# cassiusfive/balatro-gym

Measured on AMD Instinct MI355X. Metric: env-steps/sec at 65536 envs, random policy; achieved HBM GB/s vs peak, higher is better.
Workload: dtype int64/f64

## Files before the change

balatro_gym_amd/csrc/bg_device.h:

```cpp
#pragma once
#include <hip/hip_runtime.h>
#include <stdint.h>
#include "bg_tables.h"

#define BG_NHOT 8
#define BG_NDECK 4
#define BG_NCOLD 7
#define BG_NTMPL 2
#define BG_MT_N 624
#define BG_MT_M 397
#define BG_MTS 640
#define BG_BLOCK 64

#define BG_DEVERR_GSTREAM 1u
#define BG_DEVERR_SHOPBLK 2u
#define BG_DEVERR_DECKRING 4u
#define BG_DEVERR_SHOPRING 8u

typedef __attribute__((address_space(1))) unsigned long long g_u64;
typedef __attribute__((address_space(1))) uint32_t g_u32;
__device__ __forceinline__ unsigned long long bg_ld8a(const void* p) { return __hip_atomic_load((g_u64*)p, __ATOMIC_RELAXED, __HIP_MEMORY_SCOPE_AGENT); }
__device__ __forceinline__ uint32_t bg_ld4a(const void* p) { return __hip_atomic_load((g_u32*)p, __ATOMIC_RELAXED, __HIP_MEMORY_SCOPE_AGENT); }
__device__ __forceinline__ void bg_st8a(void* p, unsigned long long v) { __hip_atomic_store((g_u64*)p, v, __ATOMIC_RELAXED, __HIP_MEMORY_SCOPE_AGENT); }
__device__ __forceinline__ uint4 bg_ld16a(const void* p) {
  const unsigned long long a = bg_ld8a(p), b = bg_ld8a((const char*)p + 8);
  return make_uint4((uint32_t)a, (uint32_t)(a >> 32), (uint32_t)b, (uint32_t)(b >> 32));
}

struct BgDev {
  int N;
  uint32_t flags;
  int max_ante;
  int KG, KS, KD;
  uint4* hot;
  uint4* deck;
  uint4* cold;
  uint4* tmpl;
  uint4* ndeck;
  uint32_t* gblk;
  uint32_t* sblk;
  uint32_t* sovf;
  uint32_t* deckmt;
  uint32_t* shopgenmt;
  uint32_t* err;
  uint32_t* wl_count;
  uint32_t* wl;
  uint32_t* wl_shop;
  uint32_t* sseed;
  uint32_t* smeta;
  const uint32_t* prod_view;
  const uint32_t* prod_in;
  uint32_t* prod_out;
  unsigned long long* dbg;
  uint4* cstate;
  uint4* ctmpl;
  uint32_t* cardmt;
  uint32_t* sealmt;
  const uint32_t* jtab;
};

struct Env {
  int64_t chips_scored, round_chips;
  int64_t best_hand;
  int32_t chips_needed, money;
  int32_t hp_total, hp_ante, jokers_sold, shop_reroll_state, shop_reroll_base;
  int32_t ante, round, phase, hands_left, discards_left, hand_size, nhand, nsel, njokers, ncons, n_magic, n_minim,
      boss_type, boss_req, bflags, shop_n;
  uint64_t hand, sel;
  uint32_t highlighted, face_down, boss_hp, boss_types, cons0, cons1;
  uint64_t jokers;
  int32_t shop_ante, d_head, d_cons, d_ready;
  uint64_t boss_cards;
  uint64_t levels;
  int32_t g_cur, g_cons, g_valid;
  int32_t g_idx, s_idx, s_cur, s_cons, s_ready;
  int32_t ndrop, nfo;
  uint64_t excess;
  int32_t max_ante;
};

#define BG_BF_FIRST_HAND 1
#define BG_BF_SHOP_EXISTS 2

__device__ __forceinline__ uint32_t bg_b(uint32_t w, int i) { return (w >> (8 * i)) & 0xffu; }

__device__ __forceinline__ void bg_unpack(const uint4 c[BG_NHOT], Env& e) {
  e.chips_scored = (int64_t)(((uint64_t)c[0].y << 32) | c[0].x);
  e.round_chips = (int64_t)(((uint64_t)c[0].w << 32) | c[0].z);
  e.best_hand = (int64_t)(((uint64_t)c[1].y << 32) | c[1].x);
  e.chips_needed = (int32_t)c[1].z;
  e.money = (int32_t)c[1].w;
  e.hp_total = (int32_t)c[2].x;
  e.hp_ante = (int32_t)(c[2].y & 0xffffu);
  e.jokers_sold = (int32_t)(c[2].y >> 16);
  e.shop_reroll_state = (int32_t)c[2].z;
  e.shop_reroll_base = (int32_t)c[2].w;
  e.ante = bg_b(c[3].x, 0); e.round = bg_b(c[3].x, 1); e.phase = bg_b(c[3].x, 2); e.hands_left = bg_b(c[3].x, 3);
  e.discards_left = bg_b(c[3].y, 0); e.hand_size = (int)(int8_t)bg_b(c[3].y, 1);  e.nhand = bg_b(c[3].y, 2); e.nsel = bg_b(c[3].y, 3);
  e.njokers = bg_b(c[3].z, 0); e.ncons = bg_b(c[3].z, 1); e.n_magic = bg_b(c[3].z, 2); e.n_minim = bg_b(c[3].z, 3);
  e.boss_type = bg_b(c[3].w, 0); e.boss_req = bg_b(c[3].w, 1); e.bflags = bg_b(c[3].w, 2); e.shop_n = bg_b(c[3].w, 3);
  e.hand = ((uint64_t)c[4].y << 32) | c[4].x;
  e.sel = ((uint64_t)c[4].w << 32) | c[4].z;
  e.highlighted = c[5].x & 0xffffu; e.face_down = bg_b(c[5].x, 2); e.boss_hp = bg_b(c[5].x, 3);
  e.boss_types = c[5].y & 0xffffu; e.cons0 = bg_b(c[5].y, 2); e.cons1 = bg_b(c[5].y, 3);
  e.jokers = (uint64_t)c[5].z | ((uint64_t)(c[5].w & 0xffu) << 32);
  e.shop_ante = bg_b(c[5].w, 1); e.d_head = bg_b(c[5].w, 2); e.d_cons = bg_b(c[5].w, 3); e.d_ready = 0;
  e.boss_cards = ((uint64_t)c[6].y << 32) | c[6].x;
  e.levels = (uint64_t)c[6].z | ((uint64_t)(c[6].w & 0xffffu) << 32);
  e.g_cur = bg_b(c[6].w, 2); e.g_cons = bg_b(c[6].w, 3); e.g_valid = 0;
  e.g_idx = (int32_t)(c[7].x & 0xffffu); e.s_idx = (int32_t)(c[7].x >> 16);
  e.s_cur = bg_b(c[7].y, 0); e.s_cons = bg_b(c[7].y, 1); e.s_ready = 0; e.ndrop = bg_b(c[7].y, 2); e.nfo = bg_b(c[7].y, 3);
  e.excess = (uint64_t)c[7].z | ((uint64_t)(c[7].w & 0xffffu) << 32);
  e.max_ante = (int32_t)(c[7].w >> 16) & 0xff;
}

__device__ __forceinline__ uint32_t bg_p4(int a, int b, int c, int d) {
  return (uint32_t)(a & 0xff) | ((uint32_t)(b & 0xff) << 8) | ((uint32_t)(c & 0xff) << 16) | ((uint32_t)(d & 0xff) << 24);
}

__device__ __forceinline__ void bg_pack(const Env& e, uint4 c[BG_NHOT]) {
  c[0] = make_uint4((uint32_t)e.chips_scored, (uint32_t)((uint64_t)e.chips_scored >> 32), (uint32_t)e.round_chips,
                    (uint32_t)((uint64_t)e.round_chips >> 32));
  c[1] = make_uint4((uint32_t)e.best_hand, (uint32_t)((uint64_t)e.best_hand >> 32), (uint32_t)e.chips_needed, (uint32_t)e.money);
  c[2] = make_uint4((uint32_t)e.hp_total, ((uint32_t)e.hp_ante & 0xffffu) | ((uint32_t)e.jokers_sold << 16),
                    (uint32_t)e.shop_reroll_state, (uint32_t)e.shop_reroll_base);
  c[3] = make_uint4(bg_p4(e.ante, e.round, e.phase, e.hands_left), bg_p4(e.discards_left, e.hand_size, e.nhand, e.nsel),
                    bg_p4(e.njokers, e.ncons, e.n_magic, e.n_minim), bg_p4(e.boss_type, e.boss_req, e.bflags, e.shop_n));
  c[4] = make_uint4((uint32_t)e.hand, (uint32_t)(e.hand >> 32), (uint32_t)e.sel, (uint32_t)(e.sel >> 32));
  c[5] = make_uint4((e.highlighted & 0xffffu) | ((e.face_down & 0xffu) << 16) | ((e.boss_hp & 0xffu) << 24),
                    (e.boss_types & 0xffffu) | ((e.cons0 & 0xffu) << 16) | ((e.cons1 & 0xffu) << 24), (uint32_t)e.jokers,
                    bg_p4((int)(e.jokers >> 32), e.shop_ante, e.d_head, e.d_cons));
  c[6] = make_uint4((uint32_t)e.boss_cards, (uint32_t)(e.boss_cards >> 32), (uint32_t)e.levels,
                    ((uint32_t)(e.levels >> 32) & 0xffffu) | ((uint32_t)(e.g_cur & 0xff) << 16) | ((uint32_t)(e.g_cons & 0xff) << 24));
  c[7] = make_uint4(((uint32_t)e.g_idx & 0xffffu) | ((uint32_t)e.s_idx << 16), bg_p4(e.s_cur, e.s_cons, e.ndrop, e.nfo),
                    (uint32_t)e.excess, ((uint32_t)(e.excess >> 32) & 0xffffu) | ((uint32_t)(e.max_ante & 0xff) << 16));
}

__device__ __forceinline__ void bg_derive_ready(Env& e, uint32_t prod) {
  e.d_ready = (int)((prod - (uint32_t)e.d_cons) & 0xffu);
  e.s_ready = (int)(((prod >> 8) - (uint32_t)e.s_cons) & 0xffu);
  e.g_valid = (int)(((prod >> 16) - (uint32_t)e.g_cons) & 0xffu);
}
__device__ __forceinline__ void bg_load_env(const BgDev& d, int env, Env& e) {
  uint4 c[BG_NHOT];
#pragma unroll
  for (int k = 0; k < BG_NHOT; k++) c[k] = d.hot[(size_t)k * d.N + env];
  bg_unpack(c, e);
  bg_derive_ready(e, d.prod_view ? d.prod_view[env] : 0u);
}
__device__ __forceinline__ void bg_store_env(const BgDev& d, int env, const Env& e) {
  uint4 c[BG_NHOT];
  bg_pack(e, c);
#pragma unroll
  for (int k = 0; k < BG_NHOT; k++) d.hot[(size_t)k * d.N + env] = c[k];
}

__device__ __forceinline__ int bg_get8(uint64_t v, int i) { return (int)((v >> (8 * i)) & 0xffull); }
__device__ __forceinline__ uint64_t bg_set8(uint64_t v, int i, int x) {
  return (v & ~(0xffull << (8 * i))) | ((uint64_t)(x & 0xff) << (8 * i));
}
__device__ __forceinline__ uint64_t bg_del8(uint64_t v, int i) {
  uint64_t lowmask = i ? ((1ull << (8 * i)) - 1) : 0ull;
  uint64_t lo = v & lowmask;
  uint64_t hi = (i < 7) ? (v >> (8 * (i + 1))) << (8 * i) : 0ull;
  return lo | hi;
}
__device__ __forceinline__ int bg_level(const Env& e, int ht) { return (int)((e.levels >> (4 * ht)) & 0xf); }

__device__ __forceinline__ uint32_t* bg_gblock(const BgDev& d, int env, int slot) { return d.gblk + ((size_t)env * d.KG + slot) * BG_MTS; }
#define BG_SW_T 56
#define BG_SW_PK 56
#define BG_SW_SEED 62
#define BG_SLOT_WORDS 64
#define BG_S_FASTMAX (BG_SW_T - 1)
static_assert(BG_SW_T >= 28 && BG_SW_PK == BG_SW_T && BG_SW_PK % 4 == 0 && BG_SW_PK + 6 == BG_SW_SEED && BG_SW_SEED + 2 == BG_SLOT_WORDS, "shop slot");
#define BG_BF_SHOP_OVF 4
__device__ __forceinline__ uint32_t* bg_sblock(const BgDev& d, int env, int slot) { return d.sblk + ((size_t)env * d.KS + slot) * BG_SLOT_WORDS; }
__device__ __forceinline__ uint32_t* bg_sovf(const BgDev& d, int env) { return d.sovf + (size_t)env * BG_MTS; }
__device__ __forceinline__ void bg_mt_seed_rolled(uint32_t* p, uint32_t key) {
  uint32_t g = 19650218u, a = g;
#pragma unroll 1
  for (uint32_t i = 1; i < 624u; i++) {
    g = 1812433253u * (g ^ (g >> 30)) + i;
    a = (g ^ ((a ^ (a >> 30)) * 1664525u)) + key;
    p[i] = a;
  }
  __builtin_amdgcn_fence(__ATOMIC_RELEASE, "agent");
  __builtin_amdgcn_fence(__ATOMIC_ACQUIRE, "agent");
  const uint32_t m1 = (p[1] ^ ((a ^ (a >> 30)) * 1664525u)) + key;
  uint32_t b = m1;
#pragma unroll 1
  for (uint32_t i = 2; i < 624u; i++) {
    b = (p[i] ^ ((b ^ (b >> 30)) * 1566083941u)) - i;
    p[i] = b;
  }
  p[1] = (m1 ^ ((b ^ (b >> 30)) * 1566083941u)) - 1u;
  p[0] = 0x80000000u;
}
__device__ __forceinline__ uint32_t* bg_deckmt(const BgDev& d, int env) { return d.deckmt + (size_t)env * BG_MTS; }
__device__ __forceinline__ uint32_t* bg_shopgenmt(const BgDev& d, int env) { return d.shopgenmt + (size_t)env * BG_MTS; }

#ifdef BG_TIMING
__shared__ unsigned long long bg_probe_lds[32];
#define BG_PROBE_BEGIN() unsigned long long _pt = __builtin_readcyclecounter()
#define BG_PROBE(k) do { unsigned long long _n = __builtin_readcyclecounter(); \
    if ((int)threadIdx.x == __ffsll((long long)__ballot(1)) - 1 + (int)(threadIdx.x & ~63u)) atomicAdd(&bg_probe_lds[k], _n - _pt); \
    _pt = __builtin_readcyclecounter(); } while (0)
#define BG_PROBE_INIT() do { if (threadIdx.x < 32) bg_probe_lds[threadIdx.x] = 0; __syncthreads(); } while (0)
#define BG_PROBE_FLUSH(d) do { __syncthreads(); if (threadIdx.x < 32 && (d).dbg && bg_probe_lds[threadIdx.x]) atomicAdd(&(d).dbg[threadIdx.x], bg_probe_lds[threadIdx.x]); } while (0)
#else
#define BG_PROBE_BEGIN() do {} while (0)
#define BG_PROBE(k) do {} while (0)
#define BG_PROBE_INIT() do {} while (0)
#define BG_PROBE_FLUSH(d) do {} while (0)
#endif

#define BG_RB 128
typedef __attribute__((address_space(3))) uint8_t lds_u8;
typedef __attribute__((address_space(3))) uint32_t lds_u32;
struct Deck0 { uint64_t lo, hi; static constexpr bool kCards = false; };
struct DeckLds { lds_u32* col; static constexpr bool kCards = false; };
struct Deck0C : Deck0 { static constexpr bool kCards = true; };
struct DeckLdsC : DeckLds { static constexpr bool kCards = true; };
#define BG_NCST 7
__device__ __forceinline__ uint32_t bg_cstate(const BgDev& d, int env, int ci) {
  return (uint32_t)((const uint16_t*)&d.cstate[(size_t)(ci >> 3) * d.N + env])[ci & 7];
}
__device__ __forceinline__ Deck0 bg_load_deck0(const BgDev& d, int env) {
  uint4 c = d.deck[env];
  Deck0 r;
  r.lo = ((uint64_t)c.y << 32) | c.x;
  r.hi = ((uint64_t)c.w << 32) | c.z;
  return r;
}
__device__ __forceinline__ void bg_deck_set(Deck0& dk, int k, uint4 c) {
  if (k == 0) { dk.lo = ((uint64_t)c.y << 32) | c.x; dk.hi = ((uint64_t)c.w << 32) | c.z; }
}
__device__ __forceinline__ void bg_deck_set(DeckLds& dk, int k, uint4 c) {
  dk.col[(4 * k) * BG_RB] = c.x; dk.col[(4 * k + 1) * BG_RB] = c.y; dk.col[(4 * k + 2) * BG_RB] = c.z; dk.col[(4 * k + 3) * BG_RB] = c.w;
}
__device__ __forceinline__ int bg_card(const BgDev& d, int env, const Deck0& k, int idx) {
  if (idx < 16) return (int)(((idx < 8 ? k.lo : k.hi) >> (8 * (idx & 7))) & 0xffull);
  const uint32_t* p = (const uint32_t*)&d.deck[(size_t)(idx >> 4) * d.N + env];
  return (int)((bg_ld4a(p + ((idx & 15) >> 2)) >> (8 * (idx & 3))) & 0xffu);
}
template <int S, bool C> struct DeckLdsS { lds_u32* col; static constexpr bool kCards = C; };
template <int S, bool C>
__device__ __forceinline__ void bg_deck_set(DeckLdsS<S, C>& dk, int k, uint4 c) {
  dk.col[(4 * k) * S] = c.x; dk.col[(4 * k + 1) * S] = c.y; dk.col[(4 * k + 2) * S] = c.z; dk.col[(4 * k + 3) * S] = c.w;
}
template <int S, bool C>
__device__ __forceinline__ int bg_card(const BgDev& d, int env, const DeckLdsS<S, C>& k, int idx) {
  return (int)((const lds_u8*)k.col)[(idx >> 2) * (S * 4) + (idx & 3)];
}
__device__ __forceinline__ int bg_card(const BgDev& d, int env, const DeckLds& k, int idx) {
  return (int)((const lds_u8*)k.col)[(idx >> 2) * (BG_RB * 4) + (idx & 3)];
}

struct DeckHead { uint64_t lo, hi; };
__device__ __forceinline__ DeckHead bg_deck_head(const BgDev& d, int env, const Deck0& k) { return DeckHead{k.lo, k.hi}; }
template <int S, bool C>
__device__ __forceinline__ DeckHead bg_deck_head(const BgDev& d, int env, const DeckLdsS<S, C>& k) {
  const uint32_t a = k.col[0], b = k.col[S], c = k.col[2 * S], e = k.col[3 * S];
  return DeckHead{((uint64_t)b << 32) | a, ((uint64_t)e << 32) | c};
}
template <class DK>
__device__ __forceinline__ int bg_card_h(const BgDev& d, int env, const DK& k, const DeckHead& h, int idx) {
  if (idx < 16) return (int)(((idx < 8 ? h.lo : h.hi) >> (8 * (idx & 7))) & 0xffull);
  return bg_card(d, env, k, idx);
}

__device__ __forceinline__ uint32_t bg_temper(uint32_t y) {
  y ^= (y >> 11);
  y ^= (y << 7) & 0x9d2c5680u;
  y ^= (y << 15) & 0xefc60000u;
  y ^= (y >> 18);
  return y;
}
__device__ __forceinline__ uint32_t bg_twist(uint32_t a, uint32_t b, uint32_t far) {
  uint32_t y = (a & 0x80000000u) | (b & 0x7fffffffu);
  return far ^ (y >> 1) ^ ((y & 1u) ? 0x9908b0dfu : 0u);
}

__device__ __forceinline__ uint32_t bg_lazy_next(uint32_t* S) {
  uint32_t c = S[BG_MT_N] & 0x3ffu;
  const uint32_t c1 = c + 1 == BG_MT_N ? 0u : c + 1, cf = c + BG_MT_M >= BG_MT_N ? c + BG_MT_M - BG_MT_N : c + BG_MT_M;
  const uint32_t y = bg_twist(S[c], S[c1], S[cf]);
  S[c] = y;
  S[BG_MT_N] = c1 | 0x80000000u;
  return bg_temper(y);
}
__device__ __forceinline__ double bg_lazy_random(uint32_t* S) {
  const uint32_t a = bg_lazy_next(S) >> 5, b = bg_lazy_next(S) >> 6;
  return ((double)a * 67108864.0 + (double)b) * (1.0 / 9007199254740992.0);
}

#define BG_WIN 16
struct JTables {
  uint64_t jd[152];
  uint32_t jm[152];
  uint64_t jr[152];
  uint8_t jf[152];
  uint8_t cost[152];
  double pow115[101];
  double pow15[16];
  double pow08[16];
  uint32_t inv[64];
};
typedef __attribute__((address_space(3))) const JTables lds_JTables;
struct RngWin {
  lds_JTables* jt;
  lds_u32* lds;
  int g_blk, g_start, g_len;
  int s_start, s_len;
  bool defer_adv;
  bool need_inv;
};
__device__ __forceinline__ void bg_win_init(RngWin& w, uint32_t* lds_lane, const JTables* jt = nullptr) {
  w.jt = (lds_JTables*)jt; w.lds = (lds_u32*)lds_lane; w.g_blk = -1; w.g_start = 0; w.g_len = 0; w.s_start = 0; w.s_len = 0; w.defer_adv = false; w.need_inv = false;
}
__device__ __noinline__ void bg_win_fill(lds_u32* lds, const uint32_t* src, int len) {
#pragma unroll 1
  for (int base = 0; base < len; base += BG_WIN) {
    uint32_t v[BG_WIN];
#pragma unroll
    for (int j = 0; j < BG_WIN; j++) v[j] = (base + j < len) ? src[base + j] : 0u;
#pragma unroll
    for (int j = 0; j < BG_WIN; j++) if (base + j < len) lds[(base + j) * BG_BLOCK] = v[j];
  }
}

__device__ __forceinline__ void bg_gnorm(const BgDev& d, Env& e) {
  if (e.g_idx >= BG_MT_N) { e.g_cur = (e.g_cur + 1 == d.KG) ? 0 : e.g_cur + 1; e.g_idx -= BG_MT_N; e.g_valid--; e.g_cons = (e.g_cons + 1) & 0xff; }
}
__device__ __forceinline__ void bg_gskip(const BgDev& d, Env& e, int count) {
  bg_gnorm(d, e);
  e.g_idx += count;
}
__device__ __forceinline__ uint32_t bg_gdraw(const BgDev& d, int env, Env& e, RngWin& w) {
  bg_gnorm(d, e);
  if (e.g_valid <= 0) { atomicOr(d.err, BG_DEVERR_GSTREAM); e.g_valid = 0; return 0u; }
  uint32_t off = (uint32_t)(e.g_idx - w.g_start);
  uint32_t y;
  if (w.g_blk == e.g_cur && off < (uint32_t)w.g_len) y = w.lds[off * BG_BLOCK];
  else y = bg_gblock(d, env, e.g_cur)[e.g_idx];
  e.g_idx++;
  return bg_temper(y);
}
__device__ __forceinline__ uint32_t bg_gpeek(const BgDev& d, int env, const Env& e, int off) {
  int idx = e.g_idx + off, blk = e.g_cur, need = 1;
  if (idx >= BG_MT_N) { idx -= BG_MT_N; blk = (blk + 1 == d.KG) ? 0 : blk + 1; need = 2; }
  if (idx >= BG_MT_N) { idx -= BG_MT_N; blk = (blk + 1 == d.KG) ? 0 : blk + 1; need = 3; }
  if (e.g_valid < need) { atomicOr(d.err, BG_DEVERR_GSTREAM); return 0u; }
  return bg_temper(bg_gblock(d, env, blk)[idx]);
}
__device__ __forceinline__ const uint32_t* bg_gpeek_addr(const BgDev& d, int env, const Env& e, int off, bool& ok) {
  int idx = e.g_idx + off, blk = e.g_cur, need = 1;
  if (idx >= BG_MT_N) { idx -= BG_MT_N; blk = (blk + 1 == d.KG) ? 0 : blk + 1; need = 2; }
  if (idx >= BG_MT_N) { idx -= BG_MT_N; blk = (blk + 1 == d.KG) ? 0 : blk + 1; need = 3; }
  ok = e.g_valid >= need;
  return bg_gblock(d, env, ok ? blk : e.g_cur) + (ok ? idx : 0);
}
__device__ __forceinline__ uint32_t bg_gtouch(const BgDev& d, int env, const Env& e, int off) {
  int idx = e.g_idx + off, blk = e.g_cur, need = 1;
  if (idx >= BG_MT_N) { idx -= BG_MT_N; blk = (blk + 1 == d.KG) ? 0 : blk + 1; need = 2; }
  if (idx >= BG_MT_N) { idx -= BG_MT_N; blk = (blk + 1 == d.KG) ? 0 : blk + 1; need = 3; }
  return e.g_valid >= need ? bg_gblock(d, env, blk)[idx] : 0u;
}
struct __attribute__((packed, aligned(4))) BgU4 { uint32_t x, y, z, w; };
__device__ __forceinline__ void bg_gpeek12(const BgDev& d, int env, const Env& e, int skip, uint32_t (&out)[12], uint32_t& avail) {
  int idx = e.g_idx + skip, blk = e.g_cur, need = 1;
  if (idx >= BG_MT_N) { idx -= BG_MT_N; blk = (blk + 1 == d.KG) ? 0 : blk + 1; need = 2; }
  if (idx >= BG_MT_N) { idx -= BG_MT_N; blk = (blk + 1 == d.KG) ? 0 : blk + 1; need = 3; }
  avail = 0;
  if (e.g_valid >= need) {
    const int in_blk = BG_MT_N - idx;
    avail = (e.g_valid > need || in_blk >= 12) ? 0xfffu : ((1u << in_blk) - 1u);
    const BgU4* p = (const BgU4*)(bg_gblock(d, env, blk) + idx);
#pragma unroll
    for (int g = 0; g < 3; g++) {
      BgU4 v = p[g];
      out[4 * g] = bg_temper(v.x); out[4 * g + 1] = bg_temper(v.y); out[4 * g + 2] = bg_temper(v.z); out[4 * g + 3] = bg_temper(v.w);
    }
  } else {
#pragma unroll
    for (int i = 0; i < 12; i++) out[i] = 0u;
  }
}
__device__ __forceinline__ void bg_gpeek12_raw(const BgDev& d, int env, const Env& e, int skip, uint32_t (&out)[12], uint32_t& avail) {
  int idx = e.g_idx + skip, blk = e.g_cur, need = 1;
  if (idx >= BG_MT_N) { idx -= BG_MT_N; blk = (blk + 1 == d.KG) ? 0 : blk + 1; need = 2; }
  if (idx >= BG_MT_N) { idx -= BG_MT_N; blk = (blk + 1 == d.KG) ? 0 : blk + 1; need = 3; }
  const bool have = e.g_valid >= need;
  const int in_blk = BG_MT_N - idx;
  avail = have ? ((e.g_valid > need || in_blk >= 12) ? 0xfffu : ((1u << in_blk) - 1u)) : 0u;
  const BgU4* p = (const BgU4*)(bg_gblock(d, env, have ? blk : e.g_cur) + (have ? idx : 0));
#pragma unroll
  for (int g = 0; g < 3; g++) {
    const BgU4 v = p[g];
    out[4 * g] = v.x; out[4 * g + 1] = v.y; out[4 * g + 2] = v.z; out[4 * g + 3] = v.w;
  }
}
__device__ __forceinline__ void bg_gprefetch(const BgDev& d, int env, Env& e, RngWin& w, int count) {
  bg_gnorm(d, e);
  if (e.g_valid <= 0) return;
  int len = BG_MT_N - e.g_idx;
  if (len > count) len = count;
  if (len > BG_WIN) len = BG_WIN;
  bg_win_fill(w.lds, bg_gblock(d, env, e.g_cur) + e.g_idx, len);
  w.g_blk = e.g_cur; w.g_start = e.g_idx; w.g_len = len;
  w.s_len = 0;
}
__device__ __noinline__ uint32_t bg_sword_slow(const uint32_t* S, int k) {
  uint32_t far;
  if (k < BG_MT_N - BG_MT_M) far = S[k + BG_MT_M];
  else {
    const int k1 = k - (BG_MT_N - BG_MT_M);
    uint32_t far1;
    if (k1 < BG_MT_N - BG_MT_M) far1 = S[k1 + BG_MT_M];
    else { const int k2 = k1 - (BG_MT_N - BG_MT_M); far1 = bg_twist(S[k2], S[k2 + 1], S[k2 + BG_MT_M]); }
    far = bg_twist(S[k1], S[k1 + 1], far1);
  }
  const uint32_t nxt = k < BG_MT_N - 1 ? S[k + 1] : bg_twist(S[0], S[1], S[BG_MT_M]);
  return bg_twist(S[k], nxt, far);
}
__device__ __forceinline__ void bg_shop_overflow(const BgDev& d, int env, Env& e) {
  bg_mt_seed_rolled(bg_sovf(d, env), bg_sblock(d, env, e.s_cur)[BG_SW_SEED]);
  __builtin_amdgcn_fence(__ATOMIC_RELEASE, "agent");
  __builtin_amdgcn_fence(__ATOMIC_ACQUIRE, "agent");
  e.bflags |= BG_BF_SHOP_OVF;
}
__device__ __forceinline__ const uint32_t* bg_sbase(const BgDev& d, int env, const Env& e, bool& full) {
  full = (e.bflags & BG_BF_SHOP_OVF) != 0;
  if (full) __builtin_amdgcn_fence(__ATOMIC_ACQUIRE, "agent");
  return full ? bg_sovf(d, env) : bg_sblock(d, env, e.s_cur);
}
__device__ __forceinline__ uint32_t bg_sdraw(const BgDev& d, int env, Env& e, RngWin& w) {
  if (e.s_idx >= BG_MT_N) { atomicOr(d.err, BG_DEVERR_SHOPBLK); return 0u; }
  uint32_t off = (uint32_t)(e.s_idx - w.s_start);
  uint32_t y;
  if (off < (uint32_t)w.s_len) y = w.lds[off * BG_BLOCK];
  else {
    if (e.s_idx > BG_S_FASTMAX && !(e.bflags & BG_BF_SHOP_OVF)) bg_shop_overflow(d, env, e);
    bool full;
    const uint32_t* S = bg_sbase(d, env, e, full);
    y = full ? bg_temper(bg_sword_slow(S, e.s_idx)) : S[e.s_idx];
  }
  e.s_idx++;
  return y;
}
__device__ __forceinline__ void bg_swin_fill(lds_u32* lds, const uint32_t* S, bool full, int k0, int len) {
  if (!full) {
    uint32_t A[BG_WIN];
#pragma unroll
    for (int j = 0; j < BG_WIN; j++) A[j] = (j < len) ? S[k0 + j] : 0u;
#pragma unroll
    for (int j = 0; j < BG_WIN; j++) if (j < len) lds[j * BG_BLOCK] = A[j];
    return;
  }
  uint32_t A[BG_WIN + 1], F[BG_WIN];
  const uint32_t* SF = S + k0 + BG_MT_M;
#pragma unroll
  for (int j = 0; j < BG_WIN + 1; j++) A[j] = (j <= len) ? S[k0 + j] : 0u;
#pragma unroll
  for (int j = 0; j < BG_WIN; j++) F[j] = (j < len) ? SF[j] : 0u;
#pragma unroll
  for (int j = 0; j < BG_WIN; j++) if (j < len) lds[j * BG_BLOCK] = bg_temper(bg_twist(A[j], A[j + 1], F[j]));
}
__device__ __forceinline__ void bg_sprefetch(const BgDev& d, int env, Env& e, RngWin& w, int count) {
  bool full;
  const uint32_t* S = bg_sbase(d, env, e, full);
  int len = (full ? (BG_MT_N - BG_MT_M) : (BG_S_FASTMAX + 1)) - e.s_idx;
  if (len > count) len = count;
  if (len > BG_WIN) len = BG_WIN;
  if (len < 0) len = 0;
  if (len > 0) bg_swin_fill(w.lds, S, full, e.s_idx, len);
  w.s_start = e.s_idx; w.s_len = len;
  w.g_len = 0; w.g_blk = -1;
}
template <bool SHOP>
__device__ __forceinline__ uint32_t bg_randbelow(const BgDev& d, int env, Env& e, RngWin& w, uint32_t n) {
  int k = 32 - __clz(n);
  uint32_t r;
  int guard = 0;
  do {
    r = (SHOP ? bg_sdraw(d, env, e, w) : bg_gdraw(d, env, e, w)) >> (32 - k);
  } while (r >= n && ++guard < 4096);
  return r < n ? r : 0u;
}
__device__ __forceinline__ double bg_grandom(const BgDev& d, int env, Env& e, RngWin& w) {
  uint32_t a = bg_gdraw(d, env, e, w) >> 5;
  uint32_t b = bg_gdraw(d, env, e, w) >> 6;
  return ((double)a * 67108864.0 + (double)b) * (1.0 / 9007199254740992.0);
}

__device__ __forceinline__ int bg_card_chips(int code) {
  int r = (code >> 2) + 2;
  return r <= 10 ? r : (r == 14 ? 11 : 10);
}
__device__ __forceinline__ void bg_hand_base(int ht, int level, int& chips, int& mult) {
  int bc, bm;
  switch (ht) {
    case 0: bc = 5; bm = 1; break;
// ... 80 lines not shown
```

balatro_gym_amd/csrc/bg_lib.hip:

```cpp
#include "../../include/balatro_mi355x.h"
#include "bg_step.h"
#include <hip/hip_ext.h>
#include <stdio.h>
#include <stdlib.h>
#include <string.h>
#include <type_traits>
#include <string>
#include <vector>


struct InfoPtrs {
  int64_t* final_score; int32_t* error; int32_t* flags; int32_t* aux; int8_t* hand_type; int8_t* cards_played;
  double* reward_terms;
  double* score_breakdown;
};

static_assert(offsetof(ObsPtrs, rows) == sizeof(bg_obs_ptrs), "the first 31 members of ObsPtrs must mirror bg_obs_ptrs");
static_assert(sizeof(InfoPtrs) == sizeof(bg_info_ptrs), "InfoPtrs must mirror bg_info_ptrs");

__device__ __forceinline__ void bg_emit_info(size_t row, const StepOut& o, uint8_t* trunc, const InfoPtrs& info) {
  if (trunc) trunc[row] = 0;
  if (info.final_score) info.final_score[row] = o.final_score;
  if (info.error) info.error[row] = o.error;
  if (info.flags) info.flags[row] = o.flags;
  if (info.aux) info.aux[row] = o.aux;
  if (info.hand_type) info.hand_type[row] = (int8_t)o.hand_type;
  if (info.cards_played) info.cards_played[row] = (int8_t)o.cards_played;
  if (info.reward_terms) {
    double2* q = (double2*)(info.reward_terms + row * 8);
#pragma unroll
    for (int i = 0; i < 4; i++) q[i] = make_double2(o.terms[2 * i], o.terms[2 * i + 1]);
  }
  if (info.score_breakdown && o.hand_type < 0) {
    double2* q = (double2*)(info.score_breakdown + row * 8);
#pragma unroll
    for (int i = 0; i < 4; i++) q[i] = make_double2(0.0, 0.0);
  }
}

#include "bg_engine.h"
#include "bg_engine3.h"

template <bool CARDS>
__global__ __launch_bounds__(BG_BLOCK) void bg_reset_kernel(BgDev d, const uint8_t* __restrict__ mask_in, ObsPtrs obs) {
  using DeckT = typename std::conditional<CARDS, Deck0C, Deck0>::type;
  int env = blockIdx.x * BG_BLOCK + threadIdx.x;
  if (env >= d.N) return;
  Env e;
  bg_load_env(d, env, e);
  DeckT dk; static_cast<Deck0&>(dk) = bg_load_deck0(d, env);
  if (!mask_in || mask_in[env]) { bg_env_reset(d, env, e, dk); bg_store_env(d, env, e); }
  ShopRegs sr; sr.valid = false;
  uint64_t mask = bg_action_mask(d, env, e, sr);
  bg_write_obs<false>(d, env, (size_t)env, e, dk, obs, mask, sr, RowExtra{0.0, 0, 0u});
}

__global__ __launch_bounds__(BG_BLOCK) void bg_observe_kernel(BgDev d, ObsPtrs obs) {
  int env = blockIdx.x * BG_BLOCK + threadIdx.x;
  if (env >= d.N) return;
  Env e;
  bg_load_env(d, env, e);
  Deck0 dk = bg_load_deck0(d, env);
  ShopRegs sr; sr.valid = false;
  uint64_t mask = bg_action_mask(d, env, e, sr);
  bg_write_obs<false>(d, env, (size_t)env, e, dk, obs, mask, sr, RowExtra{0.0, 0, 0u});
}

struct alignas(64) BgG16 { uint32_t v[16]; };
struct BgGenrandTab {
  BgG16 blk[BG_MT_N / 16];
  constexpr BgGenrandTab() : blk{} {
    uint32_t x = 19650218u;
    blk[0].v[0] = x;
    for (int i = 1; i < BG_MT_N; i++) { x = 1812433253u * (x ^ (x >> 30)) + (uint32_t)i; blk[i / 16].v[i % 16] = x; }
  }
};
static_assert(BG_MT_N % 16 == 0, "624 = 39 blocks of 16");
static constexpr BgGenrandTab BG_GENRAND{};

template <bool SLOT>
__device__ __forceinline__ void bg_mt_seed_impl(uint32_t* p, uint32_t key) {
  constexpr int NB = BG_MT_N / 16;
  uint4* p4 = (uint4*)p;
  uint32_t a = BG_GENRAND.blk[0].v[0], a1 = 0;
  {
    BgG16 cur = BG_GENRAND.blk[0];
#pragma unroll 1
    for (int b = 0; b < NB; b++) {
      const BgG16 nxt = BG_GENRAND.blk[b + 1 < NB ? b + 1 : NB - 1];
#pragma unroll
      for (int c = 0; c < 16; c++) {
        if (b > 0 || c >= 1) {
          a = (cur.v[c] ^ ((a ^ (a >> 30)) * 1664525u)) + key;
          if (b == 0 && c == 1) a1 = a;
        }
      }
      cur = nxt;
    }
  }
  const uint32_t a1w = (a1 ^ ((a ^ (a >> 30)) * 1664525u)) + key;
  a = BG_GENRAND.blk[0].v[0];
  a = (BG_GENRAND.blk[0].v[1] ^ ((a ^ (a >> 30)) * 1664525u)) + key;
  uint32_t bprev = a1w, w2 = 0, w3 = 0;
  uint32_t far0 = 0, far1 = 0, out2 = 0, out3 = 0;
  uint32_t acc = 0;
  {
    BgG16 cur = BG_GENRAND.blk[0];
#pragma unroll 1
    for (int b = 0; b < NB; b++) {
      const BgG16 nxt = BG_GENRAND.blk[b + 1 < NB ? b + 1 : NB - 1];
      uint32_t v[16];
#pragma unroll
      for (int c = 0; c < 16; c++) {
        v[c] = 0;
        if (b > 0 || c >= 2) {
          a = (cur.v[c] ^ ((a ^ (a >> 30)) * 1664525u)) + key;
          bprev = (a ^ ((bprev ^ (bprev >> 30)) * 1566083941u)) - (uint32_t)(16 * b + c);
          v[c] = bprev;
        }
      }
      if (b == 0) { w2 = v[2]; w3 = v[3]; }
      if constexpr (!SLOT) {
#pragma unroll
        for (int k = 0; k < 4; k++) {
          const int q = 4 * b + k;
          if (q == 0) continue;
          p4[q] = make_uint4(v[4 * k], v[4 * k + 1], v[4 * k + 2], v[4 * k + 3]);
        }
      } else {
        if (b < 4) {
#pragma unroll
          for (int k = 0; k < 4; k++) if (4 * b + k > 0) p4[4 * b + k] = make_uint4(v[4 * k], v[4 * k + 1], v[4 * k + 2], v[4 * k + 3]);
        } else if (b >= 24 && b <= 28) {
          const int kb = 16 * b - BG_MT_M;
          if (b == 24) { far0 = v[13]; far1 = v[14]; out2 = bg_temper(bg_twist(w2, w3, v[15])); }
          else {
            const int g0 = kb >> 2;
            uint32_t nr[20];
#pragma unroll
            for (int g = 0; g < 5; g++) {
              uint4 t = make_uint4(0u, 0u, 0u, 0u);
              if (g0 + g > 0 && g0 + g < BG_SLOT_WORDS / 4) t = p4[g0 + g];
              nr[4 * g] = t.x; nr[4 * g + 1] = t.y; nr[4 * g + 2] = t.z; nr[4 * g + 3] = t.w;
            }
            if (b == 25) nr[3] = w3;
            auto outputs = [&](auto kbc) {
              constexpr int KB = decltype(kbc)::value;
#pragma unroll
              for (int c = 0; c < 16; c++) {
                const int k = KB + c;
                if (k < BG_SW_T) {
                  const uint32_t o = bg_temper(bg_twist(nr[3 + c], nr[4 + c], v[c]));
                  if (k == 3) out3 = o; else p[k] = o;
                  if (k >= 4 && k < 24) {
                    acc |= (o >> 24) << (8 * (k & 3));
                    if ((k & 3) == 3) { p[BG_SW_PK + (k >> 2)] = acc; acc = 0u; }
                  }
                }
              }
            };
            if (b == 25) outputs(std::integral_constant<int, 16 * 25 - BG_MT_M>{});
            else if (b == 26) outputs(std::integral_constant<int, 16 * 26 - BG_MT_M>{});
            else if (b == 27) outputs(std::integral_constant<int, 16 * 27 - BG_MT_M>{});
            else outputs(std::integral_constant<int, 16 * 28 - BG_MT_M>{});
          }
        }
      }
      cur = nxt;
    }
  }
  const uint32_t w1 = (a1w ^ ((bprev ^ (bprev >> 30)) * 1566083941u)) - 1u;
  if constexpr (!SLOT) p4[0] = make_uint4(0x80000000u, w1, w2, w3);
  else {
    const uint32_t out0 = bg_temper(bg_twist(0x80000000u, w1, far0)), out1 = bg_temper(bg_twist(w1, w2, far1));
    p4[0] = make_uint4(out0, out1, out2, out3);
    static_assert(BG_SW_PK == 56 && BG_SW_SEED == 62 && BG_SLOT_WORDS == 64, "slot tail layout");
    p[BG_SW_PK] = (out0 >> 24) | ((out1 >> 24) << 8) | ((out2 >> 24) << 16) | (out3 & 0xff000000u);
    *(uint2*)(p + BG_SW_SEED) = make_uint2(key, 0u);
  }
}
__device__ void bg_mt_seed(uint32_t* __restrict__ p, uint32_t key) { bg_mt_seed_impl<false>(p, key); }
__device__ void bg_mt_seed_slot(uint32_t* __restrict__ p, uint32_t key) { bg_mt_seed_impl<true>(p, key); }

__device__ __forceinline__ uint32_t bg_q156(uint32_t q) { return q >= 156u ? q - 156u : q; }
#define BG_LAZY_U 4
#define BG_LAZY_U_SEEDRING 2
#define BG_WL_COUNTERS 32
#define BG_REFILL_WAVE_PRIO 0
template <int U = BG_LAZY_U, class F>
__device__ __forceinline__ uint32_t bg_lazy_stream(uint32_t* S, uint32_t c, bool active, F&& take) {
  uint4* S4 = (uint4*)S;
  uint32_t q = c >> 2, off = c & 3u, fq = bg_q156(q + 99u);
  uint4 a[U + 1], f[U + 1];
#pragma unroll
  for (int g = 0; g <= U; g++) { a[g] = make_uint4(0, 0, 0, 0); f[g] = a[g]; }
  if (active) {
#pragma unroll
    for (int g = 0; g <= U; g++) { a[g] = S4[bg_q156(q + (uint32_t)g)]; f[g] = S4[bg_q156(fq + (uint32_t)g)]; }
  }
#pragma unroll 1
  while (__ballot(active) != 0ull) {
    uint4 an[U], fn[U];
#pragma unroll
    for (int g = 0; g < U; g++) { an[g] = a[0]; fn[g] = a[0]; }
    if (active) {
#pragma unroll
      for (int g = 0; g < U; g++) { an[g] = S4[bg_q156(q + (uint32_t)(U + 1 + g))]; fn[g] = S4[bg_q156(fq + (uint32_t)(U + 1 + g))]; }
    }
    bool more = active;
#pragma unroll
    for (int g = 0; g < U; g++) {
      const uint4 a0 = a[g], f0 = f[g];
      const uint32_t n0 = bg_twist(a0.x, a0.y, f0.y), n1 = bg_twist(a0.y, a0.z, f0.z), n2 = bg_twist(a0.z, a0.w, f0.w), n3 = bg_twist(a0.w, a[g + 1].x, f[g + 1].x);
      const uint32_t goff = g == 0 ? off : 0u;
      uint4 o = a0;
      uint32_t used = 0;
      if (more && goff == 0u) { o.x = n0; used++; more = take(n0); }
      if (more && goff <= 1u) { o.y = n1; used++; more = take(n1); }
      if (more && goff <= 2u) { o.z = n2; used++; more = take(n2); }
      if (more) { o.w = n3; used++; more = take(n3); }
      if (used) {
        const uint32_t qg = bg_q156(q + (uint32_t)g);
        S4[qg] = o;
        if (!more) { c = 4u * qg + goff + used; if (c >= (uint32_t)BG_MT_N) c -= (uint32_t)BG_MT_N; active = false; }
      }
    }
    q = bg_q156(q + (uint32_t)U); fq = bg_q156(fq + (uint32_t)U); off = 0u;
    a[0] = a[U]; f[0] = f[U];
#pragma unroll
    for (int g = 0; g < U; g++) { a[g + 1] = an[g]; f[g + 1] = fn[g]; }
  }
  return c;
}

#define BG_MTB 16
#define BG_SSEED 128
#define BG_LAZY_SEEDED 0x80000000u
__device__ void bg_mt_twist(const uint32_t* src, uint32_t* dst) {
  uint32_t cur = src[0], first_new = 0;
  const uint4* s4 = (const uint4*)src;
  uint4* d4 = (uint4*)dst;
#pragma unroll 1
  for (int base = 0; base < BG_MT_N; base += BG_MTB) {
    uint32_t nx[BG_MTB + 4], fr[BG_MTB + 4];
#pragma unroll
    for (int g = 0; g < BG_MTB / 4 + 1; g++) { uint4 v = s4[base / 4 + g]; nx[4 * g] = v.x; nx[4 * g + 1] = v.y; nx[4 * g + 2] = v.z; nx[4 * g + 3] = v.w; }
    if (base == 224) {
#pragma unroll
      for (int j = 0; j < BG_MTB; j++) { int kk = base + j; fr[j + 1] = (kk < BG_MT_N - BG_MT_M) ? src[kk + BG_MT_M] : dst[kk + BG_MT_M - BG_MT_N]; }
    } else {
      const uint4* f4 = base < 224 ? s4 + (base + BG_MT_M - 1) / 4 : (const uint4*)dst + (base + BG_MT_M - BG_MT_N - 1) / 4;
#pragma unroll
      for (int g = 0; g < BG_MTB / 4 + 1; g++) { uint4 v = f4[g]; fr[4 * g] = v.x; fr[4 * g + 1] = v.y; fr[4 * g + 2] = v.z; fr[4 * g + 3] = v.w; }
    }
    uint32_t v[BG_MTB];
#pragma unroll
    for (int j = 0; j < BG_MTB; j++) {
      uint32_t nxt = (base + j == BG_MT_N - 1) ? first_new : nx[j + 1];
      v[j] = bg_twist(cur, nxt, fr[j + 1]);
      if (base + j == 0) first_new = v[j];
      cur = nxt;
    }
#pragma unroll
    for (int j = 0; j < BG_MTB / 4; j++) d4[base / 4 + j] = make_uint4(v[4 * j], v[4 * j + 1], v[4 * j + 2], v[4 * j + 3]);
  }
}

#include "bg_ops.h"
#include "bg_sim.h"
#include "bg_encode.h"
#include "bg_gae.h"
#include "bg_norm.h"
#include "bg_head.h"

__global__ __launch_bounds__(BG_BLOCK) void bg_seed_kernel(BgDev d, const int64_t* __restrict__ seeds,
                                                          const uint8_t* __restrict__ mask_in, int reseed_global) {
  int env = blockIdx.x * BG_BLOCK + threadIdx.x;
  if (env >= d.N) return;
  if (mask_in && !mask_in[env]) return;
  RngWin w;
  bg_win_init(w, nullptr);
  Env e;
  bg_load_env(d, env, e);
  int64_t seed = seeds[env];
  if (reseed_global) {
    uint32_t gs = (uint32_t)((uint64_t)seed + 16000ull);
    uint32_t* g = bg_gblock(d, env, 0);
    bg_mt_seed(g, gs);
    bg_mt_twist(g, g);
    e.g_cur = 0; e.g_idx = 0; e.g_cons = 0; e.g_valid = 1;
  }
  if (seed == 0) {
    uint64_t r;
    int guard = 0;
    do {
      uint64_t lo = bg_gdraw(d, env, e, w);
      uint64_t hi = bg_gdraw(d, env, e, w) >> 31;
      r = lo | (hi << 32);
    } while (r >= 4294967296ull && ++guard < 4096);
    seed = (int64_t)(r & 0xffffffffull);
  }
  uint32_t base = (uint32_t)(uint64_t)seed;
  bg_mt_seed(bg_deckmt(d, env), base);
  bg_deckmt(d, env)[BG_MT_N] = BG_LAZY_SEEDED;
  bg_mt_seed(bg_shopgenmt(d, env), base + 2000u);
  bg_shopgenmt(d, env)[BG_MT_N] = BG_LAZY_SEEDED;
  if (d.cardmt) {
    bg_mt_seed(d.cardmt + (size_t)env * BG_MTS, base + 11000u);
    d.cardmt[(size_t)env * BG_MTS + BG_MT_N] = BG_LAZY_SEEDED;
    bg_mt_seed(d.sealmt + (size_t)env * BG_MTS, base + 13000u);
    d.sealmt[(size_t)env * BG_MTS + BG_MT_N] = BG_LAZY_SEEDED;
  }
  e.d_head = 0; e.d_cons = 0; e.d_ready = 0;
  e.s_cons = 0; e.s_ready = 0;
  d.smeta[env] = 0;
  {
    uint32_t gp = reseed_global ? 1u : (uint32_t)((e.g_cons + e.g_valid) & 0xff);
    uint32_t pv = 0u | (0u << 8) | (gp << 16) | 0x80000000u;
    d.prod_out[env] = pv;
    ((uint32_t*)d.prod_in)[env] = pv;
  }
  bg_store_env(d, env, e);
}

__global__ __launch_bounds__(BG_BLOCK) void bg_refill_zero_kernel(BgDev d) { if (threadIdx.x < BG_WL_COUNTERS) d.wl_count[threadIdx.x] = 0; }

struct BgPart { uint32_t p, q; };
__device__ __forceinline__ uint32_t bg_part_lo(uint32_t count, BgPart pt) { return (uint32_t)(((uint64_t)count * pt.p) / pt.q); }
__device__ __forceinline__ uint32_t bg_part_hi(uint32_t count, BgPart pt) { return (uint32_t)(((uint64_t)count * (pt.p + 1u)) / pt.q); }

__global__ __launch_bounds__(BG_BLOCK) void bg_refill_scan_kernel(BgDev d) {
  int env = blockIdx.x * BG_BLOCK + threadIdx.x;
  if (env >= d.N) return;
  size_t N = d.N;
  uint32_t w5 = ((const uint32_t*)&d.hot[(size_t)5 * N + env])[3];
  uint32_t w6 = ((const uint32_t*)&d.hot[(size_t)6 * N + env])[3];
  uint2 w7 = *((const uint2*)&d.hot[(size_t)7 * N + env]);
  uint32_t prod = d.prod_in[env];
  int d_cons = bg_b(w5, 3), g_cons = bg_b(w6, 3), s_cur = bg_b(w7.y, 0), s_cons = bg_b(w7.y, 1);
  int d_ready = (int)((prod - (uint32_t)d_cons) & 0xffu);
  int s_ready = (int)(((prod >> 8) - (uint32_t)s_cons) & 0xffu);
  int g_valid = (int)(((prod >> 16) - (uint32_t)g_cons) & 0xffu);
  const bool seeded = (prod >> 31) != 0;
  if (!seeded) { d.prod_out[env] = prod; return; }
  if (s_ready < d.KS - 1) {
    uint32_t sm = d.smeta[env];
    int head = (int)(sm & 0xffu), cnt = (int)((sm >> 8) & 0xffu);
    int emitted = d.KS - 1 - s_ready;
    if (emitted > cnt) emitted = cnt;
    if (emitted > 0) {
      const uint32_t base = atomicAdd(&d.wl_count[3], (uint32_t)emitted);
#pragma unroll 1
      for (int k = 0; k < emitted; k++) {
        int slot = s_cur + 1 + s_ready + k; while (slot >= d.KS) slot -= d.KS;
        d.wl_shop[2 * (size_t)(base + k)] = (uint32_t)env | ((uint32_t)slot << 24);
        d.wl_shop[2 * (size_t)(base + k) + 1] = d.sseed[(size_t)env * BG_SSEED + ((head + k) & (BG_SSEED - 1))];
      }
      head = (head + emitted) & (BG_SSEED - 1); cnt -= emitted;
    } else emitted = 0;
    if (emitted) {
      d.smeta[env] = (uint32_t)head | ((uint32_t)cnt << 8);
      prod = (prod & 0xffff00ffu) | ((((prod >> 8) + (uint32_t)emitted) & 0xffu) << 8);
    }
    if (cnt < BG_SSEED - 8) { uint32_t i = atomicAdd(&d.wl_count[1], 1u); d.wl[N + i] = (uint32_t)env; }
  }
  d.prod_out[env] = prod;
  if (d_ready < d.KD) { uint32_t i = atomicAdd(&d.wl_count[0], 1u); d.wl[i] = (uint32_t)env; }
  if (g_valid > 0 && g_valid < d.KG) { uint32_t i = atomicAdd(&d.wl_count[2], 1u); d.wl[2 * N + i] = (uint32_t)env; }
}

__global__ __launch_bounds__(BG_BLOCK) __attribute__((amdgpu_waves_per_eu(4, 4))) void bg_refill_deck_kernel(BgDev d, BgPart pt, uint32_t cursor_idx, uint32_t max_made) {
  __builtin_amdgcn_s_setprio(BG_REFILL_WAVE_PRIO);
  __shared__ uint8_t sdeck[52][BG_BLOCK];
  const size_t N = d.N;
  const int tid = threadIdx.x;
  const uint32_t count0 = d.wl_count[0], lo = bg_part_lo(count0, pt), count = bg_part_hi(count0, pt);
  uint32_t* const cursor = &d.wl_count[cursor_idx];
  const int cap = max_made ? (int)max_made : 1 << 30;
  int env = 0, d_head = 0, d_ready = 0, made = 0;
  uint32_t prod = 0, cur = 0;
  uint32_t* mt = bg_deckmt(d, 0);
  bool have = false, need = false, dry = false;
#pragma unroll 1
  while (true) {
    if (!dry) {
      const unsigned long long freem = __ballot(!have);
      if (freem != 0ull) {
        const int leader = __ffsll(freem) - 1, nfree = __popcll(freem);
        uint32_t base = 0;
        if (tid == leader) base = atomicAdd(cursor, (uint32_t)nfree);
        base = lo + (uint32_t)__shfl((int)base, leader);
        dry = base + (uint32_t)nfree >= count;
        const uint32_t my = base + (uint32_t)__popcll(freem & ((1ull << tid) - 1ull));
        if (!have && my < count) {
          env = (int)d.wl[my];
          mt = bg_deckmt(d, env);
          const uint32_t w5 = ((const uint32_t*)&d.hot[(size_t)5 * N + env])[3];
          prod = d.prod_out[env];
          d_head = bg_b(w5, 2);
          d_ready = (int)((prod - (uint32_t)bg_b(w5, 3)) & 0xffu);
          cur = mt[BG_MT_N] & 0x3ffu;
          made = 0;
          need = d_ready < d.KD;
          have = need;
        }
      }
    }
    if (__ballot(need) == 0ull) { if (dry) break; continue; }
    if (need) { int p = 0; for (int s = 0; s < 4; s++) for (int r = 0; r < 13; r++) sdeck[p++][tid] = (uint8_t)(r * 4 + s); }
    int i = 51;
    cur = bg_lazy_stream(mt, cur, need, [&](uint32_t y) {
      const int k = 32 - __clz((uint32_t)(i + 1));
      const uint32_t j = bg_temper(y) >> (32 - k);
      if (j <= (uint32_t)i) {
        const uint8_t a = sdeck[i][tid], b = sdeck[j][tid];
        sdeck[i][tid] = b; sdeck[j][tid] = a;
        i--;
      }
      return i >= 1;
    });
    if (need) {
      const int slot = (d_head + d_ready) % d.KD;
#pragma unroll
      for (int k = 0; k < BG_NDECK; k++) {
        uint32_t wv[4] = {0, 0, 0, 0};
#pragma unroll
        for (int b = 0; b < 16; b++) { int i2 = k * 16 + b; if (i2 < 52) wv[b >> 2] |= (uint32_t)sdeck[i2][tid] << (8 * (b & 3)); }
        d.ndeck[((size_t)slot * BG_NDECK + k) * N + env] = make_uint4(wv[0], wv[1], wv[2], wv[3]);
      }
      d_ready++; made++;
      need = d_ready < d.KD && made < cap;
      if (!need) {
        mt[BG_MT_N] = cur | BG_LAZY_SEEDED;
        ((uint8_t*)&d.prod_out[env])[0] = (uint8_t)((prod + (uint32_t)made) & 0xffu);
        have = false;
      }
    }
  }
}

__global__ __launch_bounds__(BG_BLOCK) void bg_refill_seedring_kernel(BgDev d, BgPart pt) {
  __builtin_amdgcn_s_setprio(BG_REFILL_WAVE_PRIO);
  size_t N = d.N;
  const uint32_t count0 = d.wl_count[1], lo = bg_part_lo(count0, pt), count = bg_part_hi(count0, pt);
  for (uint32_t base = lo + blockIdx.x * BG_BLOCK; base < count; base += gridDim.x * BG_BLOCK) {
    const bool valid = base + threadIdx.x < count;
    const int env = valid ? (int)d.wl[N + base + threadIdx.x] : 0;
    uint32_t* mt = bg_shopgenmt(d, env);
    int head = 0, cnt = BG_SSEED;
    uint32_t cur = 0;
    if (valid) {
      const uint32_t sm = d.smeta[env];
      head = (int)(sm & 0xffu); cnt = (int)((sm >> 8) & 0xffu);
      cur = mt[BG_MT_N] & 0x3ffu;
    }
    const bool need = valid && cnt < BG_SSEED;
    cur = bg_lazy_stream<BG_LAZY_U_SEEDRING>(mt, cur, need, [&](uint32_t y) {
      const uint32_t r = bg_temper(y);
      if (r < 2147483648u) { d.sseed[(size_t)env * BG_SSEED + ((head + cnt) & (BG_SSEED - 1))] = r; cnt++; }
      return cnt < BG_SSEED;
    });
    if (need) {
      mt[BG_MT_N] = cur | BG_LAZY_SEEDED;
      d.smeta[env] = (uint32_t)head | ((uint32_t)cnt << 8);
    }
  }
}

__global__ __launch_bounds__(BG_BLOCK, 8) void bg_refill_shop_kernel(BgDev d, BgPart pt) {
  const uint32_t count0 = d.wl_count[3], lo = bg_part_lo(count0, pt), count = bg_part_hi(count0, pt);
  for (uint32_t item = lo + blockIdx.x * BG_BLOCK + threadIdx.x; item < count; item += gridDim.x * BG_BLOCK) {
    uint32_t es = d.wl_shop[2 * (size_t)item], seed = d.wl_shop[2 * (size_t)item + 1];
    bg_mt_seed_slot(bg_sblock(d, (int)(es & 0xffffffu), (int)(es >> 24)), seed);
  }
}
__global__ __launch_bounds__(BG_BLOCK) void bg_refill_gblk_kernel(BgDev d, BgPart pt) {
  __builtin_amdgcn_s_setprio(BG_REFILL_WAVE_PRIO);
  const size_t N = d.N;
  const uint32_t count0 = d.wl_count[2], lo = bg_part_lo(count0, pt), count = bg_part_hi(count0, pt);
  const int l = threadIdx.x;
  constexpr int NR = (BG_MT_N + 63) / 64;
  for (uint32_t item = lo + blockIdx.x; item < count; item += gridDim.x) {
    const int env = (int)d.wl[2 * N + item];
    const uint32_t w6 = ((const uint32_t*)&d.hot[(size_t)6 * N + env])[3];
    const uint32_t prod = d.prod_out[env];
    const int g_cur = bg_b(w6, 2), g_cons = bg_b(w6, 3);
    int g_valid = (int)(((prod >> 16) - (uint32_t)g_cons) & 0xffu);
    if (g_valid <= 0 || g_valid >= d.KG) continue;
    int last = (g_cur + g_valid - 1) % d.KG, made = 0;
    uint32_t o[NR + 1];
    {
      const uint32_t* src = bg_gblock(d, env, last);
#pragma unroll
      for (int r = 0; r < NR; r++) o[r] = (64 * r + l < BG_MT_N) ? __builtin_nontemporal_load(&src[64 * r + l]) : 0u;
      o[NR] = 0u;
    }
#pragma unroll 1
    while (g_valid < d.KG) {
      const int nxt = last + 1 == d.KG ? 0 : last + 1;
      uint32_t* dst = bg_gblock(d, env, nxt);
      uint32_t n[NR];
#pragma unroll
      for (int r = 0; r < NR; r++) {
        const int k = 64 * r + l;
        const uint32_t up_same = __shfl(o[r], (l + 1) & 63), up_next = __shfl(o[r + 1], 0);
        uint32_t up = l == 63 ? up_next : up_same;
        if (r == NR - 1) { const uint32_t new0 = __shfl(n[0], 0); if (k == BG_MT_N - 1) up = new0; }
        uint32_t far = 0u;
        if (64 * r < BG_MT_N - BG_MT_M) {
          const uint32_t a = r + 6 < NR ? __shfl(o[r + 6], (l + 13) & 63) : 0u, b2 = r + 7 < NR ? __shfl(o[r + 7], (l + 13) & 63) : 0u;
          far = l + 13 < 64 ? a : b2;
        }
        if (64 * r + 63 >= BG_MT_N - BG_MT_M) {
          const uint32_t a = r >= 4 ? __shfl(n[r >= 4 ? r - 4 : 0], (l + 29) & 63) : 0u, b2 = r >= 3 ? __shfl(n[r >= 3 ? r - 3 : 0], (l + 29) & 63) : 0u;
          const uint32_t fn = l + 29 < 64 ? a : b2;
          if (k >= BG_MT_N - BG_MT_M) far = fn;
        }
        n[r] = bg_twist(o[r], up, far);
        if (k < BG_MT_N) __builtin_nontemporal_store(n[r], &dst[k]);
      }
      if (l < 16) bg_gblock(d, env, last)[BG_MT_N + l] = n[0];
#pragma unroll
      for (int r = 0; r < NR; r++) o[r] = n[r];
      last = nxt; g_valid++; made++;
    }
    if (made && l == 0) {
      const uint32_t g = ((prod >> 16) + (uint32_t)made) & 0xffu;
      ((uint8_t*)&d.prod_out[env])[2] = (uint8_t)g;
    }
  }
}

__global__ __launch_bounds__(BG_BLOCK) void bg_inject_kernel(BgDev d, const uint8_t* __restrict__ mask_in) {
  int env = blockIdx.x * BG_BLOCK + threadIdx.x;
  if (env >= d.N) return;
  if (mask_in && !mask_in[env]) return;
  Env e;
  bg_load_env(d, env, e);
  uint4 t0 = d.tmpl[env], t1 = d.tmpl[(size_t)d.N + env];
  if (t0.y & 0x80000000u) { e.njokers = (int)bg_b(t0.y, 1); e.jokers = (uint64_t)t0.x | ((uint64_t)(t0.y & 0xffu) << 32); }
  if (t0.y & 0x40000000u) e.money = (int32_t)t0.z;
  if (t0.y & 0x20000000u) e.ante = (int)bg_b(t0.y, 2);
  if (t0.y & 0x10000000u) { e.levels = (uint64_t)t1.x | ((uint64_t)(t1.y & 0xffffu) << 32); e.excess = 0; }
  if (t1.z & 0x80000000u) { e.ncons = (int)bg_b(t1.z, 0); e.cons0 = bg_b(t1.z, 1); e.cons1 = bg_b(t1.z, 2); }
  bg_store_env(d, env, e);
}

__global__ __launch_bounds__(256) void bg_tables_build_kernel(uint32_t* out) {
  __shared__ JTables jt;
  { uint32_t* w = (uint32_t*)&jt; for (int i = threadIdx.x; i < (int)(sizeof(JTables) / 4); i += blockDim.x) w[i] = 0u; }
  __syncthreads();
  bg_tables_init(&jt);
  const uint32_t* w = (const uint32_t*)&jt;
  for (int i = threadIdx.x; i < (int)(sizeof(JTables) / 4); i += blockDim.x) out[i] = w[i];
}

__global__ __launch_bounds__(BG_BLOCK) void bg_inject_deck_kernel(BgDev d, const uint4* __restrict__ decks, const uint8_t* __restrict__ mask_in) {
  int env = blockIdx.x * BG_BLOCK + threadIdx.x;
  if (env >= d.N) return;
  if (mask_in && !mask_in[env]) return;
#pragma unroll
  for (int k = 0; k < BG_NDECK; k++) d.deck[(size_t)k * d.N + env] = decks[(size_t)env * BG_NDECK + k];
}
__global__ __launch_bounds__(BG_BLOCK) void bg_set_cap_kernel(BgDev d, const int32_t* __restrict__ caps, int scalar, const uint8_t* __restrict__ mask_in) {
  int env = blockIdx.x * BG_BLOCK + threadIdx.x;
  if (env >= d.N) return;
  if (mask_in && !mask_in[env]) return;
  uint32_t* w = ((uint32_t*)&d.hot[(size_t)7 * d.N + env]) + 3;
  const int cap = caps ? caps[env] : scalar;
  *w = (*w & 0xffffu) | ((uint32_t)(cap & 0xff) << 16);
}

struct bg_handle {
  BgDev dev;
  int device_id;
  bool seeded;
  int64_t* d_seeds;
  uint8_t* d_mask;
  uint32_t* d_jtab;
  int steps_since_refill;
  std::vector<uint4> h_tmpl;
  std::vector<hipEvent_t> ev_pool;
  std::vector<uint8_t> h_cap;
  uint64_t bytes;
  std::string err;
  bool profiling;
  uint32_t* d_prod[2];
  long refill_seq;
  long refill_done;
  long view_min;
  bool async_refill;
  hipStream_t side;
  hipEvent_t ev_refill[2];
  hipEvent_t ev_rollout;
  std::vector<hipEvent_t> ev_rollout_t, ev_refill_t, ev_step_t;
  std::vector<int> rollout_steps;
  struct RefillPiece { int kind; uint32_t part, nparts; int grid; uint32_t cursor, max_made; };
  std::vector<RefillPiece> pieces;
  size_t piece_next;
  BgDev piece_dev;
  int refill_sliced, piece_parts[4], deck_passes;
  uint32_t eng_smask; int eng_copiers;
  int engine;
  int e3_cfg, e3_epw;
  uint8_t* gpeer[8]; uint8_t** d_gpeer; int gworld, grank;
};

static std::string g_create_err;

struct BgDeviceGuard {
  int prev = -1;
  bool switched = false;
  explicit BgDeviceGuard(int dev) {
    if (hipGetDevice(&prev) == hipSuccess && prev != dev) switched = hipSetDevice(dev) == hipSuccess;
  }
  ~BgDeviceGuard() { if (switched) (void)hipSetDevice(prev); }
};
#define BG_GUARD(h) BgDeviceGuard _guard((h)->device_id)

#define BG_HIP(call)                                                                                   \
  do {                                                                                                 \
    hipError_t _e = (call);                                                                            \
    if (_e != hipSuccess) {                                                                            \
      h->err = std::string(#call) + ": " + hipGetErrorString(_e);                                      \
      return BG_E_HIP;                                                                                 \
    }                                                                                                  \
  } while (0)

template <typename T>
static hipError_t bg_alloc(bg_handle* h, T** p, size_t count) {
  size_t bytes = count * sizeof(T);
  hipError_t e = hipMalloc((void**)p, bytes);
  if (e != hipSuccess) return e;
  h->bytes += bytes;
  return hipMemset(*p, 0, bytes);
}

static int bg_grid(const bg_handle* h) { return (h->dev.N + BG_BLOCK - 1) / BG_BLOCK; }

static hipEvent_t bg_ev_take(bg_handle* h) {
  if (!h->ev_pool.empty()) { hipEvent_t e = h->ev_pool.back(); h->ev_pool.pop_back(); return e; }
  hipEvent_t e = nullptr;
  return hipEventCreate(&e) == hipSuccess ? e : nullptr;
}
static void bg_ev_begin(bg_handle* h, std::vector<hipEvent_t>& v, hipStream_t s) {
  if (!h->profiling) return;
  hipEvent_t a = bg_ev_take(h), b = bg_ev_take(h);
  if (!a || !b) { if (a) h->ev_pool.push_back(a); if (b) h->ev_pool.push_back(b); return; }
  v.push_back(a); v.push_back(b);
  (void)hipEventRecord(a, s);
}
static void bg_ev_pair(bg_handle* h, std::vector<hipEvent_t>& v, hipEvent_t& a, hipEvent_t& b) {
  a = b = nullptr;
  if (!h->profiling) return;
  a = bg_ev_take(h); b = bg_ev_take(h);
  if (!a || !b) { if (a) h->ev_pool.push_back(a); if (b) h->ev_pool.push_back(b); a = b = nullptr; return; }
  v.push_back(a); v.push_back(b);
}
static void bg_ev_end(bg_handle* h, std::vector<hipEvent_t>& v, hipStream_t s) {
  if (!h->profiling || v.empty()) return;
  (void)hipEventRecord(v.back(), s);
}
static double bg_ev_sum(bg_handle* h, std::vector<hipEvent_t>& v) {
  double ms = 0;
  for (size_t i = 0; i + 1 < v.size(); i += 2) {
    float f = 0;
    if (hipEventElapsedTime(&f, v[i], v[i + 1]) == hipSuccess) ms += f;
    h->ev_pool.push_back(v[i]); h->ev_pool.push_back(v[i + 1]);
  }
  v.clear();
  return ms;
}

#ifndef BG_BUILD_SIGNATURE
#define BG_BUILD_SIGNATURE "unsigned"
#endif

extern "C" {

static const char bg_sig_marker[] = "bgsig:" BG_BUILD_SIGNATURE;
const char* bg_build_signature(void) { return bg_sig_marker + 6; }

int bg_debug_counters(bg_handle* h, unsigned long long* out16) {
  if (!h || !out16) return BG_E_ARG;
  BG_GUARD(h);
  BG_HIP(hipDeviceSynchronize());
  BG_HIP(hipMemcpy(out16, h->dev.dbg, 32 * sizeof(unsigned long long), hipMemcpyDeviceToHost));
  BG_HIP(hipMemset(h->dev.dbg, 0, 32 * sizeof(unsigned long long)));
  return 0;
}

static long bg_gwords(int flags, int steps) { return (flags & BG_FLAG_SCORER_JOKERS) ? 32l * steps + 128 : 24l * steps; }
static int bg_gsteps(int flags, int blocks) {
  const long w = (long)blocks * BG_MT_N;
  const long t = (flags & BG_FLAG_SCORER_JOKERS) ? (w - 128) / 32 : w / 24;
  return t < 0 ? 0 : (int)t;
}

int bg_debug_worklists(bg_handle* h, unsigned int* out4) {
  if (!h || !out4) return BG_E_ARG;
  BG_GUARD(h);
  BG_HIP(hipDeviceSynchronize());
  BG_HIP(hipMemcpy(out4, h->dev.wl_count, 4 * sizeof(unsigned int), hipMemcpyDeviceToHost));
  return 0;
}

int bg_set_profiling(bg_handle* h, int enable) {
  if (!h) return BG_E_ARG;
  h->profiling = enable != 0;
  if (h->profiling) { BG_GUARD(h); while (h->ev_pool.size() < 128) { hipEvent_t e = nullptr; if (hipEventCreate(&e) != hipSuccess) break; h->ev_pool.push_back(e); } }
  return 0;
}

int bg_get_profile(bg_handle* h, double* out8) {
  if (!h || !out8) return BG_E_ARG;
  BG_GUARD(h);
  BG_HIP(hipDeviceSynchronize());
  double nr = (double)(h->ev_rollout_t.size() / 2), nf = (double)(h->ev_refill_t.size() / 2), ns = (double)(h->ev_step_t.size() / 2);
  double steps = 0;
  for (int t : h->rollout_steps) steps += t;
  h->rollout_steps.clear();
  out8[0] = bg_ev_sum(h, h->ev_rollout_t); out8[1] = nr; out8[2] = steps;
  out8[3] = bg_ev_sum(h, h->ev_refill_t); out8[4] = nf;
  out8[5] = bg_ev_sum(h, h->ev_step_t); out8[6] = ns; out8[7] = 0;
  return 0;
}

int bg_create(int n_envs, int device_id, uint32_t flags, int max_ante, bg_handle** out) { return bg_create_ex(n_envs, device_id, flags, max_ante, 0, out); }

int bg_create_ex(int n_envs, int device_id, uint32_t flags, int max_ante, int fused_steps_hint, bg_handle** out) {
  if (!out || n_envs <= 0) { g_create_err = "bg_create: bad arguments"; return BG_E_ARG; }
  int ndev = 0;
  if (hipGetDeviceCount(&ndev) != hipSuccess || ndev <= 0) {
    g_create_err = "bg_create: no HIP device visible (this library has no CPU fallback)";
    return BG_E_NODEVICE;
  }
  if (device_id < 0 || device_id >= ndev) { g_create_err = "bg_create: device_id out of range"; return BG_E_ARG; }
  bg_handle* h = new bg_handle();
  h->device_id = device_id; h->seeded = false; h->bytes = 0; h->profiling = false;
  { const char* av = getenv("BG_ASYNC_REFILL"); h->async_refill = av ? atoi(av) != 0 : true; }
  {
    auto geti = [](const char* k, int dflt) { const char* v = getenv(k); return v ? atoi(v) : dflt; };
    h->refill_sliced = geti("BG_REFILL_SLICED", 1);
    { const int dp[4] = {2, 1, 2, 8};
      for (int k = 0; k < 4; k++) h->piece_parts[k] = dp[k];
      auto get4 = [](const char* k, int* out, int lo, int hi) { const char* v = getenv(k); if (!v) return; int a[4]; if (sscanf(v, "%d,%d,%d,%d", &a[0], &a[1], &a[2], &a[3]) == 4) for (int i = 0; i < 4; i++) out[i] = a[i] < lo ? lo : a[i] > hi ? hi : a[i]; };
      get4("BG_REFILL_PARTS", h->piece_parts, 1, 16); }
    h->piece_next = 0;
    h->deck_passes = 3;
    while (h->deck_passes * h->piece_parts[0] > BG_WL_COUNTERS - 8) { if (h->deck_passes > 1) h->deck_passes--; else h->piece_parts[0]--; }
    h->eng_smask = (uint32_t)geti("BG_ENG_SMASK", BG_ENG_SMASK_DEFAULT); h->eng_copiers = geti("BG_ENG_COPIERS", 0); if (h->eng_copiers < 0 || h->eng_copiers > 3) h->eng_copiers = 0;
    if (h->eng_smask == 0 || h->eng_smask >= (1u << BG_ENG_NW) || __builtin_popcount(h->eng_smask) > BG_ENG_NSV) h->eng_smask = BG_ENG_SMASK_DEFAULT;
    h->engine = geti("BG_ENGINE", 3);
    if (h->engine != 1 && h->engine != 3) { delete h; g_create_err = "bg_create: BG_ENGINE must be 3 (bg_engine3.h, the default) or 1 (bg_engine.h); the two-kernel engine 2 was retired in round 5"; return BG_E_ARG; }
    h->e3_cfg = geti("BG_E3_CFG", 0);
    if (h->e3_cfg != 0 && h->e3_cfg != 113 && h->e3_cfg != 213 && h->e3_cfg != 413) { delete h; g_create_err = "bg_create: BG_E3_CFG must be 113, 213 or 413 (100 x owner waves + 10 x slices + service waves)"; return BG_E_ARG; }
    for (int g = 0; g < 8; g++) h->gpeer[g] = nullptr;
    h->d_gpeer = nullptr;
    h->gworld = 0; h->grank = 0;
    h->e3_epw = geti("BG_E3_EPW", 0);
    if (h->e3_epw != 0 && (h->e3_epw < 1 || h->e3_epw > 64)) { delete h; g_create_err = "bg_create: BG_E3_EPW must be in [1, 64]"; return BG_E_ARG; }
  }
  h->d_prod[0] = h->d_prod[1] = nullptr; h->refill_seq = 0; h->view_min = 0; h->refill_done = -1; h->side = nullptr;
  h->ev_refill[0] = h->ev_refill[1] = nullptr; h->ev_rollout = nullptr;
  h->d_seeds = nullptr; h->d_mask = nullptr; h->d_jtab = nullptr; h->steps_since_refill = 0;
  memset(&h->dev, 0, sizeof(h->dev));
  BgDev& d = h->dev;
  d.N = n_envs; d.flags = flags; d.max_ante = max_ante;
  const char* kg = getenv("BG_KG"); const char* ks = getenv("BG_KS"); const char* kd = getenv("BG_KD");
  int dsd = n_envs <= 131072 ? 248 : (n_envs <= 262144 ? 124 : (n_envs <= 1048576 ? 24 : 12));
  int dg = 2 * (int)((bg_gwords(flags, 3 * (dsd / 2)) + BG_MT_N - 1) / BG_MT_N) + 1; if (dg < 5) dg = 5;
  if (fused_steps_hint > 0) {
    const int hint = fused_steps_hint > 372 ? 372 : fused_steps_hint;
    int ring = 2 * ((hint + 2) / 3); if (ring < 4) ring = 4;
    int gb = 2 * (int)((bg_gwords(flags, hint) + BG_MT_N - 1) / BG_MT_N) + 1; if (gb < 5) gb = 5;
    if (ring < dsd) dsd = ring;
    if (gb < dg) dg = gb;
  }
  d.KG = kg ? atoi(kg) : dg; d.KS = ks ? atoi(ks) : dsd + 1; d.KD = kd ? atoi(kd) : dsd;
  if (d.KG < 2 || d.KS < 2 || d.KD < 1 || d.KG > 250 || d.KS > 250 || d.KD > 250) { delete h; g_create_err = "bg_create: bad ring depths"; return BG_E_ARG; }
  size_t N = (size_t)n_envs;
  BG_GUARD(h);
  hipError_t e = hipSuccess;
  if (e == hipSuccess) e = bg_alloc(h, &d.hot, BG_NHOT * N);
  if (e == hipSuccess) e = bg_alloc(h, &d.deck, BG_NDECK * N);
  if (e == hipSuccess) e = bg_alloc(h, &d.cold, BG_NCOLD * N);
  if (e == hipSuccess) e = bg_alloc(h, &d.tmpl, BG_NTMPL * N);
  if (e == hipSuccess) e = bg_alloc(h, &d.ndeck, (size_t)d.KD * BG_NDECK * N);
  if (e == hipSuccess) e = bg_alloc(h, &d.gblk, (size_t)d.KG * BG_MTS * N);
  if (e == hipSuccess) e = bg_alloc(h, &d.sblk, (size_t)d.KS * BG_SLOT_WORDS * N);
  if (e == hipSuccess) e = bg_alloc(h, &d.sovf, (size_t)BG_MTS * N);
  if (e == hipSuccess && (flags & BG_FLAG_CARD_STATES)) {
    e = bg_alloc(h, &d.cstate, (size_t)BG_NCST * N);
    if (e == hipSuccess) e = bg_alloc(h, &d.ctmpl, (size_t)BG_NCST * N);
    if (e == hipSuccess) e = bg_alloc(h, &d.cardmt, (size_t)BG_MTS * N);
    if (e == hipSuccess) e = bg_alloc(h, &d.sealmt, (size_t)BG_MTS * N);
  }
  if (e == hipSuccess) e = bg_alloc(h, &d.deckmt, (size_t)BG_MTS * N);
  if (e == hipSuccess) e = bg_alloc(h, &d.shopgenmt, (size_t)BG_MTS * N);
  if (e == hipSuccess) e = bg_alloc(h, &d.wl_count, BG_WL_COUNTERS);
  if (e == hipSuccess) e = bg_alloc(h, &d.wl, 3 * N);
  if (e == hipSuccess) e = bg_alloc(h, &d.wl_shop, 2 * N * (size_t)(d.KS - 1));
  if (e == hipSuccess) e = bg_alloc(h, &d.sseed, (size_t)BG_SSEED * N);
  if (e == hipSuccess) e = bg_alloc(h, &d.smeta, N);
  if (e == hipSuccess) e = bg_alloc(h, &h->d_prod[0], N);
  if (e == hipSuccess) e = bg_alloc(h, &h->d_prod[1], N);
  int prio_least = 0, prio_greatest = 0;
  if (e == hipSuccess) e = hipDeviceGetStreamPriorityRange(&prio_least, &prio_greatest);
  if (e == hipSuccess) e = hipStreamCreateWithPriority(&h->side, hipStreamNonBlocking, prio_least);
  if (e == hipSuccess) e = hipEventCreateWithFlags(&h->ev_refill[0], hipEventDisableTiming);
  if (e == hipSuccess) e = hipEventCreateWithFlags(&h->ev_refill[1], hipEventDisableTiming);
  if (e == hipSuccess) e = hipEventCreateWithFlags(&h->ev_rollout, hipEventDisableTiming);
  if (e == hipSuccess) e = bg_alloc(h, &h->d_jtab, (sizeof(JTables) + 3) / 4);
  if (e == hipSuccess) e = bg_alloc(h, &d.dbg, 32);
  if (e == hipSuccess) e = bg_alloc(h, &d.err, 4);
  if (e == hipSuccess) e = bg_alloc(h, &h->d_seeds, N);
  if (e == hipSuccess) e = bg_alloc(h, &h->d_mask, N);
  if (e != hipSuccess) {
    g_create_err = std::string("bg_create: ") + hipGetErrorString(e);
    bg_destroy(h);
    return BG_E_HIP;
  }
  d.prod_view = h->d_prod[0]; d.prod_in = h->d_prod[0]; d.prod_out = h->d_prod[1];
  d.jtab = h->d_jtab;
  hipLaunchKernelGGL(bg_tables_build_kernel, dim3(1), dim3(256), 0, 0, h->d_jtab);
  if (hipGetLastError() != hipSuccess || hipDeviceSynchronize() != hipSuccess) { g_create_err = "bg_create: table kernel failed"; bg_destroy(h); return BG_E_HIP; }
  h->h_tmpl.assign(BG_NTMPL * N, make_uint4(0, 0, 0, 0));
  h->h_cap.assign(N, (uint8_t)(max_ante > 0 && max_ante < 256 ? max_ante : 0));
  if (max_ante < 0 || max_ante > 255) { g_create_err = "bg_create: max_ante must be in [0, 255]"; bg_destroy(h); return BG_E_ARG; }
  if (max_ante > 0) {
    hipLaunchKernelGGL(bg_set_cap_kernel, dim3(bg_grid(h)), dim3(BG_BLOCK), 0, 0, d, (const int32_t*)nullptr, max_ante, (const uint8_t*)nullptr);
    if (hipGetLastError() != hipSuccess || hipDeviceSynchronize() != hipSuccess) { g_create_err = "bg_create: cap kernel failed"; bg_destroy(h); return BG_E_HIP; }
  }
  *out = h;
  return 0;
}

int bg_destroy(bg_handle* h) {
  if (!h) return 0;
  { BG_GUARD(h);
  BgDev& d = h->dev;
  (void)hipDeviceSynchronize();
  if (h->side) (void)hipStreamDestroy(h->side);
  for (int i = 0; i < 2; i++) if (h->ev_refill[i]) (void)hipEventDestroy(h->ev_refill[i]);
  if (h->ev_rollout) (void)hipEventDestroy(h->ev_rollout);
  for (hipEvent_t e : h->ev_pool) (void)hipEventDestroy(e);
  for (auto* v : {&h->ev_rollout_t, &h->ev_refill_t, &h->ev_step_t}) for (hipEvent_t e : *v) (void)hipEventDestroy(e);
  hipFree(h->d_prod[0]); hipFree(h->d_prod[1]);
  hipFree(d.hot); hipFree(d.deck); hipFree(d.cold); hipFree(d.tmpl); hipFree(d.ndeck); hipFree(d.gblk); hipFree(d.sblk); hipFree(d.sovf);
  hipFree(d.deckmt); hipFree(d.shopgenmt); hipFree(d.err); hipFree(h->d_seeds); hipFree(h->d_mask); hipFree(d.wl_count); hipFree(d.wl); hipFree(d.wl_shop); hipFree(d.sseed); hipFree(d.smeta); hipFree(d.dbg); hipFree(h->d_jtab); hipFree(h->d_gpeer); hipFree(d.cstate); hipFree(d.ctmpl); hipFree(d.cardmt); hipFree(d.sealmt);
  }
  delete h;
  return 0;
}

const char* bg_last_error(const bg_handle* h) { return h ? h->err.c_str() : g_create_err.c_str(); }
int bg_num_envs(const bg_handle* h) { return h ? h->dev.N : 0; }

static int bg_chunk_limit(const bg_handle* h, bool* async_out) {
  int ring = h->dev.KD < h->dev.KS - 1 ? h->dev.KD : h->dev.KS - 1;
  int gblocks = h->dev.KG - 1;
  const bool async = h->async_refill && ring >= 2 && gblocks >= 2;
  if (async) { ring /= 2; gblocks /= 2; }
  int max_chunk = 3 * ring;
  int gchunk = bg_gsteps(h->dev.flags, gblocks);
  if (gchunk < max_chunk) max_chunk = gchunk;
  if (max_chunk < 1) max_chunk = 1;
  if (async_out) *async_out = async;
  return max_chunk;
}
int bg_max_fused_steps(const bg_handle* h) { return h ? bg_chunk_limit(h, nullptr) : 0; }
uint64_t bg_state_bytes(const bg_handle* h) { return h ? h->bytes : 0; }

static uint32_t* bg_prod_latest(bg_handle* h) { return h->d_prod[(h->refill_seq + 1) & 1]; }

static BgDev bg_dev_view(bg_handle* h, const uint32_t* view) {
  BgDev d = h->dev;
  d.prod_view = view;
  return d;
}

static int bg_refill_pieces(bg_handle* h, int n);
static int bg_wait_refill(bg_handle* h, hipStream_t s, int back) {
  long i = h->refill_seq - 1 - back;
  if (i < 0) return 0;
  if (back == 0 && h->piece_next < h->pieces.size()) { int rc = bg_refill_pieces(h, 1 << 30); if (rc) return rc; }
  BG_HIP(hipStreamWaitEvent(s, h->ev_refill[i & 1], 0));
  return 0;
}

static int bg_refill_pieces(bg_handle* h, int n) {
  const BgDev& d = h->piece_dev;
  hipStream_t s = h->side;
  while (n-- > 0 && h->piece_next < h->pieces.size()) {
    const bg_handle::RefillPiece& pc = h->pieces[h->piece_next++];
    const BgPart pt{pc.part, pc.nparts};
    hipEvent_t ea = nullptr, eb = nullptr;
    bg_ev_pair(h, h->ev_refill_t, ea, eb);
    const dim3 g(pc.grid), b(BG_BLOCK);
    if (ea) {
      if (pc.kind == 0) hipExtLaunchKernelGGL(bg_refill_deck_kernel, g, b, 0, s, ea, eb, 0, d, pt, pc.cursor, pc.max_made);
      else if (pc.kind == 1) hipExtLaunchKernelGGL(bg_refill_seedring_kernel, g, b, 0, s, ea, eb, 0, d, pt);
      else if (pc.kind == 2) hipExtLaunchKernelGGL(bg_refill_gblk_kernel, g, b, 0, s, ea, eb, 0, d, pt);
      else hipExtLaunchKernelGGL(bg_refill_shop_kernel, g, b, 0, s, ea, eb, 0, d, pt);
    } else {
      if (pc.kind == 0) hipLaunchKernelGGL(bg_refill_deck_kernel, g, b, 0, s, d, pt, pc.cursor, pc.max_made);
      else if (pc.kind == 1) hipLaunchKernelGGL(bg_refill_seedring_kernel, g, b, 0, s, d, pt);
      else if (pc.kind == 2) hipLaunchKernelGGL(bg_refill_gblk_kernel, g, b, 0, s, d, pt);
      else hipLaunchKernelGGL(bg_refill_shop_kernel, g, b, 0, s, d, pt);
    }
    BG_HIP(hipGetLastError());
    if (h->piece_next == h->pieces.size()) BG_HIP(hipEventRecord(h->ev_refill[(h->refill_seq - 1) & 1], s));
  }
  return 0;
}

static int bg_refill_on(bg_handle* h, hipStream_t s, int steps_hint = -1, bool sliced = false) {
  BgDev d = h->dev;
  d.prod_in = bg_prod_latest(h);
  d.prod_out = h->d_prod[h->refill_seq & 1];
  d.prod_view = nullptr;
  bg_ev_begin(h, h->ev_refill_t, s);
  hipLaunchKernelGGL(bg_refill_zero_kernel, dim3(1), dim3(BG_BLOCK), 0, s, d);
  hipLaunchKernelGGL(bg_refill_scan_kernel, dim3(bg_grid(h)), dim3(BG_BLOCK), 0, s, d);
  if (sliced && s == h->side) {
    bg_ev_end(h, h->ev_refill_t, s);
    BG_HIP(hipGetLastError());
    h->pieces.clear(); h->piece_next = 0; h->piece_dev = d;
    static const int grid[4] = {512, 768, 1024, 1024};
    std::vector<bg_handle::RefillPiece> q[4];
    for (int pass = 0; pass < h->deck_passes; pass++)
      for (int p = 0; p < h->piece_parts[0]; p++)
        q[0].push_back({0, (uint32_t)p, (uint32_t)h->piece_parts[0], grid[0], (uint32_t)(8 + pass * h->piece_parts[0] + p), pass + 1 < h->deck_passes ? 6u : 0u});
    for (int kind = 1; kind < 4; kind++)
      for (int p = 0; p < h->piece_parts[kind]; p++) q[kind].push_back({kind, (uint32_t)p, (uint32_t)h->piece_parts[kind], grid[kind], 0u, 0u});
    static const int order[4] = {3, 0, 2, 1};
    size_t taken[4] = {0, 0, 0, 0};
    for (;;) {
      int best = -1; double share = 0.0;
      for (const int k : order) {
        if (taken[k] >= q[k].size()) continue;
        const double sh = (double)(q[k].size() - taken[k]) / (double)q[k].size();
        if (best < 0 || sh > share + 1e-9) { best = k; share = sh; }
      }
      if (best < 0) break;
      h->pieces.push_back(q[best][taken[best]++]);
    }
    h->refill_seq++;
    h->steps_since_refill = 0;
    return 0;
  }
  const BgPart whole{0u, 1u};
  const int full = 4096;
  int dense = full;
  if (steps_hint >= 0 && steps_hint < 372) { dense = (int)((long)full * (steps_hint + 24) / 372); if (dense < 512) dense = 512; if (dense > full) dense = full; }
  hipLaunchKernelGGL(bg_refill_deck_kernel, dim3(dense), dim3(BG_BLOCK), 0, s, d, whole, 4u, 0u);
  hipLaunchKernelGGL(bg_refill_seedring_kernel, dim3(dense), dim3(BG_BLOCK), 0, s, d, whole);
  hipLaunchKernelGGL(bg_refill_gblk_kernel, dim3(dense), dim3(BG_BLOCK), 0, s, d, whole);
  hipLaunchKernelGGL(bg_refill_shop_kernel, dim3(dense), dim3(BG_BLOCK), 0, s, d, whole);
  bg_ev_end(h, h->ev_refill_t, s);
  BG_HIP(hipGetLastError());
  BG_HIP(hipEventRecord(h->ev_refill[h->refill_seq & 1], s));
  h->refill_seq++;
  h->steps_since_refill = 0;
  return 0;
}

int bg_refill(bg_handle* h, void* stream) {
  if (!h) return BG_E_ARG;
  BG_GUARD(h);
  hipStream_t s = (hipStream_t)stream;
  int rc = bg_wait_refill(h, s, 0);
  if (rc) return rc;
  rc = bg_refill_on(h, s);
  h->view_min = h->refill_seq - 1;
  return rc;
}

int bg_check(bg_handle* h, void* stream) {
  if (!h) return BG_E_ARG;
  BG_GUARD(h);
  uint32_t w = 0;
  BG_HIP(hipMemcpyAsync(&w, h->dev.err, sizeof(w), hipMemcpyDeviceToHost, (hipStream_t)stream));
  BG_HIP(hipStreamSynchronize((hipStream_t)stream));
  if (w) {
    char buf[256];
    snprintf(buf, sizeof(buf), "device invariant violated: error word 0x%x (1 global-stream underflow, 2 shop block, 4 deck ring, 8 shop ring, 16 a bounded wait inside the step engine expired)", w);
    h->err = buf;
    return BG_E_INTERNAL;
  }
  return 0;
}

int bg_seed(bg_handle* h, const int64_t* seeds_host, const uint8_t* mask_host, int reseed_global, void* stream) {
  if (!h || !seeds_host) return BG_E_ARG;
  BG_GUARD(h);
  hipStream_t s = (hipStream_t)stream;
  size_t N = h->dev.N;
  BG_HIP(hipMemcpyAsync(h->d_seeds, seeds_host, N * sizeof(int64_t), hipMemcpyHostToDevice, s));
  if (mask_host) BG_HIP(hipMemcpyAsync(h->d_mask, mask_host, N, hipMemcpyHostToDevice, s));
  { int rcw = bg_wait_refill(h, s, 0); if (rcw) return rcw; }
  BgDev dseed = bg_dev_view(h, bg_prod_latest(h));
  dseed.prod_in = h->d_prod[0]; dseed.prod_out = h->d_prod[1];
  hipLaunchKernelGGL(bg_seed_kernel, dim3(bg_grid(h)), dim3(BG_BLOCK), 0, s, dseed, (const int64_t*)h->d_seeds,
                     mask_host ? (const uint8_t*)h->d_mask : (const uint8_t*)nullptr, reseed_global);
  BG_HIP(hipGetLastError());
  BG_HIP(hipStreamSynchronize(s));
  h->seeded = true;
  int rc = bg_refill(h, stream);
  if (rc) return rc;
  return bg_refill(h, stream);
}

static int bg_require_seeded(bg_handle* h) {
  if (!h) return BG_E_ARG;
  if (!h->seeded) { h->err = "bg_seed must be called before reset/step (streams are unseeded)"; return BG_E_ARG; }
  return 0;
}

static ObsPtrs bg_obs(const bg_obs_ptrs* o) {
  ObsPtrs p;
  memset(&p, 0, sizeof(p));
  if (o) memcpy(&p, o, sizeof(*o));
  return p;
}
static InfoPtrs bg_info(const bg_info_ptrs* o) {
  InfoPtrs p;
  if (o) memcpy(&p, o, sizeof(p)); else memset(&p, 0, sizeof(p));
  return p;
}

static void bg_obs_advance(ObsPtrs& o, size_t off) {
  if (o.hand) o.hand += off * 8; if (o.hand_size) o.hand_size += off; if (o.deck_size) o.deck_size += off;
  if (o.selected_cards) o.selected_cards += off * 8; if (o.chips_scored) o.chips_scored += off;
  if (o.round_chips_scored) o.round_chips_scored += off; if (o.progress_ratio) o.progress_ratio += off;
  if (o.mult) o.mult += off; if (o.chips_needed) o.chips_needed += off; if (o.money) o.money += off;
  if (o.ante) o.ante += off; if (o.round) o.round += off; if (o.hands_left) o.hands_left += off;
  if (o.discards_left) o.discards_left += off; if (o.joker_count) o.joker_count += off;
  if (o.joker_ids) o.joker_ids += off * 10; if (o.joker_slots) o.joker_slots += off;
  if (o.consumable_count) o.consumable_count += off; if (o.consumables) o.consumables += off * 5;
  if (o.consumable_slots) o.consumable_slots += off; if (o.shop_items) o.shop_items += off * 10;
  if (o.shop_costs) o.shop_costs += off * 10; if (o.shop_rerolls) o.shop_rerolls += off;
  if (o.hand_levels) o.hand_levels += off * 12; if (o.phase) o.phase += off; if (o.action_mask) o.action_mask += off * 60;
  if (o.hands_played) o.hands_played += off; if (o.best_hand_this_ante) o.best_hand_this_ante += off;
  if (o.boss_blind_active) o.boss_blind_active += off; if (o.boss_blind_type) o.boss_blind_type += off;
  if (o.face_down_cards) o.face_down_cards += off * 8;
}
static void bg_info_advance(InfoPtrs& p, size_t off) {
  if (p.final_score) p.final_score += off; if (p.error) p.error += off; if (p.flags) p.flags += off; if (p.aux) p.aux += off;
  if (p.hand_type) p.hand_type += off; if (p.cards_played) p.cards_played += off; if (p.reward_terms) p.reward_terms += off * 8;
  if (p.score_breakdown) p.score_breakdown += off * 8;
}

int bg_reset(bg_handle* h, const uint8_t* mask_dev, const bg_obs_ptrs* obs, void* stream) {
  int rc = bg_require_seeded(h);
  if (rc) return rc;
  BG_GUARD(h);
  rc = bg_wait_refill(h, (hipStream_t)stream, 0);
  if (rc) return rc;
  if (h->dev.cstate) hipLaunchKernelGGL(bg_reset_kernel<true>, dim3(bg_grid(h)), dim3(BG_BLOCK), 0, (hipStream_t)stream, bg_dev_view(h, bg_prod_latest(h)), mask_dev, bg_obs(obs));
  else hipLaunchKernelGGL(bg_reset_kernel<false>, dim3(bg_grid(h)), dim3(BG_BLOCK), 0, (hipStream_t)stream, bg_dev_view(h, bg_prod_latest(h)), mask_dev, bg_obs(obs));
  BG_HIP(hipGetLastError());
  return bg_refill(h, stream);
}

static int bg_engine_waves(int T) {
  if (T <= 192) return BG_ENG_NW - 1;
  return BG_ENG_NW;
}
static void bg_engine_launch(bg_handle* h, const BgDev& dv, const EngineArgs& a0, bool hash, bool info, hipStream_t st, hipEvent_t ev_a = nullptr, hipEvent_t ev_b = nullptr) {
  const bool cards = h->dev.cstate != nullptr;
  EngineArgs a = a0;
  if (h->engine == 3 && a.obs.rows && !info && !a.reward && !a.term && !a.actions_out) {
    a.th_play = a.th_other = 0x7fffffffu; a.th_more = 0u;
    const int cfg = h->e3_cfg ? h->e3_cfg : (h->dev.N <= 16384 ? 113 : (h->dev.N <= 32768 ? 213 : 413));
    int epw = 64;
    if (cfg == 113) {
      epw = h->e3_epw ? h->e3_epw : 64;
      if (!h->e3_epw) { while (epw > 16 && (h->dev.N + epw - 1) / epw < 256) epw >>= 1; }
      a.epw = (uint32_t)epw;
    }
#define BG_E3K(HV, CV, NOWV, KSV, NSVV, AV) do { \
      const dim3 g_((NOWV * KSV == 1) ? (h->dev.N + epw - 1) / epw : (h->dev.N + NOWV * KSV * 64 - 1) / (NOWV * KSV * 64)), b_((NOWV + NSVV) * BG_BLOCK); \
      if (ev_a) hipExtLaunchKernelGGL((bg_engine3_kernel<HV, CV, NOWV, KSV, NSVV, AV>), g_, b_, 0, st, ev_a, ev_b, 0, dv, a); \
      else hipLaunchKernelGGL((bg_engine3_kernel<HV, CV, NOWV, KSV, NSVV, AV>), g_, b_, 0, st, dv, a); } while (0)
#define BG_E3(NOWV, KSV, NSVV) do { \
      if (a.actions_in) { if (cards) BG_E3K(false, true, NOWV, KSV, NSVV, true); else BG_E3K(false, false, NOWV, KSV, NSVV, true); } \
      else if (hash && cards) BG_E3K(true, true, NOWV, KSV, NSVV, false); else if (hash) BG_E3K(true, false, NOWV, KSV, NSVV, false); \
      else if (cards) BG_E3K(false, true, NOWV, KSV, NSVV, false); else BG_E3K(false, false, NOWV, KSV, NSVV, false); } while (0)
    switch (cfg) {
      case 113: BG_E3(1, 1, 3); break;
      case 213: BG_E3(2, 1, 3); break;
      default: BG_E3(4, 1, 3); break;
    }
#undef BG_E3
#undef BG_E3K
    return;
  }
  a.n_waves = (uint32_t)bg_engine_waves((int)a.T);
  if (a.T == 1 && a.actions_in) a.th_play = a.th_other = 1u;
  a.copier = a.obs.rows ? (uint32_t)(h->eng_copiers > 0 ? h->eng_copiers : (a.T == 1 ? 2 : 1)) : 0u;
  if (a.copier && a.n_waves > BG_ENG_NW - a.copier) a.n_waves = BG_ENG_NW - a.copier;
  if (a.n_waves < BG_ENG_NW && a.serve_mask == BG_ENG_SMASK_DEFAULT)
    a.serve_mask = a.n_waves <= BG_ENG_NSV ? (1u << a.n_waves) - 1u : ((1u << BG_ENG_NSV) - 1u) << (a.n_waves - BG_ENG_NSV);
  if ((a.serve_mask & ((1u << a.n_waves) - 1u)) == 0u)
    a.serve_mask = a.n_waves <= BG_ENG_NSV ? (1u << a.n_waves) - 1u : ((1u << BG_ENG_NSV) - 1u) << (a.n_waves - BG_ENG_NSV);
  const dim3 g((h->dev.N + BG_ENG_NE - 1) / BG_ENG_NE), b(BG_ENG_NW * BG_BLOCK);
#define BG_ENG(HASHV, CARDSV, INFOV) do { \
    if (ev_a) hipExtLaunchKernelGGL((bg_engine_kernel<HASHV, CARDSV, INFOV>), g, b, 0, st, ev_a, ev_b, 0, dv, a); \
    else hipLaunchKernelGGL((bg_engine_kernel<HASHV, CARDSV, INFOV>), g, b, 0, st, dv, a); } while (0)
  if (info) { if (cards) BG_ENG(false, true, true); else BG_ENG(false, false, true); }
  else if (hash && cards) BG_ENG(true, true, false);
  else if (hash) BG_ENG(true, false, false);
  else if (cards) BG_ENG(false, true, false);
  else BG_ENG(false, false, false);
#undef BG_ENG
}

static void bg_engine_queues(const bg_handle* h, EngineArgs& a) { a.th_run = a.th_play = a.th_other = 64u; a.th_part = 1u; a.th_more = 0u; a.serve_mask = h->eng_smask; }

static int bg_step_budget(const bg_handle* h) {
  const int ring = h->dev.KD < h->dev.KS - 1 ? h->dev.KD : h->dev.KS - 1;
  int lim = 3 * ring;
  const int g = bg_gsteps(h->dev.flags, h->dev.KG - 1);
  if (g < lim) lim = g;
  return lim < 1 ? 1 : lim;
}

static int bg_step_impl(bg_handle* h, int K, const int32_t* actions_dev, const bg_obs_ptrs* obs, int obs_stride_steps, double* reward_dev,
                        uint8_t* terminated_dev, uint8_t* truncated_dev, const bg_info_ptrs* info, void* stream,
                        uint8_t* rows_dev = nullptr, uint64_t row_stride = 0) {
  int rc = bg_require_seeded(h);
  if (rc) return rc;
  BG_GUARD(h);
  if (!actions_dev || K <= 0) return BG_E_ARG;
  hipStream_t st = (hipStream_t)stream;
  const int budget = bg_step_budget(h);
  const size_t N = (size_t)h->dev.N;
  int done = 0;
  while (done < K) {
    if (h->steps_since_refill >= budget) { rc = bg_refill(h, stream); if (rc) return rc; }
    int chunk = K - done;
    if (chunk > budget - h->steps_since_refill) chunk = budget - h->steps_since_refill;
    rc = bg_wait_refill(h, st, 0);
    if (rc) return rc;
    const BgDev dv = bg_dev_view(h, bg_prod_latest(h));
    hipEvent_t ev_a = nullptr, ev_b = nullptr;
    bg_ev_pair(h, h->ev_step_t, ev_a, ev_b);
    {
      EngineArgs ea;
      memset(&ea, 0, sizeof(ea));
      ea.T = chunk; ea.actions_in = actions_dev + (size_t)done * N;
      ea.obs = bg_obs(obs); ea.obs_stride_steps = obs_stride_steps;
      const size_t off = obs_stride_steps ? (size_t)done * N : 0;
      if (off) bg_obs_advance(ea.obs, off);
      if (rows_dev) { ea.obs.rows = rows_dev; ea.obs.row_stride = (uint32_t)row_stride; }
      ea.reward = reward_dev ? reward_dev + off : nullptr; ea.term = terminated_dev ? terminated_dev + off : nullptr;
      ea.trunc = truncated_dev ? truncated_dev + off : nullptr;
      ea.info = bg_info(info);
      if (off) bg_info_advance(ea.info, off);
      bg_engine_queues(h, ea);
      ea.autoreset = (h->dev.flags & BG_FLAG_AUTORESET) ? 1u : 0u;
      bg_engine_launch(h, dv, ea, false, true, st, ev_a, ev_b);
    }
    BG_HIP(hipGetLastError());
    h->steps_since_refill += chunk;
    done += chunk;
  }
  return 0;
}

int bg_step(bg_handle* h, const int32_t* actions_dev, const bg_obs_ptrs* obs, double* reward_dev, uint8_t* terminated_dev,
            uint8_t* truncated_dev, const bg_info_ptrs* info, void* stream) {
  return bg_step_impl(h, 1, actions_dev, obs, 0, reward_dev, terminated_dev, truncated_dev, info, stream);
}

int bg_step_many(bg_handle* h, int K, const int32_t* actions_dev, const bg_obs_ptrs* obs, int obs_stride_steps, double* reward_dev,
                 uint8_t* terminated_dev, uint8_t* truncated_dev, const bg_info_ptrs* info, void* stream) {
  return bg_step_impl(h, K, actions_dev, obs, obs_stride_steps, reward_dev, terminated_dev, truncated_dev, info, stream);
}

static const char* bg_rows_args(const void* rows_dev, uint64_t row_stride_bytes) {
  if (!rows_dev || row_stride_bytes < BG_ROW_BYTES || (row_stride_bytes & 15) || ((uintptr_t)rows_dev & 15) || row_stride_bytes > 0xffffffffull)
    return "rows_dev must be 16-byte aligned and row_stride_bytes a multiple of 16, >= BG_ROW_BYTES";
  return nullptr;
}

int bg_step_rows(bg_handle* h, const int32_t* actions_dev, uint8_t* rows_dev, uint64_t row_stride_bytes, double* reward_dev,
                 uint8_t* terminated_dev, uint8_t* truncated_dev, const bg_info_ptrs* info, void* stream) {
  if (!h) return BG_E_ARG;
  if (const char* m = bg_rows_args(rows_dev, row_stride_bytes)) { h->err = std::string("bg_step_rows: ") + m; return BG_E_ARG; }
  return bg_step_impl(h, 1, actions_dev, nullptr, 0, reward_dev, terminated_dev, truncated_dev, info, stream, rows_dev, row_stride_bytes);
}

int bg_observe_rows(bg_handle* h, uint8_t* rows_dev, uint64_t row_stride_bytes, void* stream) {
  if (!h) return BG_E_ARG;
  if (const char* m = bg_rows_args(rows_dev, row_stride_bytes)) { h->err = std::string("bg_observe_rows: ") + m; return BG_E_ARG; }
  BG_GUARD(h);
  ObsPtrs o = bg_obs(nullptr);
  o.rows = rows_dev; o.row_stride = (uint32_t)row_stride_bytes;
  { const int rcw = bg_wait_refill(h, (hipStream_t)stream, 0); if (rcw) return rcw; }
  hipLaunchKernelGGL(bg_observe_kernel, dim3(bg_grid(h)), dim3(BG_BLOCK), 0, (hipStream_t)stream, bg_dev_view(h, bg_prod_latest(h)), o);
  BG_HIP(hipGetLastError());
  return 0;
}

int bg_observe(bg_handle* h, const bg_obs_ptrs* obs, void* stream) {
  if (!h) return BG_E_ARG;
  BG_GUARD(h);
  { const int rcw = bg_wait_refill(h, (hipStream_t)stream, 0); if (rcw) return rcw; }
  hipLaunchKernelGGL(bg_observe_kernel, dim3(bg_grid(h)), dim3(BG_BLOCK), 0, (hipStream_t)stream, bg_dev_view(h, bg_prod_latest(h)), bg_obs(obs));
  BG_HIP(hipGetLastError());
  return 0;
}

static int bg_rollout_impl(bg_handle* h, int T, int policy, uint64_t policy_seed, uint64_t env_index0, uint64_t t0,
                           const bg_obs_ptrs* obs, uint8_t* rows_dev, size_t row_stride, int obs_stride_steps,
                           double* reward_dev, uint8_t* terminated_dev, int32_t* actions_out_dev,
                           bg_rollout_stats* stats_dev, void* stream, const int32_t* actions_in_dev = nullptr, bool autoreset = true) {
  int rc = bg_require_seeded(h);
  if (rc) return rc;
  BG_GUARD(h);
  if (T <= 0) return BG_E_ARG;
  bool async = false;
  const int max_chunk = bg_chunk_limit(h, &async);
  if (async && h->steps_since_refill > max_chunk) { rc = bg_refill(h, stream); if (rc) return rc; }
  int done = 0;
  while (done < T) {
    int chunk = T - done < max_chunk ? T - done : max_chunk;
    ObsPtrs o = bg_obs(obs);
    size_t off = obs_stride_steps ? (size_t)done * (size_t)h->dev.N : 0;
    if (rows_dev) { o.rows = rows_dev + off * row_stride; o.row_stride = (uint32_t)row_stride; }
    if (off) bg_obs_advance(o, off);
    if (h->profiling) h->rollout_steps.push_back(chunk);
    const bool need = h->steps_since_refill + chunk > max_chunk;
    const long s0 = h->refill_seq;
    const bool refill_after = need && async && s0 >= 1 && s0 - 1 >= h->view_min;
    const bool pieces_after = !need && async && h->piece_next < h->pieces.size();
    if (pieces_after) BG_HIP(hipEventRecord(h->ev_rollout, (hipStream_t)stream));
    if (need && async) {
      BG_HIP(hipEventRecord(h->ev_rollout, (hipStream_t)stream));
      if (h->piece_next < h->pieces.size()) {
        BG_HIP(hipStreamWaitEvent(h->side, h->ev_rollout, 0));
        rc = bg_refill_pieces(h, 1 << 30);
        if (rc) return rc;
      }
      if (!refill_after) {
        BG_HIP(hipStreamWaitEvent(h->side, h->ev_rollout, 0));
        rc = bg_wait_refill(h, h->side, 0);
        if (rc) return rc;
        rc = bg_refill_on(h, h->side, h->steps_since_refill + chunk);
        if (rc) return rc;
      }
    } else if (need) {
      rc = bg_refill(h, stream);
      if (rc) return rc;
    }
    long vi = h->refill_seq - 1;
    if (refill_after) vi = s0 - 1;
    else if (async && vi - 1 >= h->view_min) vi--;
    if (vi >= 0 && vi > h->refill_done) {
      if (hipEventQuery(h->ev_refill[vi & 1]) == hipSuccess) h->refill_done = vi;
      else BG_HIP(hipStreamWaitEvent((hipStream_t)stream, h->ev_refill[vi & 1], 0));
    }
    const uint32_t* view = vi >= 0 ? h->d_prod[vi & 1] : bg_prod_latest(h);
    hipEvent_t ev_a = nullptr, ev_b = nullptr;
    bg_ev_pair(h, h->ev_rollout_t, ev_a, ev_b);
    BgDev dv = bg_dev_view(h, view);
    {
      const bool hash = (policy & BG_POLICY_HASH_OBS) != 0;
      const int pol = policy & 0xff;
      double* rw = reward_dev ? reward_dev + off : nullptr;
      uint8_t* tm = terminated_dev ? terminated_dev + off : nullptr;
      int32_t* ac = actions_out_dev ? actions_out_dev + off : nullptr;
      hipStream_t st = (hipStream_t)stream;
      uint64_t tt = t0 + (uint64_t)done;
      EngineArgs ea;
      memset(&ea, 0, sizeof(ea));
      ea.T = chunk; ea.policy = pol; ea.policy_seed = policy_seed; ea.env_index0 = env_index0; ea.t0 = tt;
      ea.obs = o; ea.obs_stride_steps = obs_stride_steps; ea.reward = rw; ea.term = tm; ea.actions_out = ac; ea.stats = stats_dev;
      bg_engine_queues(h, ea); ea.autoreset = autoreset ? 1u : 0u;
      if (actions_in_dev) ea.actions_in = actions_in_dev + (size_t)done * (size_t)h->dev.N;
      if (h->gworld > 0 && rows_dev && h->engine == 3 && done + chunk == T) {
        ea.gpeer = h->d_gpeer;
        ea.gworld = (uint32_t)h->gworld; ea.grank = (uint32_t)h->grank;
      }
      bg_engine_launch(h, dv, ea, hash, false, st, ev_a, ev_b);
    }
    BG_HIP(hipGetLastError());
    if (refill_after) {
      BG_HIP(hipStreamWaitEvent(h->side, h->ev_rollout, 0));
      rc = bg_wait_refill(h, h->side, 0);
      if (rc) return rc;
      const bool sliced = h->refill_sliced != 0 && 2 * chunk <= max_chunk;
      rc = bg_refill_on(h, h->side, h->steps_since_refill + chunk, sliced);
      if (rc) return rc;
    }
    if ((refill_after || pieces_after) && h->piece_next < h->pieces.size()) {
      const int u = h->steps_since_refill;
      int m = 1 + (max_chunk - (u + chunk)) / (chunk > 0 ? chunk : 1);
      if (m < 1) m = 1;
      const int pending = (int)(h->pieces.size() - h->piece_next), extra = refill_after ? 1 : 0;
      const int np = (pending + extra + m - 1) / m - extra;
      if (np > 0) {
        if (!refill_after) BG_HIP(hipStreamWaitEvent(h->side, h->ev_rollout, 0));
        rc = bg_refill_pieces(h, np);
        if (rc) return rc;
      }
    }
    h->steps_since_refill += chunk;
    done += chunk;
  }
  return 0;
}

int bg_set_gather_peers(bg_handle* h, void* const* bufs, int world, int rank) {
  if (!h) return BG_E_ARG;
  if (world == 0) { h->gworld = 0; return 0; }
  if (!bufs || world < 1 || world > 8 || rank < 0 || rank >= world) { h->err = "bg_set_gather_peers: world must be 1..8, rank inside it, bufs the world gather buffers"; return BG_E_ARG; }
  if (h->engine != 3) { h->err = "bg_set_gather_peers: only bg_engine3.h's packed-record rollouts write gather buffers (BG_ENGINE=3)"; return BG_E_ARG; }
  BG_GUARD(h);
  for (int g = 0; g < world; g++) {
    if (!bufs[g] || ((uintptr_t)bufs[g] & 15)) { h->err = "bg_set_gather_peers: every gather buffer must be a 16-byte aligned device pointer"; return BG_E_ARG; }
    hipPointerAttribute_t at;
    memset(&at, 0, sizeof(at));
    if (hipPointerGetAttributes(&at, bufs[g]) != hipSuccess) { (void)hipGetLastError(); h->err = "bg_set_gather_peers: a gather buffer is not a device allocation this process knows"; return BG_E_ARG; }
    if (at.device != h->device_id) {
      int can = 0;
      if (hipDeviceCanAccessPeer(&can, h->device_id, at.device) != hipSuccess || !can) { (void)hipGetLastError(); h->err = "bg_set_gather_peers: this device cannot access a peer's gather buffer (no peer access between the two devices)"; return BG_E_ARG; }
      const hipError_t pe = hipDeviceEnablePeerAccess(at.device, 0);
      if (pe != hipSuccess && pe != hipErrorPeerAccessAlreadyEnabled) { (void)hipGetLastError(); h->err = std::string("bg_set_gather_peers: hipDeviceEnablePeerAccess: ") + hipGetErrorString(pe); return BG_E_HIP; }
      (void)hipGetLastError();
    }
  }
  for (int g = 0; g < 8; g++) h->gpeer[g] = g < world ? (uint8_t*)bufs[g] : nullptr;
  if (!h->d_gpeer) BG_HIP(hipMalloc((void**)&h->d_gpeer, sizeof(h->gpeer)));
  BG_HIP(hipDeviceSynchronize());
  BG_HIP(hipMemcpy(h->d_gpeer, h->gpeer, sizeof(h->gpeer), hipMemcpyHostToDevice));
  h->gworld = world; h->grank = rank;
  return 0;
}

int bg_rollout(bg_handle* h, int T, int policy, uint64_t policy_seed, uint64_t env_index0, uint64_t t0,
               const bg_obs_ptrs* obs, int obs_stride_steps, double* reward_dev, uint8_t* terminated_dev,
               int32_t* actions_out_dev, bg_rollout_stats* stats_dev, void* stream) {
  return bg_rollout_impl(h, T, policy, policy_seed, env_index0, t0, obs, nullptr, 0, obs_stride_steps, reward_dev,
                         terminated_dev, actions_out_dev, stats_dev, stream);
}

int bg_rollout_rows(bg_handle* h, int T, int policy, uint64_t policy_seed, uint64_t env_index0, uint64_t t0,
                    uint8_t* rows_dev, uint64_t row_stride_bytes, int rows_stride_steps, bg_rollout_stats* stats_dev,
                    void* stream) {
  if (!h) return BG_E_ARG;
  if ((uint64_t)h->dev.N * (uint64_t)bg_max_fused_steps(h) > 0xffffffffull) { h->err = "bg_rollout_rows: more than 2**32 records per launch (envs x fused steps)"; return BG_E_ARG; }
  if (!rows_dev || row_stride_bytes < BG_ROW_BYTES || (row_stride_bytes & 15) || ((uintptr_t)rows_dev & 15) || row_stride_bytes > 0xffffffffull) {
    h->err = "bg_rollout_rows: rows_dev must be 16-byte aligned and row_stride_bytes a multiple of 16, >= BG_ROW_BYTES";
    return BG_E_ARG;
  }
  return bg_rollout_impl(h, T, policy, policy_seed, env_index0, t0, nullptr, rows_dev, (size_t)row_stride_bytes,
                         rows_stride_steps, nullptr, nullptr, nullptr, stats_dev, stream);
}

int bg_step_many_rows(bg_handle* h, int K, const int32_t* actions_dev, uint8_t* rows_dev, uint64_t row_stride_bytes,
                      int rows_stride_steps, bg_rollout_stats* stats_dev, void* stream) {
  if (!h) return BG_E_ARG;
  if (!actions_dev || K <= 0) { h->err = "bg_step_many_rows: actions_dev must be a device pointer to [K, N] int32 actions, K > 0"; return BG_E_ARG; }
  if ((uint64_t)h->dev.N * (uint64_t)bg_max_fused_steps(h) > 0xffffffffull) { h->err = "bg_step_many_rows: more than 2**32 records per launch (envs x fused steps)"; return BG_E_ARG; }
  if (const char* m = bg_rows_args(rows_dev, row_stride_bytes)) { h->err = std::string("bg_step_many_rows: ") + m; return BG_E_ARG; }
  return bg_rollout_impl(h, K, 0, 0, 0, 0, nullptr, rows_dev, (size_t)row_stride_bytes, rows_stride_steps, nullptr, nullptr, nullptr, stats_dev,
                         stream, actions_dev, (h->dev.flags & BG_FLAG_AUTORESET) != 0);
}

__global__ __launch_bounds__(BG_BLOCK) void bg_inject_cards_kernel(BgDev d, const uint16_t* __restrict__ cs, const uint8_t* __restrict__ mask_in, int apply_now) {
  int env = blockIdx.x * BG_BLOCK + threadIdx.x;
  if (env >= d.N) return;
  if (mask_in && !mask_in[env]) return;
  const uint4* src = (const uint4*)(cs + (size_t)env * 56);
#pragma unroll
  for (int k = 0; k < BG_NCST; k++) {
    uint4 v = src[k];
    d.ctmpl[(size_t)k * d.N + env] = v;
    if (apply_now) d.cstate[(size_t)k * d.N + env] = v;
  }
}

int bg_inject_cards(bg_handle* h, const uint8_t* enh_host, const uint8_t* edition_host, const uint8_t* seal_host,
                    const uint8_t* mask_host, int apply_now, void* stream) {
  if (!h) return BG_E_ARG;
  if (!h->dev.cstate) { h->err = "bg_inject_cards: the handle was created without BG_FLAG_CARD_STATES"; return BG_E_ARG; }
  BG_GUARD(h);
  hipStream_t s = (hipStream_t)stream;
  const size_t N = h->dev.N;
  std::vector<uint16_t> packed(N * 56, 0);
  for (size_t i = 0; i < N; i++)
    for (int c = 0; c < 52; c++) {
      const uint32_t e = enh_host ? enh_host[i * 52 + c] : 0, d = edition_host ? edition_host[i * 52 + c] : 0, sl = seal_host ? seal_host[i * 52 + c] : 0;
      if (e > 15 || d > 15 || sl > 15) { h->err = "bg_inject_cards: state codes are 0..15"; return BG_E_ARG; }
      packed[i * 56 + c] = (uint16_t)(e | (d << 4) | (sl << 8));
    }
  uint16_t* dcs = nullptr;
  BG_HIP(hipMalloc(&dcs, packed.size() * sizeof(uint16_t)));
  BG_HIP(hipMemcpyAsync(dcs, packed.data(), packed.size() * sizeof(uint16_t), hipMemcpyHostToDevice, s));
  if (mask_host) BG_HIP(hipMemcpyAsync(h->d_mask, mask_host, N, hipMemcpyHostToDevice, s));
  hipLaunchKernelGGL(bg_inject_cards_kernel, dim3(bg_grid(h)), dim3(BG_BLOCK), 0, s, h->dev, (const uint16_t*)dcs,
                     mask_host ? (const uint8_t*)h->d_mask : (const uint8_t*)nullptr, apply_now);
  BG_HIP(hipGetLastError());
  BG_HIP(hipStreamSynchronize(s));
  BG_HIP(hipFree(dcs));
  return 0;
}

int bg_inject(bg_handle* h, const int32_t* jokers_host, const int32_t* njokers_host, const int64_t* money_host,
              const int32_t* ante_host, const uint8_t* levels_host, const uint8_t* mask_host, int apply_now, void* stream) {
  if (!h) return BG_E_ARG;
  BG_GUARD(h);
  hipStream_t s = (hipStream_t)stream;
  size_t N = h->dev.N;
  for (size_t i = 0; i < N; i++) {
    if (mask_host && !mask_host[i]) continue;
    uint4& t0 = h->h_tmpl[i];
    uint4& t1 = h->h_tmpl[N + i];
    uint32_t fl = t0.y >> 24;
    uint32_t j4 = t0.y & 0xffu, nj = (t0.y >> 8) & 0xffu, an = (t0.y >> 16) & 0xffu;
    if (jokers_host && njokers_host) {
      int n = njokers_host[i];
      if (n < 0 || n > 5) { h->err = "bg_inject: njokers must be in [0,5]"; return BG_E_ARG; }
      uint32_t lo = 0; j4 = 0;
      for (int k = 0; k < n; k++) {
        int id = jokers_host[i * 5 + k];
        if (id < 1 || id > 150) { h->err = "bg_inject: joker id out of range"; return BG_E_ARG; }
        if (k < 4) lo |= (uint32_t)id << (8 * k); else j4 = (uint32_t)id;
      }
      t0.x = lo; nj = (uint32_t)n; fl |= 0x80u;
    }
    if (money_host) { if (money_host[i] >= 0) { t0.z = (uint32_t)(int32_t)money_host[i]; fl |= 0x40u; } else fl &= ~0x40u; }
    if (ante_host) {
      if (ante_host[i] > 255 || (h->h_cap[i] > 0 && ante_host[i] > (int)h->h_cap[i])) { h->err = "bg_inject: template ante above the env's curriculum cap (max_ante)"; return BG_E_ARG; }
      if (ante_host[i] > 0) { an = (uint32_t)ante_host[i] & 0xffu; fl |= 0x20u; } else fl &= ~0x20u;
    }
    if (levels_host) {
      uint64_t lv = 0; bool any = false;
      for (int k = 0; k < 12; k++) { int l = levels_host[i * 12 + k]; if (l) any = true; if (l < 1) l = 1; if (l > 15) l = 15; lv |= (uint64_t)l << (4 * k); }
      if (any) { t1.x = (uint32_t)lv; t1.y = (uint32_t)(lv >> 32); fl |= 0x10u; } else fl &= ~0x10u;
    }
    t0.y = j4 | (nj << 8) | (an << 16) | (fl << 24);
  }
  BG_HIP(hipMemcpyAsync(h->dev.tmpl, h->h_tmpl.data(), BG_NTMPL * N * sizeof(uint4), hipMemcpyHostToDevice, s));
  if (apply_now) {
    if (mask_host) BG_HIP(hipMemcpyAsync(h->d_mask, mask_host, N, hipMemcpyHostToDevice, s));
    { const int rcw = bg_wait_refill(h, s, 0); if (rcw) return rcw; }
    hipLaunchKernelGGL(bg_inject_kernel, dim3(bg_grid(h)), dim3(BG_BLOCK), 0, s, bg_dev_view(h, bg_prod_latest(h)),
                       mask_host ? (const uint8_t*)h->d_mask : (const uint8_t*)nullptr);
    BG_HIP(hipGetLastError());
  }
  BG_HIP(hipStreamSynchronize(s));
  return 0;
}

int bg_inject_consumables(bg_handle* h, const int32_t* ids_host, const int32_t* n_host, const uint8_t* mask_host, int apply_now,
                          void* stream) {
  if (!h || !ids_host || !n_host) return BG_E_ARG;
  BG_GUARD(h);
  hipStream_t s = (hipStream_t)stream;
  size_t N = h->dev.N;
  for (size_t i = 0; i < N; i++) {
    if (mask_host && !mask_host[i]) continue;
    int n = n_host[i];
    if (n < 0) { h->h_tmpl[N + i].z = 0; continue; }
    if (n > 2) { h->err = "bg_inject_consumables: an env holds at most consumable_slots = 2"; return BG_E_ARG; }
    uint32_t v = 0x80000000u | (uint32_t)n;
    for (int k = 0; k < n; k++) {
      int id = ids_host[i * 2 + k];
      bool planet = id >= 30 && id <= 41, other = (id >= 1 && id <= 22) || (id >= 50 && id <= 67);
      if (!planet && !other) { h->err = "bg_inject_consumables: ids are 1-22 (tarots), 30-41 (planets), 50-67 (spectrals)"; return BG_E_ARG; }
      if (other && !h->dev.cstate) { h->err = "bg_inject_consumables: tarot / spectral cards need BG_FLAG_CARD_STATES"; return BG_E_ARG; }
      v |= (uint32_t)id << (8 * (k + 1));
    }
    h->h_tmpl[N + i].z = v;
  }
  BG_HIP(hipMemcpyAsync(h->dev.tmpl, h->h_tmpl.data(), BG_NTMPL * N * sizeof(uint4), hipMemcpyHostToDevice, s));
  if (apply_now) {
    if (mask_host) BG_HIP(hipMemcpyAsync(h->d_mask, mask_host, N, hipMemcpyHostToDevice, s));
    { const int rcw = bg_wait_refill(h, s, 0); if (rcw) return rcw; }
    hipLaunchKernelGGL(bg_inject_kernel, dim3(bg_grid(h)), dim3(BG_BLOCK), 0, s, bg_dev_view(h, bg_prod_latest(h)),
                       mask_host ? (const uint8_t*)h->d_mask : (const uint8_t*)nullptr);
    BG_HIP(hipGetLastError());
  }
  BG_HIP(hipStreamSynchronize(s));
  return 0;
}

struct BgSlice { void* base; size_t rows; size_t elem; };
static void bg_slices(bg_handle* h, std::vector<BgSlice>& v) {
  BgDev& d = h->dev;
  v.push_back({d.hot, BG_NHOT, 16}); v.push_back({d.deck, BG_NDECK, 16}); v.push_back({d.cold, BG_NCOLD, 16});
  v.push_back({d.tmpl, BG_NTMPL, 16}); v.push_back({d.ndeck, (size_t)d.KD * BG_NDECK, 16});
  v.push_back({d.gblk, 1, (size_t)d.KG * BG_MTS * 4}); v.push_back({d.sblk, 1, (size_t)d.KS * BG_SLOT_WORDS * 4}); v.push_back({d.sovf, 1, (size_t)BG_MTS * 4});
  v.push_back({d.deckmt, 1, (size_t)BG_MTS * 4}); v.push_back({d.shopgenmt, 1, (size_t)BG_MTS * 4});
  v.push_back({d.sseed, 1, BG_SSEED * 4}); v.push_back({d.smeta, 1, 4});
  v.push_back({bg_prod_latest(h), 1, 4});
  if (d.cstate) { v.push_back({d.cstate, BG_NCST, 16}); v.push_back({d.ctmpl, BG_NCST, 16}); v.push_back({d.cardmt, 1, (size_t)BG_MTS * 4}); v.push_back({d.sealmt, 1, (size_t)BG_MTS * 4}); }
}
uint64_t bg_state_blob_bytes(const bg_handle* h) {
  if (!h) return 0;
  std::vector<BgSlice> v;
  bg_slices(const_cast<bg_handle*>(h), v);
  uint64_t b = 16;
  for (auto& s : v) b += s.rows * s.elem;
  return b;
}
#define BG_BLOB_MAGIC 0x42474d58u
#define BG_BLOB_VERSION 7u
static int bg_blob_args(bg_handle* h, const char* fn, int env_index, const void* blob, uint64_t blob_bytes) {
  if (!h) return BG_E_ARG;
  char buf[200];
  if (!blob) { h->err = std::string(fn) + ": null blob"; return BG_E_ARG; }
  if (env_index < 0 || env_index >= h->dev.N) { snprintf(buf, sizeof(buf), "%s: env_index %d out of range [0, %d)", fn, env_index, h->dev.N); h->err = buf; return BG_E_ARG; }
  const uint64_t want = bg_state_blob_bytes(h);
  if (blob_bytes < want) {
    snprintf(buf, sizeof(buf), "%s: blob of %llu bytes, this handle's blobs are %llu bytes (ring depths and card-state flag decide the size)", fn,
             (unsigned long long)blob_bytes, (unsigned long long)want);
    h->err = buf; return BG_E_ARG;
  }
  return 0;
}
int bg_get_state(bg_handle* h, int env_index, void* blob_host, uint64_t blob_bytes) {
  int rc = bg_blob_args(h, "bg_get_state", env_index, blob_host, blob_bytes);
  if (rc) return rc;
  BG_GUARD(h);
  rc = bg_refill_pieces(h, 1 << 30);
  if (rc) return rc;
  BG_HIP(hipDeviceSynchronize());
  uint8_t* out = (uint8_t*)blob_host;
  uint32_t hdr[4] = {BG_BLOB_MAGIC, BG_BLOB_VERSION, (uint32_t)h->dev.KG | (h->dev.cstate ? 0x10000u : 0u), (uint32_t)h->dev.KS | ((uint32_t)h->dev.KD << 16)};
  memcpy(out, hdr, 16); out += 16;
  std::vector<BgSlice> v;
  bg_slices(h, v);
  size_t N = h->dev.N;
  for (auto& s : v) {
    BG_HIP(hipMemcpy2D(out, s.elem, (uint8_t*)s.base + (size_t)env_index * s.elem, N * s.elem, s.elem, s.rows, hipMemcpyDeviceToHost));
    out += s.rows * s.elem;
  }
  return 0;
}
int bg_set_state(bg_handle* h, int env_index, const void* blob_host, uint64_t blob_bytes) {
  int rc = bg_blob_args(h, "bg_set_state", env_index, blob_host, blob_bytes);
  if (rc) return rc;
  BG_GUARD(h);
  const uint8_t* in = (const uint8_t*)blob_host;
  uint32_t hdr[4];
  memcpy(hdr, in, 16); in += 16;
  char buf[200];
  if (hdr[0] != BG_BLOB_MAGIC) { h->err = "bg_set_state: not a state blob (bad magic)"; return BG_E_ARG; }
  if (hdr[1] != BG_BLOB_VERSION) { snprintf(buf, sizeof(buf), "bg_set_state: blob version %u, this library reads version %u", hdr[1], BG_BLOB_VERSION); h->err = buf; return BG_E_ARG; }
  if (hdr[2] != ((uint32_t)h->dev.KG | (h->dev.cstate ? 0x10000u : 0u)) || hdr[3] != ((uint32_t)h->dev.KS | ((uint32_t)h->dev.KD << 16))) {
    snprintf(buf, sizeof(buf), "bg_set_state: the blob was saved with ring depths %u/%u/%u%s, this handle has %d/%d/%d%s", hdr[2] & 0xffffu, hdr[3] & 0xffffu, hdr[3] >> 16,
             (hdr[2] & 0x10000u) ? " + card states" : "", h->dev.KG, h->dev.KS, h->dev.KD, h->dev.cstate ? " + card states" : "");
    h->err = buf; return BG_E_ARG;
  }
  rc = bg_refill_pieces(h, 1 << 30);
  if (rc) return rc;
  BG_HIP(hipDeviceSynchronize());
  std::vector<BgSlice> v;
  bg_slices(h, v);
  size_t N = h->dev.N;
  for (auto& s : v) {
    BG_HIP(hipMemcpy2D((uint8_t*)s.base + (size_t)env_index * s.elem, N * s.elem, in, s.elem, s.elem, s.rows, hipMemcpyHostToDevice));
    if (s.base == (void*)h->dev.tmpl)
      for (size_t r = 0; r < s.rows; r++) memcpy(&h->h_tmpl[r * N + (size_t)env_index], in + r * s.elem, sizeof(uint4));
    if (s.base == (void*)h->dev.hot) { uint4 c7; memcpy(&c7, in + 7 * s.elem, sizeof(uint4)); h->h_cap[env_index] = (uint8_t)((c7.w >> 16) & 0xffu); }
    in += s.rows * s.elem;
  }
  {
    uint32_t w = 0;
    BG_HIP(hipMemcpy(&w, bg_prod_latest(h) + env_index, 4, hipMemcpyDeviceToHost));
    BG_HIP(hipMemcpy(h->d_prod[0] + env_index, &w, 4, hipMemcpyHostToDevice));
    BG_HIP(hipMemcpy(h->d_prod[1] + env_index, &w, 4, hipMemcpyHostToDevice));
  }
  h->seeded = true;
  h->steps_since_refill = 1 << 30;
  return 0;
}

int bg_inject_deck(bg_handle* h, const uint8_t* decks_host, const uint8_t* mask_host, void* stream) {
  if (!h || !decks_host) return BG_E_ARG;
  BG_GUARD(h);
  hipStream_t s = (hipStream_t)stream;
  const size_t N = h->dev.N;
  std::vector<uint8_t> packed(N * 64, 0);
  for (size_t i = 0; i < N; i++) {
    if (mask_host && !mask_host[i]) continue;
    uint64_t seen = 0;
    for (int c = 0; c < 52; c++) {
      const uint8_t v = decks_host[i * 52 + c];
      if (v >= 52 || ((seen >> v) & 1ull)) { h->err = "bg_inject_deck: every deck must be a permutation of the 52 card codes (rank-2)*4+suit"; return BG_E_ARG; }
      seen |= 1ull << v;
      packed[i * 64 + c] = v;
    }
  }
  uint4* dd = nullptr;
  BG_HIP(hipMalloc((void**)&dd, packed.size()));
  BG_HIP(hipMemcpyAsync(dd, packed.data(), packed.size(), hipMemcpyHostToDevice, s));
  if (mask_host) BG_HIP(hipMemcpyAsync(h->d_mask, mask_host, N, hipMemcpyHostToDevice, s));
  { int rcw = bg_wait_refill(h, s, 0); if (rcw) { (void)hipFree(dd); return rcw; } }
  hipLaunchKernelGGL(bg_inject_deck_kernel, dim3(bg_grid(h)), dim3(BG_BLOCK), 0, s, h->dev, (const uint4*)dd,
                     mask_host ? (const uint8_t*)h->d_mask : (const uint8_t*)nullptr);
  BG_HIP(hipGetLastError());
  BG_HIP(hipStreamSynchronize(s));
  BG_HIP(hipFree(dd));
  return 0;
}

int bg_set_max_ante(bg_handle* h, int max_ante, const int32_t* per_env_host, const uint8_t* mask_host, void* stream) {
  if (!h) return BG_E_ARG;
  BG_GUARD(h);
  hipStream_t s = (hipStream_t)stream;
  const size_t N = h->dev.N;
  if (!per_env_host && (max_ante < 0 || max_ante > 255)) { h->err = "bg_set_max_ante: the cap must be in [0, 255] (0 = none)"; return BG_E_ARG; }
  int32_t* dc = nullptr;
  for (size_t i = 0; i < N; i++) {
    if (mask_host && !mask_host[i]) continue;
    const int c = per_env_host ? per_env_host[i] : max_ante;
    if (c < 0 || c > 255) { h->err = "bg_set_max_ante: every cap must be in [0, 255] (0 = none)"; return BG_E_ARG; }
    const uint32_t ty = h->h_tmpl[i].y;
    if (c > 0 && ((ty >> 24) & 0x20u) && (int)((ty >> 16) & 0xffu) > c) { h->err = "bg_set_max_ante: a cap below the env's template ante (bg_inject)"; return BG_E_ARG; }
  }
  for (size_t i = 0; i < N; i++)
    if (!mask_host || mask_host[i]) h->h_cap[i] = (uint8_t)(per_env_host ? per_env_host[i] : max_ante);
  if (per_env_host) {
    BG_HIP(hipMalloc((void**)&dc, N * sizeof(int32_t)));
    BG_HIP(hipMemcpyAsync(dc, per_env_host, N * sizeof(int32_t), hipMemcpyHostToDevice, s));
  }
  if (mask_host) BG_HIP(hipMemcpyAsync(h->d_mask, mask_host, N, hipMemcpyHostToDevice, s));
  hipLaunchKernelGGL(bg_set_cap_kernel, dim3(bg_grid(h)), dim3(BG_BLOCK), 0, s, h->dev, (const int32_t*)dc, max_ante,
                     mask_host ? (const uint8_t*)h->d_mask : (const uint8_t*)nullptr);
  BG_HIP(hipGetLastError());
  BG_HIP(hipStreamSynchronize(s));
  if (dc) BG_HIP(hipFree(dc));
  if (!per_env_host && !mask_host) h->dev.max_ante = max_ante;
  return 0;
}

#define BG_HIP0(call)                                                                                  \
  do {                                                                                                 \
    hipError_t _e = (call);                                                                            \
    if (_e != hipSuccess) {                                                                            \
      g_create_err = std::string(#call) + ": " + hipGetErrorString(_e);                                \
      return BG_E_HIP;                                                                                 \
    }                                                                                                  \
  } while (0)

typedef uint32_t bg_cp_u32x4 __attribute__((ext_vector_type(4)));
__global__ __launch_bounds__(256) void bg_stream_copy_kernel(const bg_cp_u32x4* __restrict__ src, bg_cp_u32x4* __restrict__ dst, size_t n16) {
  const size_t i = (size_t)blockIdx.x * 256 * 4 + threadIdx.x;
  bg_cp_u32x4 v[4];
#pragma unroll
  for (int k = 0; k < 4; k++) if (i + (size_t)k * 256 < n16) v[k] = __builtin_nontemporal_load(&src[i + (size_t)k * 256]);
#pragma unroll
  for (int k = 0; k < 4; k++) if (i + (size_t)k * 256 < n16) __builtin_nontemporal_store(v[k], &dst[i + (size_t)k * 256]);
}
int bg_bench_copy(const void* src_dev, void* dst_dev, uint64_t bytes, int iters, double* gbps_out, void* stream) {
  if (!src_dev || !dst_dev || !gbps_out || bytes < 16 || iters < 1 || ((uintptr_t)src_dev & 15) || ((uintptr_t)dst_dev & 15)) { g_create_err = "bg_bench_copy: bad arguments"; return BG_E_ARG; }
  hipStream_t s = (hipStream_t)stream;
  const size_t n16 = bytes / 16;
  const unsigned grid = (unsigned)((n16 + 1023) / 1024);
  hipEvent_t a, b;
  BG_HIP0(hipEventCreate(&a)); BG_HIP0(hipEventCreate(&b));
  for (int i = 0; i < 2; i++) hipLaunchKernelGGL(bg_stream_copy_kernel, dim3(grid), dim3(256), 0, s, (const bg_cp_u32x4*)src_dev, (bg_cp_u32x4*)dst_dev, n16);
  BG_HIP0(hipEventRecord(a, s));
  for (int i = 0; i < iters; i++) hipLaunchKernelGGL(bg_stream_copy_kernel, dim3(grid), dim3(256), 0, s, (const bg_cp_u32x4*)src_dev, (bg_cp_u32x4*)dst_dev, n16);
  BG_HIP0(hipEventRecord(b, s));
  BG_HIP0(hipGetLastError());
  BG_HIP0(hipEventSynchronize(b));
  float ms = 0;
  BG_HIP0(hipEventElapsedTime(&ms, a, b));
  (void)hipEventDestroy(a); (void)hipEventDestroy(b);
  *gbps_out = ms > 0 ? 2.0 * (double)(n16 * 16) * iters / (ms * 1e-3) / 1e9 : 0.0;
  return 0;
}

__global__ __launch_bounds__(256) void bg_stream_fill_kernel(uint4* __restrict__ dst, size_t n16, uint32_t seed) {
  const size_t i = (size_t)blockIdx.x * 256 + threadIdx.x;
  if (i < n16) dst[i] = make_uint4(seed, (uint32_t)i, 0u, seed ^ (uint32_t)i);
}
int bg_bench_fill(void* dst_dev, uint64_t bytes, int iters, double* gbps_out, void* stream) {
  if (!dst_dev || !gbps_out || bytes < 16 || iters < 1 || ((uintptr_t)dst_dev & 15)) { g_create_err = "bg_bench_fill: bad arguments"; return BG_E_ARG; }
  hipStream_t s = (hipStream_t)stream;
  const size_t n16 = bytes / 16;
  const unsigned grid = (unsigned)((n16 + 255) / 256);
  hipEvent_t a, b;
  BG_HIP0(hipEventCreate(&a)); BG_HIP0(hipEventCreate(&b));
  for (int i = 0; i < 2; i++) hipLaunchKernelGGL(bg_stream_fill_kernel, dim3(grid), dim3(256), 0, s, (uint4*)dst_dev, n16, 0u);
  BG_HIP0(hipEventRecord(a, s));
  for (int i = 0; i < iters; i++) hipLaunchKernelGGL(bg_stream_fill_kernel, dim3(grid), dim3(256), 0, s, (uint4*)dst_dev, n16, (uint32_t)i + 1u);
  BG_HIP0(hipEventRecord(b, s));
  BG_HIP0(hipGetLastError());
  BG_HIP0(hipEventSynchronize(b));
  float ms = 0;
  BG_HIP0(hipEventElapsedTime(&ms, a, b));
  (void)hipEventDestroy(a); (void)hipEventDestroy(b);
  *gbps_out = ms > 0 ? (double)(n16 * 16) * iters / (ms * 1e-3) / 1e9 : 0.0;
  return 0;
}

struct BgOpTimer {
  hipEvent_t a = nullptr, b = nullptr;
  bool on = false;
  int begin(float* out, hipStream_t s) { on = out != nullptr; if (!on) return 0; BG_HIP0(hipEventCreate(&a)); BG_HIP0(hipEventCreate(&b)); BG_HIP0(hipEventRecord(a, s)); return 0; }
  void mark(hipStream_t s) { if (on) (void)hipEventRecord(b, s); }
  int end(float* out) { if (!on) return 0; BG_HIP0(hipEventSynchronize(b)); BG_HIP0(hipEventElapsedTime(out, a, b)); (void)hipEventDestroy(a); (void)hipEventDestroy(b); return 0; }
};

int bg_classify_batch_ex(const uint8_t* cards_dev, const uint8_t* n_dev, uint8_t* hand_type_dev, int64_t m, int lanes_per_case,
                         float* kernel_ms_out, void* stream) {
  if (!cards_dev || !n_dev || !hand_type_dev || m < 0 || ((uintptr_t)cards_dev & 7) || (lanes_per_case != 1 && lanes_per_case != 8)) {
    g_create_err = "bg_classify_batch: bad arguments (cards_dev must be 8-byte aligned, lanes_per_case 1 or 8)"; return BG_E_ARG;
  }
  if (kernel_ms_out) *kernel_ms_out = 0.f;
  if (m == 0) return 0;
  hipStream_t s = (hipStream_t)stream;
  BgOpTimer tm;
  int rc = tm.begin(kernel_ms_out, s);
  if (rc) return rc;
  if (lanes_per_case == 1)
    hipLaunchKernelGGL(bg_classify_batch_kernel, dim3((unsigned)((m + BG_BLOCK - 1) / BG_BLOCK)), dim3(BG_BLOCK), 0, s, cards_dev, n_dev, hand_type_dev, (long long)m);
  else
    hipLaunchKernelGGL(bg_classify_batch_l8_kernel, dim3((unsigned)((m * 8 + BG_BLOCK - 1) / BG_BLOCK)), dim3(BG_BLOCK), 0, s, cards_dev, n_dev, hand_type_dev, (long long)m);
  tm.mark(s);
  BG_HIP0(hipGetLastError());
  return tm.end(kernel_ms_out);
}
int bg_classify_batch(const uint8_t* cards_dev, const uint8_t* n_dev, uint8_t* hand_type_dev, int64_t m, void* stream) {
  return bg_classify_batch_ex(cards_dev, n_dev, hand_type_dev, m, 1, nullptr, stream);
}

int bg_encode_cols(int layout) { const int d = bg_enc_cols(layout); return d > 0 ? d : BG_E_ARG; }

int bg_encode_rows(const uint8_t* rows_dev, uint64_t row_stride_bytes, int64_t m, int layout, int out_dtype, void* out_dev,
                   uint64_t out_stride_elems, float* kernel_ms_out, void* stream) {
  const int D = bg_enc_cols(layout);
  const uint64_t es = out_dtype == BG_ENC_F32 ? 4u : 2u;
  const char* bad = nullptr;
  if (D < 0) bad = "layout must be BG_ENC_PRODUCED, BG_ENC_FIXED or BG_ENC_EXTRACTOR";
  else if (out_dtype != BG_ENC_F32 && out_dtype != BG_ENC_BF16) bad = "out_dtype must be BG_ENC_F32 or BG_ENC_BF16";
  else if (m < 0 || m > (int64_t)BG_ENC_RECS * 0x7fffffffll) bad = "m out of range";
  else if (const char* r = bg_rows_args(rows_dev, row_stride_bytes)) bad = r;
  else if (!out_dev || ((uintptr_t)out_dev & (es - 1))) bad = "out_dev must be a device pointer aligned to its element type";
  else if (out_stride_elems < (uint64_t)D || out_stride_elems > 0xffffffffull) bad = "out_stride_elems must be >= the layout's column count";
  if (bad) { g_create_err = std::string("bg_encode_rows: ") + bad; return BG_E_ARG; }
  if (kernel_ms_out) *kernel_ms_out = 0.f;
  if (m == 0) return 0;
  const bool base16 = ((uintptr_t)out_dev & 15) == 0;
  const int st = base16 && (out_stride_elems * es) % 16 == 0 ? BG_ENC_ST_ROWS : base16 && out_stride_elems == (uint64_t)D ? BG_ENC_ST_FLAT : BG_ENC_ST_ELEM;
  const unsigned grid = (unsigned)((m + BG_ENC_RECS - 1) / BG_ENC_RECS);
  hipStream_t s = (hipStream_t)stream;
  BgOpTimer tm;
  int rc = tm.begin(kernel_ms_out, s);
  if (rc) return rc;
#define BG_ENC_GO(L, T) bg_encode_launch<L, T>(st, grid, s, rows_dev, row_stride_bytes, (long long)m, out_dev, out_stride_elems)
  if (out_dtype == BG_ENC_F32) { if (layout == BG_ENC_PRODUCED) BG_ENC_GO(BG_ENC_PRODUCED, BG_ENC_F32); else if (layout == BG_ENC_FIXED) BG_ENC_GO(BG_ENC_FIXED, BG_ENC_F32); else BG_ENC_GO(BG_ENC_EXTRACTOR, BG_ENC_F32); }
  else { if (layout == BG_ENC_PRODUCED) BG_ENC_GO(BG_ENC_PRODUCED, BG_ENC_BF16); else if (layout == BG_ENC_FIXED) BG_ENC_GO(BG_ENC_FIXED, BG_ENC_BF16); else BG_ENC_GO(BG_ENC_EXTRACTOR, BG_ENC_BF16); }
#undef BG_ENC_GO
  tm.mark(s);
  BG_HIP0(hipGetLastError());
  return tm.end(kernel_ms_out);
}

static const char* bg_scan_args(const uint8_t* rows_dev, uint64_t row_stride_bytes, int K, int64_t N) {
  if (K < 0 || N < 0 || N > (int64_t)BG_GAE_ENVS * 0x7fffffffll) return "K / N out of range";
  return bg_rows_args(rows_dev, row_stride_bytes);
}

int bg_gae_rows_ex(const uint8_t* rows_dev, uint64_t row_stride_bytes, int K, int64_t N, const float* values_dev, const float* last_values_dev,
                   double gamma, double gae_lambda, float* advantages_dev, float* returns_dev, const double* rewards_dev, float* kernel_ms_out, void* stream) {
  const char* const who = rewards_dev ? "bg_gae_rows_ex: " : "bg_gae_rows: ";
  const char* bad = bg_scan_args(rows_dev, row_stride_bytes, K, N);
  if (!bad && (!values_dev || !last_values_dev || !advantages_dev)) bad = "values_dev, last_values_dev and advantages_dev must be device pointers";
  else if (!bad && (((uintptr_t)values_dev | (uintptr_t)last_values_dev | (uintptr_t)advantages_dev | (uintptr_t)returns_dev) & 3)) bad = "float arrays must be 4-byte aligned";
  else if (!bad && ((uintptr_t)rewards_dev & 7)) bad = "rewards_dev must be 8-byte aligned";
  else if (!bad && (advantages_dev == values_dev || returns_dev == values_dev || (returns_dev && returns_dev == advantages_dev))) bad = "advantages_dev / returns_dev must not be the same pointer as values_dev or as each other";
  else if (!bad && rewards_dev && ((const void*)rewards_dev == (const void*)advantages_dev || (const void*)rewards_dev == (const void*)returns_dev)) bad = "advantages_dev / returns_dev must not be the same pointer as rewards_dev";
  if (bad) { g_create_err = std::string(who) + bad; return BG_E_ARG; }
  if (kernel_ms_out) *kernel_ms_out = 0.f;
  if (K == 0 || N == 0) return 0;
  const unsigned grid = (unsigned)((N + BG_GAE_ENVS - 1) / BG_GAE_ENVS);
  const float g = bg_gae_g(gamma), gl = bg_gae_gl(gamma, gae_lambda);
  hipStream_t s = (hipStream_t)stream;
  BgOpTimer tm;
  int rc = tm.begin(kernel_ms_out, s);
  if (rc) return rc;
#define BG_GAE_GO(R, W) hipLaunchKernelGGL((bg_gae_kernel<R, W>), dim3(grid), dim3(BG_GAE_BLOCK), 0, s, rows_dev, row_stride_bytes, K, (long long)N, values_dev, last_values_dev, g, gl, advantages_dev, returns_dev, rewards_dev)
  if (returns_dev) { if (rewards_dev) BG_GAE_GO(true, true); else BG_GAE_GO(true, false); }
  else { if (rewards_dev) BG_GAE_GO(false, true); else BG_GAE_GO(false, false); }
#undef BG_GAE_GO
  tm.mark(s);
  BG_HIP0(hipGetLastError());
  return tm.end(kernel_ms_out);
}
int bg_gae_rows(const uint8_t* rows_dev, uint64_t row_stride_bytes, int K, int64_t N, const float* values_dev, const float* last_values_dev,
                double gamma, double gae_lambda, float* advantages_dev, float* returns_dev, float* kernel_ms_out, void* stream) {
  return bg_gae_rows_ex(rows_dev, row_stride_bytes, K, N, values_dev, last_values_dev, gamma, gae_lambda, advantages_dev, returns_dev, nullptr, kernel_ms_out, stream);
}

int bg_episode_stats_rows(const uint8_t* rows_dev, uint64_t row_stride_bytes, int K, int64_t N, double* ep_return_carry_dev, int32_t* ep_len_carry_dev,
                          double* ep_return_dev, int32_t* ep_len_dev, float* kernel_ms_out, void* stream) {
  const char* bad = bg_scan_args(rows_dev, row_stride_bytes, K, N);
  if (!bad && (!ep_return_carry_dev || !ep_len_carry_dev)) bad = "ep_return_carry_dev and ep_len_carry_dev must be device pointers";
  else if (!bad && ((((uintptr_t)ep_return_carry_dev | (uintptr_t)ep_return_dev) & 7) || (((uintptr_t)ep_len_carry_dev | (uintptr_t)ep_len_dev) & 3))) bad = "float64 arrays must be 8-byte aligned, int32 arrays 4-byte aligned";
  else if (!bad && (ep_return_dev == ep_return_carry_dev || ep_len_dev == ep_len_carry_dev)) bad = "ep_return_dev / ep_len_dev must not be the same pointer as their carry";
  if (bad) { g_create_err = std::string("bg_episode_stats_rows: ") + bad; return BG_E_ARG; }
  if (kernel_ms_out) *kernel_ms_out = 0.f;
  if (K == 0 || N == 0) return 0;
  const unsigned grid = (unsigned)((N + BG_GAE_ENVS - 1) / BG_GAE_ENVS);
  hipStream_t s = (hipStream_t)stream;
  BgOpTimer tm;
// ... 248 lines not shown
```

balatro_gym_amd/vec_env.py:

```python
from __future__ import annotations

import ctypes as C
import random as _pyrandom
from typing import Dict, Optional, Sequence

import numpy as np
import torch

from . import _native as nat

_TORCH_DT = {"int8": torch.int8, "int16": torch.int16, "int32": torch.int32, "int64": torch.int64,
             "float32": torch.float32, "float64": torch.float64, "uint8": torch.uint8}


def _align(n: int, a: int = 256) -> int:
    return (n + a - 1) // a * a


def _check_out_tensor(name: str, t: Optional[torch.Tensor], dtype: torch.dtype, device: torch.device, n: int, rows: Optional[int]):
    if t is None:
        return
    if t.dtype != dtype or t.device != device or not t.is_contiguous():
        raise ValueError(f"{name} must be a contiguous {dtype} tensor on {device} (got {t.dtype} on {t.device}"
                         f"{'' if t.is_contiguous() else ', not contiguous'})")
# ... 154 lines not shown

    def set_gather_peers(self, buffers: Sequence[Optional[torch.Tensor]], rank: int) -> None:
        world = len(buffers)
        if world == 0:
            self._check(self._L.bg_set_gather_peers(self._h, None, 0, 0), "bg_set_gather_peers")
            self._gather_keep = None
            return
        for b in buffers:
            if b.dtype != torch.uint8 or tuple(b.shape) != (world, self.num_envs, nat.ROW_BYTES) or not b.is_contiguous():
                raise ValueError(f"every gather buffer must be a contiguous uint8 [{world}, {self.num_envs}, {nat.ROW_BYTES}] tensor")
        arr = (C.c_void_p * world)(*[b.data_ptr() for b in buffers])
        self._check(self._L.bg_set_gather_peers(self._h, C.cast(arr, C.c_void_p), world, int(rank)), "bg_set_gather_peers")
        self._gather_keep = list(buffers)

    def obs_flat_bytes(self, n: int) -> int:
        return int(n) * self._rowbuf.row_stride if self._rowbuf is not None else obs_flat_bytes(int(n))

    def state_bytes(self) -> int:
        return int(self._L.bg_state_bytes(self._h))

    @property
    def max_fused_steps(self) -> int:
        return int(self._L.bg_max_fused_steps(self._h))

    def close(self):
        if getattr(self, "_h", None) is not None and self._h:
            torch.cuda.synchronize(self.device)
            self._L.bg_destroy(self._h)
            self._h = None

    def __del__(self):
        try:
            self.close()
        except Exception:
            pass

    def seed(self, seeds: Optional[Sequence[int]] = None, mask: Optional[Sequence[bool]] = None, reseed_global: bool = True):
        n = self.num_envs
        if seeds is None:
            seeds = [_pyrandom.randint(0, 2 ** 32 - 1) for _ in range(n)]
        arr = np.ascontiguousarray(np.asarray(seeds, dtype=np.int64))
        if arr.shape != (n,):
            raise ValueError(f"seeds must have shape ({n},)")
        m = None if mask is None else np.ascontiguousarray(np.asarray(mask, dtype=np.uint8))
        with torch.cuda.device(self.device):
            self._check(self._L.bg_seed(self._h, arr.ctypes.data_as(C.c_void_p),
                                        None if m is None else m.ctypes.data_as(C.c_void_p),
                                        1 if reseed_global else 0, self._stream()), "bg_seed")
        self.seeds = arr.copy() if mask is None else np.where(np.asarray(mask, bool), arr, getattr(self, "seeds", arr))

    def reset(self, *, seed: Optional[Sequence[int]] = None, mask: Optional[torch.Tensor] = None):
        if seed is not None:
            hm = None if mask is None else mask.to("cpu").numpy().astype(np.uint8)
            self.seed(seed, hm, reseed_global=False)
        mptr = None
        if mask is not None:
            mask = mask.to(device=self.device, dtype=torch.uint8).contiguous()
            mptr = C.c_void_p(mask.data_ptr())
        with torch.cuda.device(self.device):
            if self._rowbuf is not None:
                self._check(self._L.bg_reset(self._h, mptr, None, self._stream()), "bg_reset")
                self._check(self._L.bg_observe_rows(self._h, self._rows_args[0], self._rows_args[1], self._stream()), "bg_observe_rows")
            else:
                self._check(self._L.bg_reset(self._h, mptr, C.byref(self._obs.ptrs), self._stream()), "bg_reset")
        return self.obs

    def step(self, actions: torch.Tensor):
        if actions.numel() != self.num_envs:
            raise ValueError(f"actions must hold {self.num_envs} elements, one per env (got {tuple(actions.shape)})")
        if actions.dtype != torch.int32 or actions.device != self.device or not actions.is_contiguous():
            actions = actions.to(device=self.device, dtype=torch.int32).contiguous()
        a = self._step_args
        if self._rowbuf is not None:
            r = self._rows_args
            rc = self._L.bg_step_rows(self._h, actions.data_ptr(), r[0], r[1], a[1], a[2], a[3], a[4],
                                      torch.cuda.current_stream(self.device).cuda_stream)
            if rc != 0:
                self._check(rc, "bg_step_rows")
            return self._row_tensors, self.reward, self.terminated, self.truncated, self.info
        rc = self._L.bg_step(self._h, actions.data_ptr(), a[0], a[1], a[2], a[3], a[4],
                             torch.cuda.current_stream(self.device).cuda_stream)
        if rc != 0:
            self._check(rc, "bg_step")
        return self._obs.tensors, self.reward, self.terminated, self.truncated, self.info

    def step_many(self, actions: torch.Tensor, obs_buffers: Optional["ObsBuffers"] = None, reward: Optional[torch.Tensor] = None,
                  terminated: Optional[torch.Tensor] = None):
        if actions.dtype != torch.int32 or actions.device != self.device or not actions.is_contiguous():
            actions = actions.to(device=self.device, dtype=torch.int32).contiguous()
        if actions.dim() != 2 or actions.shape[1] != self.num_envs:
            raise ValueError(f"actions must be [K, {self.num_envs}]")
        K = int(actions.shape[0])
        if isinstance(obs_buffers, RowBuffers):
            if K < 1:
                raise ValueError(f"actions must be [K, {self.num_envs}] with K >= 1")
            if obs_buffers.steps < K and obs_buffers.steps > 1:
                raise ValueError("obs_buffers has fewer rows than steps")
            if reward is not None or terminated is not None:
                raise ValueError("packed records already carry reward / action / terminated")
            if obs_buffers.n != self.num_envs or obs_buffers.rows.device != self.device:
                raise ValueError(f"obs_buffers must hold records of {self.num_envs} envs on {self.device}")
            self._stats.zero_()
            rc = self._L.bg_step_many_rows(
                self._h, K, C.c_void_p(actions.data_ptr()), C.c_void_p(obs_buffers.rows.data_ptr()), C.c_uint64(obs_buffers.row_stride),
                1 if obs_buffers.steps > 1 else 0, C.c_void_p(self._stats.data_ptr()), self._stream())
            if rc != 0:
                self._check(rc, "bg_step_many_rows")
            if self._rowbuf is not None:
                self.observe()
            return obs_buffers.tensors, obs_buffers.reward, obs_buffers.terminated, None, None
        keep = obs_buffers is not None and obs_buffers.steps > 1
        if keep and obs_buffers.steps < K:
            raise ValueError("obs_buffers has fewer rows than steps")
        if not keep and (reward is not None or terminated is not None):
            raise ValueError("reward / terminated tensors need per-step obs_buffers: without them the live tensors hold the last call's values")
        _check_out_tensor("reward", reward, torch.float64, self.device, self.num_envs, K)
        _check_out_tensor("terminated", terminated, torch.uint8, self.device, self.num_envs, K)
        ob = obs_buffers if keep else self._obs
        rw = reward if keep else self.reward
        tm = terminated if keep else self.terminated
        with torch.cuda.device(self.device):
            self._check(self._L.bg_step_many(
                self._h, K, C.c_void_p(actions.data_ptr()), C.byref(ob.ptrs), 1 if keep else 0, None if rw is None else C.c_void_p(rw.data_ptr()),
                None if tm is None else C.c_void_p(tm.data_ptr()), None if keep else C.c_void_p(self.truncated.data_ptr()),
                None if keep else C.byref(self._info_ptrs), self._stream()), "bg_step_many")
        if self._rowbuf is not None:
            self.observe()
            if not keep:
                return self._row_tensors, rw, tm, self.truncated, self.info
        if keep:
            return ob.tensors, rw, tm, None, None
        return ob.tensors, rw, tm, self.truncated, self.info

    def observe(self):
        with torch.cuda.device(self.device):
            if self._rowbuf is not None:
                self._check(self._L.bg_observe_rows(self._h, self._rows_args[0], self._rows_args[1], self._stream()), "bg_observe_rows")
            else:
                self._check(self._L.bg_observe(self._h, C.byref(self._obs.ptrs), self._stream()), "bg_observe")
        return self.obs

    def rollout(self, steps: int, policy: int = nat.POLICY_UNIFORM, policy_seed: int = 0, env_index0: int = 0,
                t0: int = 0, obs_buffers: Optional[ObsBuffers] = None, reward: Optional[torch.Tensor] = None,
                terminated: Optional[torch.Tensor] = None, actions: Optional[torch.Tensor] = None,
                zero_stats: bool = True):
        if isinstance(obs_buffers, RowBuffers):
            if obs_buffers.steps < steps and obs_buffers.steps > 1:
                raise ValueError("obs_buffers has fewer rows than steps")
            if reward is not None or terminated is not None or actions is not None:
                raise ValueError("packed records already carry reward / action / terminated")
            if zero_stats:
                self._stats.zero_()
            rc = self._L.bg_rollout_rows(
                self._h, int(steps), int(policy), C.c_uint64(policy_seed), C.c_uint64(env_index0), C.c_uint64(t0),
                C.c_void_p(obs_buffers.rows.data_ptr()), C.c_uint64(getattr(obs_buffers, "row_stride", nat.ROW_BYTES)), 1 if obs_buffers.steps > 1 else 0,
                C.c_void_p(self._stats.data_ptr()), self._stream())
            if rc != 0:
                self._check(rc, "bg_rollout_rows")
            if self._rowbuf is not None:
                self.observe()
            return self._stats
        ob = obs_buffers or self._obs
        stride = 1 if (obs_buffers is not None and obs_buffers.steps > 1) else 0
        if stride and obs_buffers.steps < steps:
            raise ValueError("obs_buffers has fewer rows than steps")
        if not stride and steps > 1:
            for name, tns in (("reward", reward), ("terminated", terminated), ("actions", actions)):
                if tns is not None and ((tns.dim() > 1 and tns.shape[0] > 1) or tns.numel() > self.num_envs):
                    raise ValueError(f"{name} has {tns.numel()} elements in shape {tuple(tns.shape)} but no per-step obs_buffers were given: every "
                                     f"step would overwrite row 0 (pass ObsBuffers(n, device, steps={steps}), or a [N] tensor for the last step's values)")
        for name, tns, dt in (("reward", reward, torch.float64), ("terminated", terminated, torch.uint8), ("actions", actions, torch.int32)):
            _check_out_tensor(name, tns, dt, self.device, self.num_envs, int(steps) if stride else None)
        if zero_stats:
            self._stats.zero_()
        with torch.cuda.device(self.device):
            self._check(self._L.bg_rollout(
                self._h, int(steps), int(policy), C.c_uint64(policy_seed), C.c_uint64(env_index0), C.c_uint64(t0),
                C.byref(ob.ptrs), stride,
                None if reward is None else C.c_void_p(reward.data_ptr()),
                None if terminated is None else C.c_void_p(terminated.data_ptr()),
                None if actions is None else C.c_void_p(actions.data_ptr()),
                C.c_void_p(self._stats.data_ptr()), self._stream()), "bg_rollout")
        if self._rowbuf is not None:
            self.observe()
        return self._stats

    def stats(self) -> Dict[str, int]:
        self.check()
        s = self._stats.cpu().numpy()
        u = s.view(np.uint64)
        return {"steps": int(u[0]), "episodes": int(u[1]), "plays": int(u[2]), "score_sum": int(s[3]),
                "reward_bits": int(u[4]), "obs_hash": int(u[5])}

    def inject(self, jokers=None, money=None, ante=None, levels=None, mask=None, apply_now: bool = True):
        n = self.num_envs
        jptr = nptr = mptr = aptr = lptr = kptr = None
        keep = []
        if jokers is not None:
            ja = np.zeros((n, 5), np.int32)
            na = np.zeros(n, np.int32)
            for i, js in enumerate(jokers):
                na[i] = len(js)
                ja[i, :len(js)] = js
            keep += [ja, na]
            jptr, nptr = ja.ctypes.data_as(C.c_void_p), na.ctypes.data_as(C.c_void_p)
        if money is not None:
            ma = np.ascontiguousarray(np.asarray(money, np.int64)); keep.append(ma); mptr = ma.ctypes.data_as(C.c_void_p)
        if ante is not None:
            aa = np.ascontiguousarray(np.asarray(ante, np.int32)); keep.append(aa); aptr = aa.ctypes.data_as(C.c_void_p)
        if levels is not None:
            la = np.ascontiguousarray(np.asarray(levels, np.uint8)); keep.append(la); lptr = la.ctypes.data_as(C.c_void_p)
        if mask is not None:
            ka = np.ascontiguousarray(np.asarray(mask, np.uint8)); keep.append(ka); kptr = ka.ctypes.data_as(C.c_void_p)
        with torch.cuda.device(self.device):
            self._check(self._L.bg_inject(self._h, jptr, nptr, mptr, aptr, lptr, kptr, 1 if apply_now else 0,
                                          self._stream()), "bg_inject")

    def set_max_ante(self, max_ante, mask=None):
        mk = None if mask is None else np.ascontiguousarray(np.asarray(mask, np.uint8))
        per = None
        if not np.isscalar(max_ante):
            per = np.ascontiguousarray(np.asarray(max_ante, np.int32))
            if per.shape != (self.num_envs,):
                raise ValueError(f"per-env caps must have shape ({self.num_envs},)")
        with torch.cuda.device(self.device):
            self._check(self._L.bg_set_max_ante(
                self._h, 0 if per is not None else int(max_ante), None if per is None else per.ctypes.data_as(C.c_void_p),
                None if mk is None else mk.ctypes.data_as(C.c_void_p), self._stream()), "bg_set_max_ante")
        if per is None and mask is None:
            self.max_ante = int(max_ante)

    def inject_deck(self, decks, mask=None):
        da = np.ascontiguousarray(np.asarray(decks, np.uint8))
        if da.shape != (self.num_envs, 52):
            raise ValueError(f"decks must have shape ({self.num_envs}, 52)")
        mk = None if mask is None else np.ascontiguousarray(np.asarray(mask, np.uint8))
        with torch.cuda.device(self.device):
            self._check(self._L.bg_inject_deck(self._h, da.ctypes.data_as(C.c_void_p),
                                               None if mk is None else mk.ctypes.data_as(C.c_void_p), self._stream()),
                        "bg_inject_deck")
        self.observe()

    def inject_cards(self, cards, mask=None, apply_now: bool = True):
        n = self.num_envs
        enh = np.zeros((n, 52), np.uint8); edi = np.zeros((n, 52), np.uint8); seal = np.zeros((n, 52), np.uint8)
        for i, cs in enumerate(cards):
            for (idx, e, d, s) in cs:
                enh[i, idx], edi[i, idx], seal[i, idx] = e, d, s
        mk = None if mask is None else np.ascontiguousarray(np.asarray(mask, np.uint8))
        with torch.cuda.device(self.device):
            self._check(self._L.bg_inject_cards(
                self._h, enh.ctypes.data_as(C.c_void_p), edi.ctypes.data_as(C.c_void_p), seal.ctypes.data_as(C.c_void_p),
                None if mk is None else mk.ctypes.data_as(C.c_void_p), 1 if apply_now else 0, self._stream()), "bg_inject_cards")
        if apply_now:
            self.observe()

    def inject_consumables(self, consumables, mask=None, apply_now: bool = True):
        n = self.num_envs
        ids = np.zeros((n, 2), np.int32)
        cnt = np.zeros(n, np.int32)
        for i, cs in enumerate(consumables):
            cnt[i] = len(cs)
            ids[i, :len(cs)] = list(cs)[:2]
        mk = None if mask is None else np.ascontiguousarray(np.asarray(mask, np.uint8))
        with torch.cuda.device(self.device):
            self._check(self._L.bg_inject_consumables(
                self._h, ids.ctypes.data_as(C.c_void_p), cnt.ctypes.data_as(C.c_void_p),
                None if mk is None else mk.ctypes.data_as(C.c_void_p), 1 if apply_now else 0, self._stream()),
                "bg_inject_consumables")
        if apply_now:
            self.observe()

    def get_state(self, env_index: int) -> bytes:
        nb = int(self._L.bg_state_blob_bytes(self._h))
        buf = (C.c_uint8 * nb)()
        self._check(self._L.bg_get_state(self._h, int(env_index), buf, nb), "bg_get_state")
        return bytes(buf)

    def set_state(self, env_index: int, blob: bytes):
        buf = (C.c_uint8 * len(blob)).from_buffer_copy(blob)
        self._check(self._L.bg_set_state(self._h, int(env_index), buf, len(blob)), "bg_set_state")

    @staticmethod
    def parse_state_blob(blob: bytes) -> Dict[str, object]:
        b = np.frombuffer(blob, np.uint8)
        hdr = b[:16].view(np.uint32)
        kg, cards, ks, kd = int(hdr[2] & 0xffff), bool(hdr[2] & 0x10000), int(hdr[3] & 0xffff), int(hdr[3] >> 16)
        out: Dict[str, object] = {"magic": int(hdr[0]), "version": int(hdr[1]), "KG": kg, "KS": ks, "KD": kd, "card_states": cards}
        off = 16

        def take(name, nbytes, dtype=np.uint8, shape=None):
            nonlocal off
            a = b[off:off + nbytes].view(dtype)
            out[name] = a.reshape(shape) if shape else a
            off += nbytes
        take("hot", nat.BLOB_NHOT * 16, np.uint32, (nat.BLOB_NHOT, 4))
        take("deck", nat.BLOB_NDECK * 16)
        take("cold", nat.BLOB_NCOLD * 16)
        take("tmpl", nat.BLOB_NTMPL * 16)
        take("ring_decks", kd * nat.BLOB_NDECK * 16, np.uint8, (kd, nat.BLOB_NDECK * 16))
        take("global_blocks", kg * nat.BLOB_MTS * 4, np.uint32, (kg, nat.BLOB_MTS))
        take("shop_slots", ks * nat.SHOP_SLOT_WORDS * 4, np.uint32, (ks, nat.SHOP_SLOT_WORDS))
        take("shop_overflow", nat.BLOB_MTS * 4, np.uint32)
        take("deck_stream", nat.BLOB_MTS * 4, np.uint32)
        take("shopgen_stream", nat.BLOB_MTS * 4, np.uint32)
        take("shop_seed_ring", nat.BLOB_SSEED * 4, np.uint32)
        take("shop_seed_meta", 4, np.uint32)
        take("producers", 4, np.uint32)
        if cards:
            take("card_states", nat.BLOB_NCST * 16, np.uint16)
            take("card_template", nat.BLOB_NCST * 16, np.uint16)
            take("card_stream", nat.BLOB_MTS * 4, np.uint32)
            take("seal_stream", nat.BLOB_MTS * 4, np.uint32)
        if off != len(b):
            raise ValueError(f"state blob of {len(b)} bytes does not parse ({off} bytes understood)")
        out["deck"] = out["deck"][:52]
        out["ring_decks"] = out["ring_decks"][:, :52]
        out["shop_slot_seeds"] = out["shop_slots"][:, nat.SHOP_SLOT_SEED_WORD]
        hot7 = out["hot"][7]
        out["shop_slot_current"] = int(hot7[1] & 0xff)
        out["global_words_consumed"] = int((out["hot"][6][3] >> 24) & 0xff) * 624 + int(hot7[0] & 0xffff)
        return out

    def set_profiling(self, enable: bool):
        self._check(self._L.bg_set_profiling(self._h, 1 if enable else 0), "bg_set_profiling")

    def get_profile(self) -> Dict[str, float]:
        out = (C.c_double * 8)()
        self._check(self._L.bg_get_profile(self._h, out), "bg_get_profile")
        return {"rollout_ms": out[0], "rollout_launches": int(out[1]), "rollout_fused_steps": int(out[2]),
                "refill_ms": out[3], "refill_launches": int(out[4]), "step_ms": out[5], "step_launches": int(out[6])}

    def check(self):
        with torch.cuda.device(self.device):
            self._check(self._L.bg_check(self._h, self._stream()), "bg_check")


def classify_batch(cards: torch.Tensor, n: torch.Tensor, lanes_per_case: int = 1, timing: bool = False):
    L = nat.load()
    if cards.dtype != torch.uint8 or n.dtype != torch.uint8 or cards.dim() != 2 or cards.shape[1] != 8 or not cards.is_cuda \
            or tuple(n.shape) != (cards.shape[0],) or n.device != cards.device:
        raise ValueError("cards must be a uint8 [M, 8] device tensor, n a uint8 [M] tensor on the same device")
    cards, n = cards.contiguous(), n.contiguous()
    out = torch.empty(cards.shape[0], dtype=torch.uint8, device=cards.device)
    ms = C.c_float(0.0)
    with torch.cuda.device(cards.device):
        rc = L.bg_classify_batch_ex(C.c_void_p(cards.data_ptr()), C.c_void_p(n.data_ptr()), C.c_void_p(out.data_ptr()),
                                    C.c_int64(cards.shape[0]), int(lanes_per_case), C.byref(ms) if timing else None,
                                    C.c_void_p(torch.cuda.current_stream(cards.device).cuda_stream))
    if rc != 0:
        raise nat.NativeError(f"bg_classify_batch failed ({rc}): {L.bg_last_error(None).decode()}")
    return (out, float(ms.value)) if timing else out


def encode_rows(rows: torch.Tensor, layout: str = "produced", dtype: torch.dtype = torch.float32, out: Optional[torch.Tensor] = None,
                timing: bool = False):
    if layout not in nat.ENC_LAYOUTS:
        raise ValueError(f"layout must be one of {sorted(nat.ENC_LAYOUTS)} (got {layout!r})")
    if dtype not in (torch.float32, torch.bfloat16):
        raise ValueError("dtype must be torch.float32 or torch.bfloat16")
    if not isinstance(rows, torch.Tensor) or rows.dtype != torch.uint8 or rows.dim() < 1 or not rows.is_contiguous():
        raise ValueError("rows must be a contiguous uint8 tensor [..., stride] of packed records")
    stride = int(rows.shape[-1])
    if stride < nat.ROW_BYTES or stride % 16:
        raise ValueError(f"the last dimension of rows is the record stride: a multiple of 16, >= {nat.ROW_BYTES} (got {stride})")
    D = nat.ENC_COLS[nat.ENC_LAYOUTS[layout]]
    lead = tuple(rows.shape[:-1])
    m = int(np.prod(lead, dtype=np.int64))
    if out is not None:
        if out.dtype != dtype or out.device != rows.device:
            raise ValueError(f"out must be a {dtype} tensor on {rows.device}")
        if tuple(out.shape[:-1]) != lead or out.shape[-1] < D:
            raise ValueError(f"out must have shape {lead + ('>= %d' % D,)} (got {tuple(out.shape)})")
        pitch = int(out.stride(-2)) if out.dim() >= 2 else int(out.shape[-1])
        dense = out.stride(-1) == 1 and pitch >= out.shape[-1]
        for d in range(out.dim() - 2, 0, -1):
            dense = dense and out.stride(d - 1) == out.stride(d) * out.shape[d]
        if not dense:
            raise ValueError("out must have a contiguous last dimension and leading dimensions that are dense over its row pitch")
    if not rows.is_cuda:
        raise ValueError("rows must be a device tensor (there is no CPU fallback)")
    if rows.data_ptr() % 16:
        raise ValueError("rows must be 16-byte aligned")
    if out is None:
        out = torch.empty(lead + (D,), dtype=dtype, device=rows.device)
        pitch = D
    if m == 0:
        return (out[..., :D], 0.0) if timing else out[..., :D]
    L = nat.load()
    ms = C.c_float(0.0)
    with torch.cuda.device(rows.device):
        rc = L.bg_encode_rows(C.c_void_p(rows.data_ptr()), C.c_uint64(stride), C.c_int64(m), nat.ENC_LAYOUTS[layout],
                              nat.ENC_F32 if dtype == torch.float32 else nat.ENC_BF16, C.c_void_p(out.data_ptr()), C.c_uint64(pitch),
                              C.byref(ms) if timing else None, C.c_void_p(torch.cuda.current_stream(rows.device).cuda_stream))
    if rc != 0:
        raise nat.NativeError(f"bg_encode_rows failed ({rc}): {L.bg_last_error(None).decode()}")
    res = out[..., :D]
    return (res, float(ms.value)) if timing else res



def _head_logits(logits) -> tuple:
    if not isinstance(logits, torch.Tensor) or logits.dtype not in (torch.float32, torch.bfloat16) or logits.dim() < 1 or logits.shape[-1] != 60:
        raise ValueError("logits must be a float32 or bfloat16 tensor [..., 60]")
    pitch = int(logits.stride(-2)) if logits.dim() >= 2 else 60
    dense = logits.stride(-1) == 1 and pitch >= 60
    for d in range(logits.dim() - 2, 0, -1):
        dense = dense and logits.stride(d - 1) == logits.stride(d) * logits.shape[d]
    if not dense:
        raise ValueError("logits must have a contiguous last dimension and leading dimensions that are dense over its row pitch")
    lead = tuple(logits.shape[:-1])
    return lead, int(np.prod(lead, dtype=np.int64)), pitch


def _head_mask(mask, lead: tuple, device: torch.device) -> tuple:
    if mask is None:
        return None, 0, 0
    if not isinstance(mask, torch.Tensor) or mask.dim() < 1:
        raise ValueError("mask must be a uint8 tensor [..., stride] of packed records, an int8 tensor [..., 60] or None")
    if mask.dtype == torch.uint8:
        stride = int(mask.shape[-1])
        if not mask.is_contiguous() or stride < nat.ROW_BYTES or stride % 16:
            raise ValueError(f"a uint8 mask is a contiguous tensor [..., stride] of packed records: stride a multiple of 16, >= {nat.ROW_BYTES}")
        off = nat.ROW_OFFSETS["action_mask"]
    elif mask.dtype == torch.int8 and mask.shape[-1] == 60:
        stride = int(mask.stride(-2)) if mask.dim() >= 2 else 60
        dense = mask.stride(-1) == 1 and stride >= 60
        for d in range(mask.dim() - 2, 0, -1):
            dense = dense and mask.stride(d - 1) == mask.stride(d) * mask.shape[d]
        if not dense or stride % 4:
            raise ValueError("an int8 mask must have a contiguous last dimension and leading dimensions dense over a row pitch that is a multiple of 4")
        off = 0
    else:
        raise ValueError("mask must be a uint8 tensor [..., stride] of packed records, an int8 tensor [..., 60] or None")
    if tuple(mask.shape[:-1]) != lead:
        raise ValueError(f"mask must have the leading shape of logits {list(lead)} (got {list(mask.shape[:-1])})")
    if mask.device != device:
        raise ValueError(f"mask must be on {device}")
    return mask, off, stride


def _head_call(name: str, logits, mask, given, flags: int, seed: int, index0: int, t: int, actions, log_prob, entropy, timing: bool):
    lead, m, pitch = _head_logits(logits)
    dev = logits.device
    mask, moff, mstride = _head_mask(mask, lead, dev)
    for what, v in (("seed", seed), ("index0", index0), ("t", t)):
        if not isinstance(v, (int, np.integer)) or isinstance(v, bool) or not 0 <= int(v) < 2 ** 64:
            raise ValueError(f"{what} must be an integer in [0, 2**64)")
    if given is not None:
        _check_scan_tensor("actions", given, torch.int32, lead, dev)
    for what, tt, dt in (("actions", actions, torch.int32), ("log_prob", log_prob, torch.float32), ("entropy", entropy, torch.float32)):
        if tt is not None:
            _check_scan_tensor(what, tt, dt, lead, dev)
    if not logits.is_cuda:
        raise ValueError("logits must be a device tensor (there is no CPU fallback)")
    if mask is not None and (mask.data_ptr() + moff) % 4:
        raise ValueError("mask must be 4-byte aligned")
    if given is None and actions is None:
        actions = torch.empty(lead, dtype=torch.int32, device=dev)
    if log_prob is None:
        log_prob = torch.empty(lead, dtype=torch.float32, device=dev)
    if entropy is None:
        entropy = torch.empty(lead, dtype=torch.float32, device=dev)
    res = (log_prob, entropy) if given is not None else (actions, log_prob, entropy)
    if m == 0:
        return res + (0.0,) if timing else res
    outs = [x.data_ptr() for x in res]
    ins = [logits.data_ptr()] + ([mask.data_ptr()] if mask is not None else []) + ([given.data_ptr()] if given is not None else [])
    if len(set(outs)) != len(outs) or set(outs) & set(ins):
        raise ValueError("outputs must not share memory with the inputs or with each other")
    L = nat.load()
    ms = C.c_float(0.0)
    with torch.cuda.device(dev):
        head = (C.c_void_p(logits.data_ptr()), nat.HEAD_F32 if logits.dtype == torch.float32 else nat.HEAD_BF16, C.c_uint64(pitch),
                C.c_void_p(mask.data_ptr() + moff) if mask is not None else None, C.c_uint64(mstride), C.c_int64(m))
        tail = (C.c_void_p(log_prob.data_ptr()), C.c_void_p(entropy.data_ptr()), C.byref(ms) if timing else None,
                C.c_void_p(torch.cuda.current_stream(dev).cuda_stream))
        if given is None:
            rc = L.bg_sample_actions(*head, C.c_uint32(flags), C.c_uint64(int(seed)), C.c_uint64(int(index0)), C.c_uint64(int(t)),
                                     C.c_void_p(actions.data_ptr()), *tail)
        else:
            rc = L.bg_evaluate_actions(*head, C.c_void_p(given.data_ptr()), *tail)
    if rc != 0:
        raise nat.NativeError(f"{name} failed ({rc}): {L.bg_last_error(None).decode()}")
    return res + (float(ms.value),) if timing else res


def sample_actions(logits: torch.Tensor, mask: Optional[torch.Tensor] = None, *, seed: int, t: int, index0: int = 0, deterministic: bool = False,
                   actions: Optional[torch.Tensor] = None, log_prob: Optional[torch.Tensor] = None, entropy: Optional[torch.Tensor] = None,
                   timing: bool = False):
    return _head_call("bg_sample_actions", logits, mask, None, nat.HEAD_DETERMINISTIC if deterministic else 0, seed, index0, t, actions, log_prob,
                      entropy, timing)


def evaluate_actions(logits: torch.Tensor, actions: torch.Tensor, mask: Optional[torch.Tensor] = None, *, log_prob: Optional[torch.Tensor] = None,
                     entropy: Optional[torch.Tensor] = None, timing: bool = False):
    if not isinstance(actions, torch.Tensor):
        raise ValueError("actions must be an int32 tensor with the leading shape of logits")
    return _head_call("bg_evaluate_actions", logits, mask, actions, 0, 0, 0, 0, None, log_prob, entropy, timing)


def _check_scan_rows(rows) -> tuple:
    if not isinstance(rows, torch.Tensor) or rows.dtype != torch.uint8 or rows.dim() != 3 or not rows.is_contiguous():
        raise ValueError("rows must be a contiguous uint8 tensor [K, N, stride] of packed records")
    K, N, stride = (int(x) for x in rows.shape)
    if stride < nat.ROW_BYTES or stride % 16:
        raise ValueError(f"the last dimension of rows is the record stride: a multiple of 16, >= {nat.ROW_BYTES} (got {stride})")
    return K, N, stride


def _check_scan_tensor(name: str, t, dtype: torch.dtype, shape: tuple, device: torch.device):
    if not isinstance(t, torch.Tensor) or t.dtype != dtype or tuple(t.shape) != shape or not t.is_contiguous() or t.device != device:
        raise ValueError(f"{name} must be a contiguous {dtype} tensor of shape {list(shape)} on {device}")


def gae_rows(rows: torch.Tensor, values: torch.Tensor, last_values: torch.Tensor, gamma: float = 0.99, gae_lambda: float = 0.95,
             advantages: Optional[torch.Tensor] = None, returns: Optional[torch.Tensor] = None, timing: bool = False,
             rewards: Optional[torch.Tensor] = None):
    K, N, stride = _check_scan_rows(rows)
    dev = rows.device
    _check_scan_tensor("values", values, torch.float32, (K, N), dev)
    _check_scan_tensor("last_values", last_values, torch.float32, (N,), dev)
    for name, t in (("advantages", advantages), ("returns", returns)):
        if t is not None:
            _check_scan_tensor(name, t, torch.float32, (K, N), dev)
    if rewards is not None:
        _check_scan_tensor("rewards", rewards, torch.float64, (K, N), dev)
    gamma, gae_lambda = float(gamma), float(gae_lambda)
    if not (np.isfinite(gamma) and np.isfinite(gae_lambda)):
        raise ValueError("gamma and gae_lambda must be finite")
    if not rows.is_cuda:
        raise ValueError("rows must be a device tensor (there is no CPU fallback)")
    if rows.data_ptr() % 16:
        raise ValueError("rows must be 16-byte aligned")
    if advantages is None:
        advantages = torch.empty((K, N), dtype=torch.float32, device=dev)
    if returns is None:
        returns = torch.empty((K, N), dtype=torch.float32, device=dev)
    ptrs = [values.data_ptr(), advantages.data_ptr(), returns.data_ptr()]
    if K * N and len(set(ptrs)) != 3:
        raise ValueError("advantages / returns must not share memory with values or with each other")
    if K * N == 0:
        return (advantages, returns, 0.0) if timing else (advantages, returns)
    L = nat.load()
    ms = C.c_float(0.0)
    with torch.cuda.device(dev):
        args = (C.c_void_p(rows.data_ptr()), C.c_uint64(stride), K, C.c_int64(N), C.c_void_p(values.data_ptr()),
                C.c_void_p(last_values.data_ptr()), C.c_double(gamma), C.c_double(gae_lambda), C.c_void_p(advantages.data_ptr()),
                C.c_void_p(returns.data_ptr()))
        tail = (C.byref(ms) if timing else None, C.c_void_p(torch.cuda.current_stream(dev).cuda_stream))
        rc = L.bg_gae_rows(*args, *tail) if rewards is None else L.bg_gae_rows_ex(*args, C.c_void_p(rewards.data_ptr()), *tail)
    if rc != 0:
        raise nat.NativeError(f"bg_gae_rows failed ({rc}): {L.bg_last_error(None).decode()}")
    return (advantages, returns, float(ms.value)) if timing else (advantages, returns)


class EpisodeStats:

    def __init__(self, n: int, device):
        if int(n) < 0:
            raise ValueError("n must be >= 0")
        self.n = int(n)
        self.device = torch.device(device)
        self.ep_return_carry = torch.zeros(self.n, dtype=torch.float64, device=self.device)
        self.ep_len_carry = torch.zeros(self.n, dtype=torch.int32, device=self.device)

    def reset(self, mask: Optional[torch.Tensor] = None) -> None:
        if mask is None:
            self.ep_return_carry.zero_()
            self.ep_len_carry.zero_()
            return
        mask = torch.as_tensor(mask)
        if tuple(mask.shape) != (self.n,):
            raise ValueError(f"mask must have shape [{self.n}]")
        mask = mask.to(device=self.device, dtype=torch.bool)
        self.ep_return_carry.masked_fill_(mask, 0.0)
        self.ep_len_carry.masked_fill_(mask, 0)

    def update(self, rows: torch.Tensor, ep_return: Optional[torch.Tensor] = None, ep_len: Optional[torch.Tensor] = None, timing: bool = False):
        K, N, stride = _check_scan_rows(rows)
        if N != self.n or rows.device != self.device:
            raise ValueError(f"rows must hold records of {self.n} envs on {self.device} (got {N} envs on {rows.device})")
        if ep_return is not None:
            _check_scan_tensor("ep_return", ep_return, torch.float64, (K, N), self.device)
        if ep_len is not None:
            _check_scan_tensor("ep_len", ep_len, torch.int32, (K, N), self.device)
        if not rows.is_cuda:
            raise ValueError("rows must be a device tensor (there is no CPU fallback)")
        if rows.data_ptr() % 16:
            raise ValueError("rows must be 16-byte aligned")
        if ep_return is None:
            ep_return = torch.empty((K, N), dtype=torch.float64, device=self.device)
        if ep_len is None:
            ep_len = torch.empty((K, N), dtype=torch.int32, device=self.device)
        if K * N == 0:
            return (ep_return, ep_len, 0.0) if timing else (ep_return, ep_len)
        L = nat.load()
        ms = C.c_float(0.0)
        with torch.cuda.device(self.device):
            rc = L.bg_episode_stats_rows(C.c_void_p(rows.data_ptr()), C.c_uint64(stride), K, C.c_int64(N), C.c_void_p(self.ep_return_carry.data_ptr()),
                                         C.c_void_p(self.ep_len_carry.data_ptr()), C.c_void_p(ep_return.data_ptr()), C.c_void_p(ep_len.data_ptr()),
                                         C.byref(ms) if timing else None, C.c_void_p(torch.cuda.current_stream(self.device).cuda_stream))
        if rc != 0:
            raise nat.NativeError(f"bg_episode_stats_rows failed ({rc}): {L.bg_last_error(None).decode()}")
        return (ep_return, ep_len, float(ms.value)) if timing else (ep_return, ep_len)


def _norm_rows(rows) -> torch.Tensor:
# ... 179 lines not shown
```

Before: 7.767 billion.

## Pre-twist deck and shop-seed MT streams into a two-block ring via wave kernel

Replaces the per-thread lazy Mersenne Twister stream, which twisted words on the fly and wrote the state back, with a two-block ring per env for the deck and shopgen streams. A new wave-cooperative twist kernel, generalised from the global-block refill, fills whole blocks ahead of time. The deck shuffle and seed-ring consumers then only read tempered words. This moves twist arithmetic and read-modify-write traffic off the divergent per-thread consumers onto coalesced wave-wide passes. In exchange it doubles ring memory per env, adds extra kernel launches per refill, and adds an inline-twist retry path and a new error code for when a ring runs dry.

```diff
diff --git a/balatro_gym_amd/csrc/bg_device.h b/balatro_gym_amd/csrc/bg_device.h
--- a/balatro_gym_amd/csrc/bg_device.h
+++ b/balatro_gym_amd/csrc/bg_device.h
@@ -16,6 +16,7 @@
 #define BG_DEVERR_SHOPBLK 2u
 #define BG_DEVERR_DECKRING 4u
 #define BG_DEVERR_SHOPRING 8u
+#define BG_DEVERR_STREAMRING 32u
 
 typedef __attribute__((address_space(1))) unsigned long long g_u64;
 typedef __attribute__((address_space(1))) uint32_t g_u32;
@@ -197,8 +198,13 @@
   p[1] = (m1 ^ ((b ^ (b >> 30)) * 1566083941u)) - 1u;
   p[0] = 0x80000000u;
 }
-__device__ __forceinline__ uint32_t* bg_deckmt(const BgDev& d, int env) { return d.deckmt + (size_t)env * BG_MTS; }
-__device__ __forceinline__ uint32_t* bg_shopgenmt(const BgDev& d, int env) { return d.shopgenmt + (size_t)env * BG_MTS; }
+#define BG_RING_K 2
+#define BG_RM_POS(m) ((m) & 0x3ffu)
+#define BG_RM_BLK(m) (((m) >> 10) & 1u)
+#define BG_RM_NB(m) (((m) >> 11) & 3u)
+#define BG_RM_PACK(pos, blk, nb) ((uint32_t)(pos) | ((uint32_t)(blk) << 10) | ((uint32_t)(nb) << 11))
+__device__ __forceinline__ uint32_t* bg_deckmt(const BgDev& d, int env) { return d.deckmt + (size_t)env * (BG_RING_K * BG_MTS); }
+__device__ __forceinline__ uint32_t* bg_shopgenmt(const BgDev& d, int env) { return d.shopgenmt + (size_t)env * (BG_RING_K * BG_MTS); }
 
 #ifdef BG_TIMING
 __shared__ unsigned long long bg_probe_lds[32];
diff --git a/balatro_gym_amd/csrc/bg_lib.hip b/balatro_gym_amd/csrc/bg_lib.hip
--- a/balatro_gym_amd/csrc/bg_lib.hip
+++ b/balatro_gym_amd/csrc/bg_lib.hip
@@ -182,56 +182,79 @@
 __device__ void bg_mt_seed(uint32_t* __restrict__ p, uint32_t key) { bg_mt_seed_impl<false>(p, key); }
 __device__ void bg_mt_seed_slot(uint32_t* __restrict__ p, uint32_t key) { bg_mt_seed_impl<true>(p, key); }
 
-__device__ __forceinline__ uint32_t bg_q156(uint32_t q) { return q >= 156u ? q - 156u : q; }
-#define BG_LAZY_U 4
-#define BG_LAZY_U_SEEDRING 2
+#define BG_RING_U 4
 #define BG_WL_COUNTERS 32
 #define BG_REFILL_WAVE_PRIO 0
-template <int U = BG_LAZY_U, class F>
-__device__ __forceinline__ uint32_t bg_lazy_stream(uint32_t* S, uint32_t c, bool active, F&& take) {
-  uint4* S4 = (uint4*)S;
-  uint32_t q = c >> 2, off = c & 3u, fq = bg_q156(q + 99u);
-  uint4 a[U + 1], f[U + 1];
-#pragma unroll
-  for (int g = 0; g <= U; g++) { a[g] = make_uint4(0, 0, 0, 0); f[g] = a[g]; }
+struct BgRingPos { uint32_t blk, pos, avail, nb; };
+__device__ __forceinline__ BgRingPos bg_ring_pos(uint32_t m) { return BgRingPos{BG_RM_BLK(m), BG_RM_POS(m), BG_RM_NB(m) * (uint32_t)BG_MT_N - BG_RM_POS(m), BG_RM_NB(m)}; }
+__device__ __forceinline__ uint32_t bg_ring_meta(const BgRingPos& p) { return BG_RM_PACK(p.pos, p.blk, p.nb); }
+__device__ __forceinline__ void bg_ring_advance(BgRingPos& p, uint32_t used) {
+  const uint32_t lin = p.pos + used, c = lin / (uint32_t)BG_MT_N;
+  p.pos = lin - c * (uint32_t)BG_MT_N; p.blk = (p.blk + c) & 1u; p.nb -= c; p.avail -= used;
+}
+__device__ __forceinline__ uint32_t bg_ring_g4(uint32_t v) { if (v >= 312u) v -= 312u; return v + (v >= 156u ? (uint32_t)(BG_MTS - BG_MT_N) / 4u : 0u); }
+template <class F>
+__device__ __forceinline__ uint32_t bg_ring_stream(const uint32_t* ring, const BgRingPos& p, bool active, bool& done, F&& take) {
+  const uint4* R4 = (const uint4*)ring;
+  const uint32_t avail = p.avail;
+  uint32_t v = p.blk * 156u + (p.pos >> 2), off = p.pos & 3u, used = 0;
+  done = false;
+  active = active && avail != 0u;
+  uint4 a[BG_RING_U];
+#pragma unroll
+  for (int g = 0; g < BG_RING_U; g++) a[g] = make_uint4(0, 0, 0, 0);
   if (active) {
 #pragma unroll
-    for (int g = 0; g <= U; g++) { a[g] = S4[bg_q156(q + (uint32_t)g)]; f[g] = S4[bg_q156(fq + (uint32_t)g)]; }
-  }
+    for (int g = 0; g < BG_RING_U; g++) a[g] = R4[bg_ring_g4(v + (uint32_t)g)];
+  }
+  auto one = [&](uint32_t y) { used++; if (!take(y)) { done = true; return false; } return used < avail; };
 #pragma unroll 1
   while (__ballot(active) != 0ull) {
-    uint4 an[U], fn[U];
-#pragma unroll
-    for (int g = 0; g < U; g++) { an[g] = a[0]; fn[g] = a[0]; }
+    uint4 an[BG_RING_U];
+#pragma unroll
+    for (int g = 0; g < BG_RING_U; g++) an[g] = a[0];
     if (active) {
 #pragma unroll
-      for (int g = 0; g < U; g++) { an[g] = S4[bg_q156(q + (uint32_t)(U + 1 + g))]; fn[g] = S4[bg_q156(fq + (uint32_t)(U + 1 + g))]; }
+      for (int g = 0; g < BG_RING_U; g++) an[g] = R4[bg_ring_g4(v + (uint32_t)(BG_RING_U + g))];
     }
     bool more = active;
 #pragma unroll
-    for (int g = 0; g < U; g++) {
-      const uint4 a0 = a[g], f0 = f[g];
-      const uint32_t n0 = bg_twist(a0.x, a0.y, f0.y), n1 = bg_twist(a0.y, a0.z, f0.z), n2 = bg_twist(a0.z, a0.w, f0.w), n3 = bg_twist(a0.w, a[g + 1].x, f[g + 1].x);
+    for (int g = 0; g < BG_RING_U; g++) {
+      const uint4 a0 = a[g];
       const uint32_t goff = g == 0 ? off : 0u;
-      uint4 o = a0;
-      uint32_t used = 0;
-      if (more && goff == 0u) { o.x = n0; used++; more = take(n0); }
-      if (more && goff <= 1u) { o.y = n1; used++; more = take(n1); }
-      if (more && goff <= 2u) { o.z = n2; used++; more = take(n2); }
-      if (more) { o.w = n3; used++; more = take(n3); }
-      if (used) {
-        const uint32_t qg = bg_q156(q + (uint32_t)g);
-        S4[qg] = o;
-        if (!more) { c = 4u * qg + goff + used; if (c >= (uint32_t)BG_MT_N) c -= (uint32_t)BG_MT_N; active = false; }
-      }
-    }
-    q = bg_q156(q + (uint32_t)U); fq = bg_q156(fq + (uint32_t)U); off = 0u;
-    a[0] = a[U]; f[0] = f[U];
-#pragma unroll
-    for (int g = 0; g < U; g++) { a[g + 1] = an[g]; f[g + 1] = fn[g]; }
-  }
-  return c;
-}
+      if (more && goff == 0u) more = one(a0.x);
+      if (more && goff <= 1u) more = one(a0.y);
+      if (more && goff <= 2u) more = one(a0.z);
+      if (more) more = one(a0.w);
+    }
+    active = more;
+    v += (uint32_t)BG_RING_U; if (v >= 312u) v -= 312u;
+    off = 0u;
+#pragma unroll
+    for (int g = 0; g < BG_RING_U; g++) a[g] = an[g];
+  }
+  return used;
+}
+template <class D>
+__device__ __forceinline__ bool bg_shuffle_word(uint32_t y, int& i, D&& card) {
+  const int k = 32 - __clz((uint32_t)(i + 1));
+  const uint32_t j = bg_temper(y) >> (32 - k);
+  if (j <= (uint32_t)i) {
+    const uint8_t a = card(i), b = card((int)j);
+    card(i) = b; card((int)j) = a;
+    i--;
+  }
+  return i >= 1;
+}
+template <class D>
+__device__ __forceinline__ bool bg_ring_shuffle(const uint32_t* ring, BgRingPos& p, bool active, D&& card) {
+  int i = 51;
+  bool done;
+  const uint32_t used = bg_ring_stream(ring, p, active, done, [&](uint32_t y) { return bg_shuffle_word(y, i, card); });
+  if (done) bg_ring_advance(p, used);
+  return done;
+}
+__device__ __forceinline__ bool bg_seed_word(uint32_t y, uint32_t& r) { r = bg_temper(y); return r < 2147483648u; }
 
 #define BG_MTB 16
 #define BG_SSEED 128
@@ -301,10 +324,16 @@
     seed = (int64_t)(r & 0xffffffffull);
   }
   uint32_t base = (uint32_t)(uint64_t)seed;
-  bg_mt_seed(bg_deckmt(d, env), base);
-  bg_deckmt(d, env)[BG_MT_N] = BG_LAZY_SEEDED;
-  bg_mt_seed(bg_shopgenmt(d, env), base + 2000u);
-  bg_shopgenmt(d, env)[BG_MT_N] = BG_LAZY_SEEDED;
+  {
+    uint32_t* r0 = bg_deckmt(d, env);
+    bg_mt_seed(r0, base);
+    bg_mt_twist(r0, r0);
+    r0[BG_MT_N] = BG_RM_PACK(0, 0, 1);
+    uint32_t* r2 = bg_shopgenmt(d, env);
+    bg_mt_seed(r2, base + 2000u);
+    bg_mt_twist(r2, r2);
+    r2[BG_MT_N] = BG_RM_PACK(0, 0, 1);
+  }
   if (d.cardmt) {
     bg_mt_seed(d.cardmt + (size_t)env * BG_MTS, base + 11000u);
     d.cardmt[(size_t)env * BG_MTS + BG_MT_N] = BG_LAZY_SEEDED;
@@ -369,7 +398,49 @@
   if (g_valid > 0 && g_valid < d.KG) { uint32_t i = atomicAdd(&d.wl_count[2], 1u); d.wl[2 * N + i] = (uint32_t)env; }
 }
 
-__global__ __launch_bounds__(BG_BLOCK) __attribute__((amdgpu_waves_per_eu(4, 4))) void bg_refill_deck_kernel(BgDev d, BgPart pt, uint32_t cursor_idx, uint32_t max_made) {
+__device__ __forceinline__ int bg_wave_twist(uint32_t* ring, int depth, int last, int valid, bool mirror, int l) {
+  constexpr int NR = (BG_MT_N + 63) / 64;
+  int made = 0;
+  uint32_t o[NR + 1];
+  {
+    const uint32_t* src = ring + (size_t)last * BG_MTS;
+#pragma unroll
+    for (int r = 0; r < NR; r++) o[r] = (64 * r + l < BG_MT_N) ? __builtin_nontemporal_load(&src[64 * r + l]) : 0u;
+    o[NR] = 0u;
+  }
+#pragma unroll 1
+  while (valid < depth) {
+    const int nxt = last + 1 == depth ? 0 : last + 1;
+    uint32_t* dst = ring + (size_t)nxt * BG_MTS;
+    uint32_t n[NR];
+#pragma unroll
+    for (int r = 0; r < NR; r++) {
+      const int k = 64 * r + l;
+      const uint32_t up_same = __shfl(o[r], (l + 1) & 63), up_next = __shfl(o[r + 1], 0);
+      uint32_t up = l == 63 ? up_next : up_same;
+      if (r == NR - 1) { const uint32_t new0 = __shfl(n[0], 0); if (k == BG_MT_N - 1) up = new0; }
+      uint32_t far = 0u;
+      if (64 * r < BG_MT_N - BG_MT_M) {
+        const uint32_t a = r + 6 < NR ? __shfl(o[r + 6], (l + 13) & 63) : 0u, b2 = r + 7 < NR ? __shfl(o[r + 7], (l + 13) & 63) : 0u;
+        far = l + 13 < 64 ? a : b2;
+      }
+      if (64 * r + 63 >= BG_MT_N - BG_MT_M) {
+        const uint32_t a = r >= 4 ? __shfl(n[r >= 4 ? r - 4 : 0], (l + 29) & 63) : 0u, b2 = r >= 3 ? __shfl(n[r >= 3 ? r - 3 : 0], (l + 29) & 63) : 0u;
+        const uint32_t fn = l + 29 < 64 ? a : b2;
+        if (k >= BG_MT_N - BG_MT_M) far = fn;
+      }
+      n[r] = bg_twist(o[r], up, far);
+      if (k < BG_MT_N) __builtin_nontemporal_store(n[r], &dst[k]);
+    }
+    if (mirror && l < 16) ring[(size_t)last * BG_MTS + BG_MT_N + l] = n[0];
+#pragma unroll
+    for (int r = 0; r < NR; r++) o[r] = n[r];
+    last = nxt; valid++; made++;
+  }
+  return made;
+}
+
+__global__ __launch_bounds__(BG_BLOCK) __attribute__((amdgpu_waves_per_eu(4, 4))) void bg_refill_deck_kernel(BgDev d, BgPart pt, uint32_t cursor_idx, uint32_t max_made, uint32_t inline_twist) {
   __builtin_amdgcn_s_setprio(BG_REFILL_WAVE_PRIO);
   __shared__ uint8_t sdeck[52][BG_BLOCK];
   const size_t N = d.N;
@@ -378,8 +449,9 @@
   uint32_t* const cursor = &d.wl_count[cursor_idx];
   const int cap = max_made ? (int)max_made : 1 << 30;
   int env = 0, d_head = 0, d_ready = 0, made = 0;
-  uint32_t prod = 0, cur = 0;
-  uint32_t* mt = bg_deckmt(d, 0);
+  uint32_t prod = 0;
+  uint32_t* ring = bg_deckmt(d, 0);
+  BgRingPos p{0u, 0u, 0u, 0u};
   bool have = false, need = false, dry = false;
 #pragma unroll 1
   while (true) {
@@ -394,12 +466,12 @@
         const uint32_t my = base + (uint32_t)__popcll(freem & ((1ull << tid) - 1ull));
         if (!have && my < count) {
           env = (int)d.wl[my];
-          mt = bg_deckmt(d, env);
+          ring = bg_deckmt(d, env);
           const uint32_t w5 = ((const uint32_t*)&d.hot[(size_t)5 * N + env])[3];
           prod = d.prod_out[env];
           d_head = bg_b(w5, 2);
           d_ready = (int)((prod - (uint32_t)bg_b(w5, 3)) & 0xffu);
-          cur = mt[BG_MT_N] & 0x3ffu;
+          p = bg_ring_pos(ring[BG_MT_N]);
           made = 0;
           need = d_ready < d.KD;
           have = need;
@@ -407,19 +479,11 @@
       }
     }
     if (__ballot(need) == 0ull) { if (dry) break; continue; }
-    if (need) { int p = 0; for (int s = 0; s < 4; s++) for (int r = 0; r < 13; r++) sdeck[p++][tid] = (uint8_t)(r * 4 + s); }
-    int i = 51;
-    cur = bg_lazy_stream(mt, cur, need, [&](uint32_t y) {
-      const int k = 32 - __clz((uint32_t)(i + 1));
-      const uint32_t j = bg_temper(y) >> (32 - k);
-      if (j <= (uint32_t)i) {
-        const uint8_t a = sdeck[i][tid], b = sdeck[j][tid];
-        sdeck[i][tid] = b; sdeck[j][tid] = a;
-        i--;
-      }
-      return i >= 1;
-    });
-    if (need) {
+    if (need) { int q = 0; for (int s = 0; s < 4; s++) for (int r = 0; r < 13; r++) sdeck[q++][tid] = (uint8_t)(r * 4 + s); }
+    const bool full = p.nb >= (uint32_t)BG_RING_K;
+    const bool done = bg_ring_shuffle(ring, p, need, [&](int k) -> uint8_t& { return sdeck[k][tid]; });
+    const bool ran_out = need && !done;
+    if (done) {
       const int slot = (d_head + d_ready) % d.KD;
 #pragma unroll
       for (int k = 0; k < BG_NDECK; k++) {
@@ -429,12 +493,25 @@
         d.ndeck[((size_t)slot * BG_NDECK + k) * N + env] = make_uint4(wv[0], wv[1], wv[2], wv[3]);
       }
       d_ready++; made++;
-      need = d_ready < d.KD && made < cap;
-      if (!need) {
-        mt[BG_MT_N] = cur | BG_LAZY_SEEDED;
-        ((uint8_t*)&d.prod_out[env])[0] = (uint8_t)((prod + (uint32_t)made) & 0xffu);
-        have = false;
+    }
+    if (ran_out && full) atomicOr(d.err, BG_DEVERR_STREAMRING);
+    const bool retry = ran_out && !full && inline_twist != 0u;
+    if (need && !retry && (ran_out || d_ready >= d.KD || made >= cap)) {
+      ring[BG_MT_N] = bg_ring_meta(p);
+      ((uint8_t*)&d.prod_out[env])[0] = (uint8_t)((prod + (uint32_t)made) & 0xffu);
+      need = false; have = false;
+    }
+    unsigned long long tw = __ballot(retry);
+    if (tw != 0ull) {
+      while (tw != 0ull) {
+        const int src = __ffsll(tw) - 1;
+        tw &= tw - 1ull;
+        const int e2 = __shfl(env, src);
+        const uint32_t blk2 = (uint32_t)__shfl((int)p.blk, src), nb2 = (uint32_t)__shfl((int)p.nb, src);
+        const int mk = bg_wave_twist(bg_deckmt(d, e2), BG_RING_K, (int)((blk2 + nb2 + 1u) & 1u), (int)nb2, false, tid);
+        if (tid == src) { p.nb += (uint32_t)mk; p.avail += (uint32_t)mk * (uint32_t)BG_MT_N; }
       }
+      __threadfence();
     }
   }
 }
@@ -446,23 +523,27 @@
   for (uint32_t base = lo + blockIdx.x * BG_BLOCK; base < count; base += gridDim.x * BG_BLOCK) {
     const bool valid = base + threadIdx.x < count;
     const int env = valid ? (int)d.wl[N + base + threadIdx.x] : 0;
-    uint32_t* mt = bg_shopgenmt(d, env);
+    uint32_t* ring = bg_shopgenmt(d, env);
     int head = 0, cnt = BG_SSEED;
-    uint32_t cur = 0;
+    BgRingPos p{0u, 0u, 0u, 0u};
     if (valid) {
       const uint32_t sm = d.smeta[env];
       head = (int)(sm & 0xffu); cnt = (int)((sm >> 8) & 0xffu);
-      cur = mt[BG_MT_N] & 0x3ffu;
+      p = bg_ring_pos(ring[BG_MT_N]);
     }
     const bool need = valid && cnt < BG_SSEED;
-    cur = bg_lazy_stream<BG_LAZY_U_SEEDRING>(mt, cur, need, [&](uint32_t y) {
-      const uint32_t r = bg_temper(y);
-      if (r < 2147483648u) { d.sseed[(size_t)env * BG_SSEED + ((head + cnt) & (BG_SSEED - 1))] = r; cnt++; }
+    const bool full = p.nb >= (uint32_t)BG_RING_K;
+    bool done;
+    const uint32_t used = bg_ring_stream(ring, p, need, done, [&](uint32_t y) {
+      uint32_t r;
+      if (bg_seed_word(y, r)) { d.sseed[(size_t)env * BG_SSEED + ((head + cnt) & (BG_SSEED - 1))] = r; cnt++; }
       return cnt < BG_SSEED;
     });
     if (need) {
-      mt[BG_MT_N] = cur | BG_LAZY_SEEDED;
+      bg_ring_advance(p, used);
+      ring[BG_MT_N] = bg_ring_meta(p);
       d.smeta[env] = (uint32_t)head | ((uint32_t)cnt << 8);
+      if (!done && full) atomicOr(d.err, BG_DEVERR_STREAMRING);
     }
   }
 }
@@ -474,59 +555,32 @@
     bg_mt_seed_slot(bg_sblock(d, (int)(es & 0xffffffu), (int)(es >> 24)), seed);
   }
 }
-__global__ __launch_bounds__(BG_BLOCK) void bg_refill_gblk_kernel(BgDev d, BgPart pt) {
+__global__ __launch_bounds__(BG_BLOCK) void bg_refill_twist_kernel(BgDev d, BgPart pt, uint32_t kind) {
   __builtin_amdgcn_s_setprio(BG_REFILL_WAVE_PRIO);
   const size_t N = d.N;
-  const uint32_t count0 = d.wl_count[2], lo = bg_part_lo(count0, pt), count = bg_part_hi(count0, pt);
+  const uint32_t count0 = d.wl_count[kind], lo = bg_part_lo(count0, pt), count = bg_part_hi(count0, pt);
+  const uint32_t* const list = d.wl + (size_t)kind * N;
   const int l = threadIdx.x;
-  constexpr int NR = (BG_MT_N + 63) / 64;
   for (uint32_t item = lo + blockIdx.x; item < count; item += gridDim.x) {
-    const int env = (int)d.wl[2 * N + item];
-    const uint32_t w6 = ((const uint32_t*)&d.hot[(size_t)6 * N + env])[3];
-    const uint32_t prod = d.prod_out[env];
-    const int g_cur = bg_b(w6, 2), g_cons = bg_b(w6, 3);
-    int g_valid = (int)(((prod >> 16) - (uint32_t)g_cons) & 0xffu);
-    if (g_valid <= 0 || g_valid >= d.KG) continue;
-    int last = (g_cur + g_valid - 1) % d.KG, made = 0;
-    uint32_t o[NR + 1];
-    {
-      const uint32_t* src = bg_gblock(d, env, last);
-#pragma unroll
-      for (int r = 0; r < NR; r++) o[r] = (64 * r + l < BG_MT_N) ? __builtin_nontemporal_load(&src[64 * r + l]) : 0u;
-      o[NR] = 0u;
-    }
-#pragma unroll 1
-    while (g_valid < d.KG) {
-      const int nxt = last + 1 == d.KG ? 0 : last + 1;
-      uint32_t* dst = bg_gblock(d, env, nxt);
-      uint32_t n[NR];
-#pragma unroll
-      for (int r = 0; r < NR; r++) {
-        const int k = 64 * r + l;
-        const uint32_t up_same = __shfl(o[r], (l + 1) & 63), up_next = __shfl(o[r + 1], 0);
-        uint32_t up = l == 63 ? up_next : up_same;
-        if (r == NR - 1) { const uint32_t new0 = __shfl(n[0], 0); if (k == BG_MT_N - 1) up = new0; }
-        uint32_t far = 0u;
-        if (64 * r < BG_MT_N - BG_MT_M) {
-          const uint32_t a = r + 6 < NR ? __shfl(o[r + 6], (l + 13) & 63) : 0u, b2 = r + 7 < NR ? __shfl(o[r + 7], (l + 13) & 63) : 0u;
-          far = l + 13 < 64 ? a : b2;
-        }
-        if (64 * r + 63 >= BG_MT_N - BG_MT_M) {
-          const uint32_t a = r >= 4 ? __shfl(n[r >= 4 ? r - 4 : 0], (l + 29) & 63) : 0u, b2 = r >= 3 ? __shfl(n[r >= 3 ? r - 3 : 0], (l + 29) & 63) : 0u;
-          const uint32_t fn = l + 29 < 64 ? a : b2;
-          if (k >= BG_MT_N - BG_MT_M) far = fn;
-        }
-        n[r] = bg_twist(o[r], up, far);
-        if (k < BG_MT_N) __builtin_nontemporal_store(n[r], &dst[k]);
+    const int env = (int)list[item];
+    if (kind == 2u) {
+      const uint32_t w6 = ((const uint32_t*)&d.hot[(size_t)6 * N + env])[3];
+      const uint32_t prod = d.prod_out[env];
+      const int g_cur = bg_b(w6, 2), g_cons = bg_b(w6, 3);
+      const int g_valid = (int)(((prod >> 16) - (uint32_t)g_cons) & 0xffu);
+      if (g_valid <= 0 || g_valid >= d.KG) continue;
+      const int made = bg_wave_twist(bg_gblock(d, env, 0), d.KG, (g_cur + g_valid - 1) % d.KG, g_valid, true, l);
+      if (made && l == 0) {
+        const uint32_t g = ((prod >> 16) + (uint32_t)made) & 0xffu;
+        ((uint8_t*)&d.prod_out[env])[2] = (uint8_t)g;
       }
-      if (l < 16) bg_gblock(d, env, last)[BG_MT_N + l] = n[0];
-#pragma unroll
-      for (int r = 0; r < NR; r++) o[r] = n[r];
-      last = nxt; g_valid++; made++;
-    }
-    if (made && l == 0) {
-      const uint32_t g = ((prod >> 16) + (uint32_t)made) & 0xffu;
-      ((uint8_t*)&d.prod_out[env])[2] = (uint8_t)g;
+    } else {
+      uint32_t* ring = kind == 0u ? bg_deckmt(d, env) : bg_shopgenmt(d, env);
+      const uint32_t m = ring[BG_MT_N];
+      const int nb = (int)BG_RM_NB(m);
+      if (nb >= BG_RING_K) continue;
+      const int made = bg_wave_twist(ring, BG_RING_K, (int)((BG_RM_BLK(m) + (uint32_t)nb + 1u) & 1u), nb, false, l);
+      if (l == 0) ring[BG_MT_N] = m + ((uint32_t)made << 11);
     }
   }
 }
@@ -796,8 +850,8 @@
     if (e == hipSuccess) e = bg_alloc(h, &d.cardmt, (size_t)BG_MTS * N);
     if (e == hipSuccess) e = bg_alloc(h, &d.sealmt, (size_t)BG_MTS * N);
   }
-  if (e == hipSuccess) e = bg_alloc(h, &d.deckmt, (size_t)BG_MTS * N);
-  if (e == hipSuccess) e = bg_alloc(h, &d.shopgenmt, (size_t)BG_MTS * N);
+  if (e == hipSuccess) e = bg_alloc(h, &d.deckmt, (size_t)BG_RING_K * BG_MTS * N);
+  if (e == hipSuccess) e = bg_alloc(h, &d.shopgenmt, (size_t)BG_RING_K * BG_MTS * N);
   if (e == hipSuccess) e = bg_alloc(h, &d.wl_count, BG_WL_COUNTERS);
   if (e == hipSuccess) e = bg_alloc(h, &d.wl, 3 * N);
   if (e == hipSuccess) e = bg_alloc(h, &d.wl_shop, 2 * N * (size_t)(d.KS - 1));
@@ -889,6 +943,7 @@
   return 0;
 }
 
+#define BG_TWIST_PIECE_GRID 1024
 static int bg_refill_pieces(bg_handle* h, int n) {
   const BgDev& d = h->piece_dev;
   hipStream_t s = h->side;
@@ -897,16 +952,25 @@
     const BgPart pt{pc.part, pc.nparts};
     hipEvent_t ea = nullptr, eb = nullptr;
     bg_ev_pair(h, h->ev_refill_t, ea, eb);
-    const dim3 g(pc.grid), b(BG_BLOCK);
+    const dim3 g(pc.grid), b(BG_BLOCK), gt(pc.kind < 3 ? BG_TWIST_PIECE_GRID : 1);
+    const uint32_t inl = pc.max_made == 0u ? 1u : 0u;
     if (ea) {
-      if (pc.kind == 0) hipExtLaunchKernelGGL(bg_refill_deck_kernel, g, b, 0, s, ea, eb, 0, d, pt, pc.cursor, pc.max_made);
-      else if (pc.kind == 1) hipExtLaunchKernelGGL(bg_refill_seedring_kernel, g, b, 0, s, ea, eb, 0, d, pt);
-      else if (pc.kind == 2) hipExtLaunchKernelGGL(bg_refill_gblk_kernel, g, b, 0, s, ea, eb, 0, d, pt);
+      if (pc.kind == 0) {
+        hipExtLaunchKernelGGL(bg_refill_twist_kernel, gt, b, 0, s, ea, nullptr, 0, d, pt, 0u);
+        hipExtLaunchKernelGGL(bg_refill_deck_kernel, g, b, 0, s, nullptr, eb, 0, d, pt, pc.cursor, pc.max_made, inl);
+      } else if (pc.kind == 1) {
+        hipExtLaunchKernelGGL(bg_refill_twist_kernel, gt, b, 0, s, ea, nullptr, 0, d, pt, 1u);
+        hipExtLaunchKernelGGL(bg_refill_seedring_kernel, g, b, 0, s, nullptr, eb, 0, d, pt);
+      } else if (pc.kind == 2) hipExtLaunchKernelGGL(bg_refill_twist_kernel, g, b, 0, s, ea, eb, 0, d, pt, 2u);
       else hipExtLaunchKernelGGL(bg_refill_shop_kernel, g, b, 0, s, ea, eb, 0, d, pt);
     } else {
-      if (pc.kind == 0) hipLaunchKernelGGL(bg_refill_deck_kernel, g, b, 0, s, d, pt, pc.cursor, pc.max_made);
-      else if (pc.kind == 1) hipLaunchKernelGGL(bg_refill_seedring_kernel, g, b, 0, s, d, pt);
-      else if (pc.kind == 2) hipLaunchKernelGGL(bg_refill_gblk_kernel, g, b, 0, s, d, pt);
+      if (pc.kind == 0) {
+        hipLaunchKernelGGL(bg_refill_twist_kernel, gt, b, 0, s, d, pt, 0u);
+        hipLaunchKernelGGL(bg_refill_deck_kernel, g, b, 0, s, d, pt, pc.cursor, pc.max_made, inl);
+      } else if (pc.kind == 1) {
+        hipLaunchKernelGGL(bg_refill_twist_kernel, gt, b, 0, s, d, pt, 1u);
+        hipLaunchKernelGGL(bg_refill_seedring_kernel, g, b, 0, s, d, pt);
+      } else if (pc.kind == 2) hipLaunchKernelGGL(bg_refill_twist_kernel, g, b, 0, s, d, pt, 2u);
       else hipLaunchKernelGGL(bg_refill_shop_kernel, g, b, 0, s, d, pt);
     }
     BG_HIP(hipGetLastError());
@@ -954,9 +1018,13 @@
   const int full = 4096;
   int dense = full;
   if (steps_hint >= 0 && steps_hint < 372) { dense = (int)((long)full * (steps_hint + 24) / 372); if (dense < 512) dense = 512; if (dense > full) dense = full; }
-  hipLaunchKernelGGL(bg_refill_deck_kernel, dim3(dense), dim3(BG_BLOCK), 0, s, d, whole, 4u, 0u);
+  hipLaunchKernelGGL(bg_refill_twist_kernel, dim3(dense), dim3(BG_BLOCK), 0, s, d, whole, 0u);
+  hipLaunchKernelGGL(bg_refill_deck_kernel, dim3(dense), dim3(BG_BLOCK), 0, s, d, whole, 4u, 0u, 0u);
+  hipLaunchKernelGGL(bg_refill_twist_kernel, dim3(dense), dim3(BG_BLOCK), 0, s, d, whole, 0u);
+  hipLaunchKernelGGL(bg_refill_deck_kernel, dim3(dense), dim3(BG_BLOCK), 0, s, d, whole, 5u, 0u, 1u);
+  hipLaunchKernelGGL(bg_refill_twist_kernel, dim3(dense), dim3(BG_BLOCK), 0, s, d, whole, 1u);
   hipLaunchKernelGGL(bg_refill_seedring_kernel, dim3(dense), dim3(BG_BLOCK), 0, s, d, whole);
-  hipLaunchKernelGGL(bg_refill_gblk_kernel, dim3(dense), dim3(BG_BLOCK), 0, s, d, whole);
+  hipLaunchKernelGGL(bg_refill_twist_kernel, dim3(dense), dim3(BG_BLOCK), 0, s, d, whole, 2u);
   hipLaunchKernelGGL(bg_refill_shop_kernel, dim3(dense), dim3(BG_BLOCK), 0, s, d, whole);
   bg_ev_end(h, h->ev_refill_t, s);
   BG_HIP(hipGetLastError());
@@ -984,8 +1052,8 @@
   BG_HIP(hipMemcpyAsync(&w, h->dev.err, sizeof(w), hipMemcpyDeviceToHost, (hipStream_t)stream));
   BG_HIP(hipStreamSynchronize((hipStream_t)stream));
   if (w) {
-    char buf[256];
-    snprintf(buf, sizeof(buf), "device invariant violated: error word 0x%x (1 global-stream underflow, 2 shop block, 4 deck ring, 8 shop ring, 16 a bounded wait inside the step engine expired)", w);
+    char buf[400];
+    snprintf(buf, sizeof(buf), "device invariant violated: error word 0x%x (1 global-stream underflow, 2 shop block, 4 deck ring, 8 shop ring, 16 a bounded wait inside the step engine expired, 32 a full stream-0 / stream-2 block ring did not finish one shuffle / seed ring)", w);
     h->err = buf;
     return BG_E_INTERNAL;
   }
@@ -1496,7 +1564,7 @@
   v.push_back({d.hot, BG_NHOT, 16}); v.push_back({d.deck, BG_NDECK, 16}); v.push_back({d.cold, BG_NCOLD, 16});
   v.push_back({d.tmpl, BG_NTMPL, 16}); v.push_back({d.ndeck, (size_t)d.KD * BG_NDECK, 16});
   v.push_back({d.gblk, 1, (size_t)d.KG * BG_MTS * 4}); v.push_back({d.sblk, 1, (size_t)d.KS * BG_SLOT_WORDS * 4}); v.push_back({d.sovf, 1, (size_t)BG_MTS * 4});
-  v.push_back({d.deckmt, 1, (size_t)BG_MTS * 4}); v.push_back({d.shopgenmt, 1, (size_t)BG_MTS * 4});
+  v.push_back({d.deckmt, 1, (size_t)BG_RING_K * BG_MTS * 4}); v.push_back({d.shopgenmt, 1, (size_t)BG_RING_K * BG_MTS * 4});
   v.push_back({d.sseed, 1, BG_SSEED * 4}); v.push_back({d.smeta, 1, 4});
   v.push_back({bg_prod_latest(h), 1, 4});
   if (d.cstate) { v.push_back({d.cstate, BG_NCST, 16}); v.push_back({d.ctmpl, BG_NCST, 16}); v.push_back({d.cardmt, 1, (size_t)BG_MTS * 4}); v.push_back({d.sealmt, 1, (size_t)BG_MTS * 4}); }
@@ -1510,7 +1578,7 @@
   return b;
 }
 #define BG_BLOB_MAGIC 0x42474d58u
-#define BG_BLOB_VERSION 7u
+#define BG_BLOB_VERSION 8u
 static int bg_blob_args(bg_handle* h, const char* fn, int env_index, const void* blob, uint64_t blob_bytes) {
   if (!h) return BG_E_ARG;
   char buf[200];
diff --git a/balatro_gym_amd/vec_env.py b/balatro_gym_amd/vec_env.py
--- a/balatro_gym_amd/vec_env.py
+++ b/balatro_gym_amd/vec_env.py
@@ -480,8 +480,8 @@
         take("global_blocks", kg * nat.BLOB_MTS * 4, np.uint32, (kg, nat.BLOB_MTS))
         take("shop_slots", ks * nat.SHOP_SLOT_WORDS * 4, np.uint32, (ks, nat.SHOP_SLOT_WORDS))
         take("shop_overflow", nat.BLOB_MTS * 4, np.uint32)
-        take("deck_stream", nat.BLOB_MTS * 4, np.uint32)
-        take("shopgen_stream", nat.BLOB_MTS * 4, np.uint32)
+        take("deck_stream", 2 * nat.BLOB_MTS * 4, np.uint32, (2, nat.BLOB_MTS))
+        take("shopgen_stream", 2 * nat.BLOB_MTS * 4, np.uint32, (2, nat.BLOB_MTS))
         take("shop_seed_ring", nat.BLOB_SSEED * 4, np.uint32)
         take("shop_seed_meta", 4, np.uint32)
         take("producers", 4, np.uint32)
```

Result: slower. 7.249 billion (-6.7%).
